# Ignalina/znippy

Hardware: AMD Instinct MI355X
Metric: decompress MB/s (uncompressed) + compress MB/s, 100k x 10KB archive (higher is better)
Workload: dtype u8; 1 GPU; 100k x 10KiB text chunks (BASELINE configs[1]); rows_per_gpu=100000, chunk_bytes=10240, bytes_per_gpu=1024000000, blob_bytes_per_gpu=6400000, parallelism=row-cursor ranges x1, pipelining=step k+1 queued before step k's counters are read (two runs in flight)

## Files before the change

### znippy_amd/csrc/api.hip

```cpp
#include <unistd.h>
#include "common.h"
#include "encode.h"
#include "../../include/znippy_hip.h"

#include <algorithm>
#include <cstdio>
#include <cstdlib>
#include <cstring>
#include <chrono>
#include <memory>
#include <string>
#include <vector>
#include <unordered_map>

namespace zn {
int measure_b3_pass_ns(int cus, hipStream_t s, float *ns_per_pass_per_simd, float *ghz);
size_t decode_lit_scratch_bytes(int grid);
void set_fused_dbg(unsigned long long *p);
void set_fused_abl(int v);
}

using namespace zn;
extern "C" void zn_rounds_totals(const uint64_t *len, const uint8_t *skip, size_t n, uint64_t out[8]);
extern "C" void zn_rows_extents(const uint64_t *bo, const uint64_t *bs, const uint64_t *oo, const uint64_t *us, size_t n, uint64_t out[8]);
extern "C" int zn_rows_pack32(const uint64_t *bo, const uint64_t *bs, const uint64_t *oo, const uint64_t *us, size_t n, uint32_t *dst);

#define HIPCHK(ctx, call)                                                                         \
    do {                                                                                          \
        hipError_t e_ = (call);                                                                   \
        if (e_ != hipSuccess) {                                                                   \
            (ctx)->err = std::string(#call) + ": " + hipGetErrorString(e_);                       \
            return ZNIPPY_E_HIP;                                                                  \
        }                                                                                         \
    } while (0)

struct TDbg {
    bool on;
    const char *what;
    std::chrono::steady_clock::time_point t;
    std::string line;
    TDbg(bool on_, const char *what_) : on(on_), what(what_), t(std::chrono::steady_clock::now()) {}
    void mark(const char *name) {
        if (!on) return;
        const auto now = std::chrono::steady_clock::now();
        char b[96];
        snprintf(b, sizeof b, " %s=%.3f", name, std::chrono::duration<double, std::milli>(now - t).count());
        line += b;
        t = now;
    }
    ~TDbg() { if (on) fprintf(stderr, "[znippy tdbg] %s:%s ms\n", what, line.c_str()); }
};

struct KTime {
    const char *name;
    hipEvent_t t0, t1;
};

struct znippy_ctx {
    int device = 0;
    hipStream_t stream = nullptr;
    bool own_stream = false;
    std::string err;
    int decode_grid = 0;
    uint8_t *lit_scratch = nullptr;
    uint32_t *cursor = nullptr;
    uint8_t *shim_in = nullptr, *shim_out = nullptr;
    size_t shim_in_cap = 0, shim_out_cap = 0;
    int encode_grid = 0, encode_grid_small = 0;
    int gen_share = 3;
    int level = 19;
    int window_log = 0;
    uint32_t *ldm = nullptr;
    size_t ldm_cap = 0;
    uint8_t *enc_prov = nullptr;
    size_t enc_prov_cap = 0;
    uint32_t *enc_seq = nullptr;
    EncTables *enc_tabs = nullptr;
    hipStream_t aux = nullptr;
    hipStream_t copy = nullptr;
    uint8_t *lit_scratch_b = nullptr;
    uint8_t *fz_lit_pool = nullptr;
    unsigned long long *fz_seq_pool = nullptr;
    uint64_t fz_lit_cap = 0, fz_seq_cap = 0;
    uint16_t *bx_fse_pool = nullptr;
    uint16_t *bx_huf_pool = nullptr;
    uint64_t bx_fse_cap = 0, bx_huf_cap = 0;
    uint32_t *rx_pool = nullptr, *rx_chunk = nullptr;
    uint8_t *rx_cdone = nullptr;
    uint64_t rx_cap = 0;
    uint8_t *vs_pool = nullptr;
    uint64_t vs_cap = 0;
    hipEvent_t ev_fork = nullptr, ev_join = nullptr, ev_join2 = nullptr;
    std::vector<KTime> ktimes;
    int n_ktimes = 0;
    std::vector<hipEvent_t> event_pool;
    bool ktime_open = false;
    std::vector<std::pair<size_t, void *>> pinned_pool;
    size_t pinned_pool_bytes = 0;
    std::vector<std::pair<size_t, void *>> dev_pool;
    std::unordered_map<void *, size_t> dev_sizes;
    size_t dev_pool_bytes = 0;
    struct {
        int dbg = 0;
        unsigned lds_pad = 0;
        int store_g = 0;
        bool no_block_items = false, no_fused_blocks = false, ddbg = false, edbg = false, no_fused_store = false,
             nohash = false, no_roles = false, no_fz = false, fz_only = false, no_bx = false, tdbg = false, no_fuse_hash = false, trace = false, no_rx = false, no_pack = false, no_lean = false, no_stored_only = false;
        unsigned roles_min = 2048;
        unsigned bx_big = BX_BIG_SEQ;
        bool bx_big_set = false;
        int ktime = 2;
    } sw;
    int cus = 256;
    int live_tables = 0;
    bool closing = false;
    unsigned long long *clk_buf = nullptr;
    enum Diag { DIAG_FUSED, DIAG_ITEMS, DIAG_FZ, DIAG_GENERAL, DIAG_BX, DIAG_ENCODE, DIAG_N };
    unsigned long long *diag[DIAG_N] = {};
};

static void read_switches(znippy_ctx *ctx) {
    auto on = [](const char *n) { const char *v = getenv(n); return v && *v && *v != '0'; };
    if (const char *e = getenv("ZNIPPY_DBG")) ctx->sw.dbg = atoi(e);
    if (const char *e = getenv("ZNIPPY_LDS_PAD")) ctx->sw.lds_pad = (unsigned)atoi(e);
    ctx->sw.no_block_items = on("ZNIPPY_NO_BLOCK_ITEMS");
    ctx->sw.no_fused_blocks = on("ZNIPPY_NO_FUSED_BLOCKS");
    ctx->sw.ddbg = on("ZNIPPY_DDBG");
    ctx->sw.edbg = on("ZNIPPY_EDBG");
    ctx->sw.no_fused_store = on("ZNIPPY_NO_FUSED_STORE");
    ctx->sw.nohash = on("ZNIPPY_NOHASH");
    ctx->sw.no_roles = on("ZNIPPY_NO_ROLES");
    ctx->sw.no_fz = on("ZNIPPY_NO_FZ");
    ctx->sw.tdbg = on("ZNIPPY_TDBG");
    ctx->sw.trace = on("ZNIPPY_TRACE");
    ctx->sw.no_lean = on("ZNIPPY_NO_LEAN");
    ctx->sw.no_pack = on("ZNIPPY_NO_PACK");
    if (const char *e = getenv("ZNIPPY_STORE_G")) ctx->sw.store_g = atoi(e) == 1 ? 1 : (atoi(e) == 2 ? 2 : 0);
    ctx->sw.no_stored_only = on("ZNIPPY_NO_STORED_ONLY");
    ctx->sw.no_rx = on("ZNIPPY_NO_RX");
    ctx->sw.no_fuse_hash = on("ZNIPPY_NO_FUSE_HASH");
    ctx->sw.no_bx = on("ZNIPPY_NO_BX");
    if (const char *e = getenv("ZNIPPY_BX_BIG")) { ctx->sw.bx_big = (unsigned)atoi(e); ctx->sw.bx_big_set = true; }
    if (const char *lv = getenv("ZNIPPY_LEVEL")) { const int v = atoi(lv); if (v >= 1 && v <= 22) ctx->level = v; }
    if (const char *wl = getenv("ZNIPPY_WINDOW_LOG")) { const int v = atoi(wl); if (v == 0 || (v >= WINDOW_LOG_MIN && v <= WINDOW_LOG_MAX)) ctx->window_log = v; }
    if (const char *gs = getenv("ZNIPPY_GEN_SHARE")) { const int v = atoi(gs); if (v >= 1 && v <= 4) ctx->gen_share = v; }
    ctx->sw.fz_only = on("ZNIPPY_FZ_ONLY");
    if (const char *e = getenv("ZNIPPY_ROLES_MIN")) ctx->sw.roles_min = (unsigned)atoi(e);
    if (const char *e = getenv("ZNIPPY_KTIME")) ctx->sw.ktime = atoi(e);
}

static void *pinned_take(znippy_ctx *ctx, size_t bytes, size_t *cap) {
    size_t best = ctx->pinned_pool.size();
    for (size_t i = 0; i < ctx->pinned_pool.size(); i++)
        if (ctx->pinned_pool[i].first >= bytes && ctx->pinned_pool[i].first <= 4 * bytes + 4096 &&
            (best == ctx->pinned_pool.size() || ctx->pinned_pool[i].first < ctx->pinned_pool[best].first))
            best = i;
    if (best != ctx->pinned_pool.size()) {
        void *p = ctx->pinned_pool[best].second;
        *cap = ctx->pinned_pool[best].first;
        ctx->pinned_pool_bytes -= *cap;
        ctx->pinned_pool.erase(ctx->pinned_pool.begin() + best);
        return p;
    }
    void *p = nullptr;
    if (hipHostMalloc(&p, bytes) != hipSuccess) return nullptr;
    *cap = bytes;
    return p;
}
static void pinned_give(znippy_ctx *ctx, void *p, size_t cap) {
    if (!p) return;
    if (ctx->pinned_pool.size() < 16 && ctx->pinned_pool_bytes + cap <= (256ull << 20)) {
        ctx->pinned_pool.emplace_back(cap, p);
        ctx->pinned_pool_bytes += cap;
    } else (void)hipHostFree(p);
}
static hipEvent_t event_take(znippy_ctx *ctx) {
    if (!ctx->event_pool.empty()) {
        hipEvent_t e = ctx->event_pool.back();
        ctx->event_pool.pop_back();
        return e;
    }
    hipEvent_t e = nullptr;
    if (hipEventCreateWithFlags(&e, hipEventDisableTiming) != hipSuccess) return nullptr;
    return e;
}
static void event_give(znippy_ctx *ctx, hipEvent_t e) {
    if (!e) return;
    if (ctx->event_pool.size() < 64) ctx->event_pool.push_back(e);
    else (void)hipEventDestroy(e);
}

template <class T>
static hipError_t tmalloc(znippy_ctx *ctx, T **out, size_t bytes) {
    bytes = std::max<size_t>(bytes, 16);
    size_t best = ctx->dev_pool.size();
    for (size_t i = 0; i < ctx->dev_pool.size(); i++)
        if (ctx->dev_pool[i].first >= bytes && ctx->dev_pool[i].first <= 2 * bytes + 4096 &&
            (best == ctx->dev_pool.size() || ctx->dev_pool[i].first < ctx->dev_pool[best].first))
            best = i;
    if (best != ctx->dev_pool.size()) {
        *out = (T *)ctx->dev_pool[best].second;
        ctx->dev_sizes[*out] = ctx->dev_pool[best].first;
        ctx->dev_pool_bytes -= ctx->dev_pool[best].first;
        ctx->dev_pool.erase(ctx->dev_pool.begin() + best);
        return hipSuccess;
    }
    void *p = nullptr;
    const hipError_t e = hipMalloc(&p, bytes);
    if (e != hipSuccess) return e;
    *out = (T *)p;
    ctx->dev_sizes[p] = bytes;
    return hipSuccess;
}
static void tfree(znippy_ctx *ctx, void *p) {
    if (!p) return;
    auto it = ctx->dev_sizes.find(p);
    if (it == ctx->dev_sizes.end()) { (void)hipFree(p); return; }
    const size_t cap = it->second;
    ctx->dev_sizes.erase(it);
    if (ctx->dev_pool.size() < 96 && ctx->dev_pool_bytes + cap <= (1ull << 30)) {
        ctx->dev_pool.emplace_back(cap, p);
        ctx->dev_pool_bytes += cap;
    } else (void)hipFree(p);
}

struct PlanBuf {
    std::vector<Tile> tiles;
    std::vector<BigUnit> big;
    uint32_t n_tile_cv = 0;
    std::vector<uint32_t> grp_big, grp_k;
};

template <class LenOf>
static void build_plan(LenOf len_of, uint32_t n, PlanBuf &p) {
    p.tiles.reserve((size_t)n / 4 + 16);
    uint32_t cur_first = 0, cur_units = 0, cur_leaves = 0;
    auto flush = [&]() {
        if (cur_units) p.tiles.push_back(Tile{cur_first, cur_units, 0, cur_leaves, 0, 0});
        cur_units = 0;
        cur_leaves = 0;
    };
    for (uint32_t u = 0; u < n; u++) {
        const uint64_t len_u = len_of(u);
        uint64_t leaves64 = len_u ? (len_u + 1023) >> 10 : 1;
        if (leaves64 > 64) {
            flush();
            uint32_t n_cvs = (uint32_t)((leaves64 + 63) / 64);
            p.big.push_back(BigUnit{u, p.n_tile_cv, n_cvs, 0});
            if (n_cvs > 64)
                for (uint32_t g = 0; g < (n_cvs + 63) / 64; g++) { p.grp_big.push_back((uint32_t)p.big.size() - 1); p.grp_k.push_back(g); }
            for (uint32_t t = 0; t < n_cvs; t++) {
                uint32_t first = t * 64;
                uint32_t nl = (uint32_t)std::min<uint64_t>(64, leaves64 - first);
                p.tiles.push_back(Tile{u, 0, first, nl, p.n_tile_cv + t, 0});
            }
            p.n_tile_cv += n_cvs;
        } else {
            uint32_t leaves = (uint32_t)leaves64;
            if (cur_units == 64 || cur_leaves + leaves > 64) flush();
            if (!cur_units) cur_first = u;
            cur_units++;
            cur_leaves += leaves;
            if (cur_units == 1 && u + 1 < n && len_of(u + 1) == len_u) {
                uint32_t v = u + 1;
                while (v < n && len_of(v) == len_u) v++;
                const uint32_t per = std::min<uint32_t>(64 / leaves, 64), run = v - u, full = run / per;
                if (full >= 1) {
                    for (uint32_t t = 0; t < full; t++) p.tiles.push_back(Tile{u + t * per, per, 0, per * leaves, 0, 0});
                    cur_units = 0; cur_leaves = 0;
                    const uint32_t rest = run - full * per;
                    if (rest) { cur_first = u + full * per; cur_units = rest; cur_leaves = rest * leaves; }
                    u = v - 1;
                }
            }
        }
    }
    flush();
    uint32_t gb = 0;
    for (BigUnit &b : p.big)
        if (b.n_cvs > 64) { b.pad = p.n_tile_cv + gb; gb += (b.n_cvs + 63) / 64; }
}

struct DevPlan {
    Tile *tiles = nullptr;
    BigUnit *big = nullptr;
    uint32_t *tile_cv = nullptr;
    uint32_t *grp_big = nullptr, *grp_k = nullptr;
    uint32_t n_grp = 0;
    uint32_t n_tiles = 0, n_big = 0;
    uint32_t max_cvs = 0;
};

static int upload_plan(znippy_ctx *ctx, const PlanBuf &p, DevPlan &d) {
    d.n_tiles = (uint32_t)p.tiles.size();
    d.n_big = (uint32_t)p.big.size();
    d.max_cvs = 0;
    for (const BigUnit &b : p.big) d.max_cvs = std::max(d.max_cvs, b.n_cvs);
    if (d.n_tiles) {
        HIPCHK(ctx, tmalloc(ctx, &d.tiles, sizeof(Tile) * d.n_tiles));
        HIPCHK(ctx, hipMemcpy(d.tiles, p.tiles.data(), sizeof(Tile) * d.n_tiles, hipMemcpyHostToDevice));
    }
    if (d.n_big) {
        HIPCHK(ctx, tmalloc(ctx, &d.big, sizeof(BigUnit) * d.n_big));
        HIPCHK(ctx, hipMemcpy(d.big, p.big.data(), sizeof(BigUnit) * d.n_big, hipMemcpyHostToDevice));
        HIPCHK(ctx, tmalloc(ctx, &d.tile_cv, 32 * ((size_t)p.n_tile_cv + p.grp_big.size())));
        d.n_grp = (uint32_t)p.grp_big.size();
        if (d.n_grp) {
            HIPCHK(ctx, tmalloc(ctx, &d.grp_big, 4 * (size_t)d.n_grp));
            HIPCHK(ctx, tmalloc(ctx, &d.grp_k, 4 * (size_t)d.n_grp));
            HIPCHK(ctx, hipMemcpy(d.grp_big, p.grp_big.data(), 4 * (size_t)d.n_grp, hipMemcpyHostToDevice));
            HIPCHK(ctx, hipMemcpy(d.grp_k, p.grp_k.data(), 4 * (size_t)d.n_grp, hipMemcpyHostToDevice));
        }
    }
    return ZNIPPY_OK;
}

static void free_plan(znippy_ctx *ctx, DevPlan &d) {
    tfree(ctx, d.tiles);
    tfree(ctx, d.big);
    tfree(ctx, d.tile_cv);
    tfree(ctx, d.grp_big);
    tfree(ctx, d.grp_k);
    d = DevPlan();
}

struct CtlRegion { size_t at, bytes; };
constexpr CtlRegion CTL_COUNTERS{0, 8 * 8};
constexpr CtlRegion CTL_HAND{64, 16 * 4};
constexpr CtlRegion CTL_CURSORS{128, 16 * 4};
constexpr CtlRegion CTL_FZ_POOL{192, 8 * 8};
constexpr CtlRegion CTL_BX_POOL{256, 16 * 8};
constexpr CtlRegion CTL_BX_CTR{384, 16 * 4};
constexpr CtlRegion CTL_RX{448, 16 * 4};
constexpr size_t CTL_HEAD = 512, CTL_MIRROR = 128, CTL_FLAG = 7;
constexpr uint32_t RX_ZERO = 15;
enum Hand : uint32_t {
    H_FUSED = 0,
    H_SERIAL = 1,
    H_ITEMS = 2,
    H_TILES = 3,
    H_FLAGGED = 5,
};
enum Cursor : uint32_t { CUR_GENERAL = 0, CUR_ROLES = 2, CUR_ITEMS = 4, CUR_FALLBACK = 8, CUR_FZ = 12, CUR_FZ_WORK = 13 };
constexpr uint32_t LEAN_ANY = 1u << H_FUSED | 1u << H_SERIAL | 1u << H_FLAGGED, LEAN_SMALL = LEAN_ANY | 1u << H_TILES, LEAN_BLOCKS = LEAN_ANY | 1u << H_ITEMS;
constexpr bool ctl_before(CtlRegion a, CtlRegion b) { return a.at + a.bytes <= b.at; }
static_assert(ctl_before(CTL_COUNTERS, CTL_HAND) && ctl_before(CTL_HAND, CTL_CURSORS) && ctl_before(CTL_CURSORS, CTL_FZ_POOL) && ctl_before(CTL_FZ_POOL, CTL_BX_POOL) &&
              ctl_before(CTL_BX_POOL, CTL_BX_CTR) && ctl_before(CTL_BX_CTR, CTL_RX) && CTL_RX.at + CTL_RX.bytes <= CTL_HEAD, "control block: regions overlap or pass the head");
static_assert(CTL_COUNTERS.at == 0 && CTL_HAND.at == CTL_COUNTERS.bytes && CTL_MIRROR == CTL_HAND.at + CTL_HAND.bytes, "the mirror is exactly counters + hand-over counts");
static_assert(CTL_FLAG < 8 && H_FLAGGED == H_SERIAL + 4 && H_FLAGGED < 8 && CUR_FZ_WORK < 16 && zn::RX_ROUNDS <= RX_ZERO && RX_ZERO < 16, "control block: a word outside its region");

struct znippy_rows {
    znippy_ctx *ctx = nullptr;
    uint64_t row_begin = 0;
    uint32_t n = 0;
    uint32_t n_compressed = 0;
    uint64_t *blob_off = nullptr, *blob_size = nullptr, *usize = nullptr, *out_off = nullptr;
    uint8_t *compressed = nullptr, *checksum = nullptr, *d_bitmap = nullptr;
    uint32_t *h_pack = nullptr, *d_pack = nullptr;
    size_t h_pack_cap = 0;
    unsigned long long *d_pack_sums = nullptr;
    uint8_t *ctl = nullptr;
    size_t ctl_bytes = 0;
    template <class T> T *ctl_at(CtlRegion g, size_t i = 0) const { return reinterpret_cast<T *>(ctl + g.at) + i; }
    uint32_t *hand(Hand h) const { return ctl_at<uint32_t>(CTL_HAND, h); }
    uint32_t *cur(Cursor c) const { return ctl_at<uint32_t>(CTL_CURSORS, c); }
    int32_t *status = nullptr;
    uint32_t *digests = nullptr;
    uint64_t *counters = nullptr;
    uint64_t *h_counters = nullptr;
    const uint32_t *mirror_hand(unsigned slot) const { return reinterpret_cast<const uint32_t *>(reinterpret_cast<const uint8_t *>(h_counters + 16 * slot) + CTL_HAND.at); }
    size_t h_counters_cap = 0;
    int bx_hint = -1;
    bool lean_ok = false;
    int lean_hint = -1;
    bool lean_blocks_ok = false;
    bool lean_mixed_ok = false;
    bool roles_off = false;
    bool small_ok = false, small_off = false;
    uint32_t *all_rows = nullptr;
    int lean_hint2 = -1;
    struct RunArgs { const void *blobs = nullptr; void *out = nullptr; uint64_t base = 0, cap = 0, blob_cap = ~0ull; bool verify = false; } run_args[2];
    uint64_t *vs_off = nullptr;
    uint64_t vs_bytes = 0;
    bool vs_built = false;
    bool no_out = false;
    hipEvent_t ev_done[2] = {nullptr, nullptr};
    uint64_t run_seq = 0;
    uint64_t ext_min_bo = 0, ext_max_bend = 0, ext_max_oend = 0;
    bool ext_wrap = false;
    std::vector<uint64_t> h_blob_off, h_blob_size, h_len, h_out_off;
    uint64_t blob_cap = ~0ull;
    uint64_t val_base = 0, val_bcap = 0, val_ocap = 0;
    bool val_done = false, val_verify = false;
    uint32_t n_bad = 0;
    bool force_full = false;
    uint8_t *status_init = nullptr;
    bool odd_out = false;
    uint64_t *corrupt = nullptr;
    uint32_t corrupt_cap = 0;
    uint32_t *list_a = nullptr;
    uint32_t n_list_a = 0;
    bool wide_rows = false;
    uint32_t *pending = nullptr;
    uint32_t n_cand = 0, n_items = 0;
    uint32_t *cand_row = nullptr, *cand_base = nullptr, *cand_nblocks = nullptr, *pending2 = nullptr;
    uint32_t *fz_base = nullptr, *fz_cap = nullptr, *fz_it_cand = nullptr, *fz_nb = nullptr, *fz_work = nullptr;
    zn::FzItem *fz_items = nullptr;
    uint32_t fz_total = 0;
    uint64_t fz_bytes = 0;
    uint32_t bx_slots = 0, bx_item_cap = 0;
    uint64_t bx_bytes = 0;
    uint64_t bx_nblk = 0;
    uint32_t *bx_cand_row = nullptr, *bx_cand_base = nullptr, *bx_cand_nb = nullptr, *bx_huf_list = nullptr, *bx_seq_list = nullptr, *bx_sort_tmp = nullptr;
    zn::FzItem *bx_items = nullptr;
    zn::BxPrep *bx_prep = nullptr;
    uint64_t rx_words = 0;
    uint64_t rx_words_small = 0;
    uint32_t rx_min = zn::RX_MIN;
    uint32_t *rx_base = nullptr, *rx_fail = nullptr, *rx_blk = nullptr, *rx_list = nullptr;
    uint32_t *item_row = nullptr, *item_k = nullptr, *item_src = nullptr, *row_flag = nullptr;
    uint32_t n_bt = 0;
    uint32_t *bt_tile = nullptr, *bt_item = nullptr;
    uint8_t *tile_done = nullptr, *item_done = nullptr;
    size_t done_bytes = 0;
    uint32_t *todo = nullptr;
    uint32_t n_small_tiles = 0;
    uint32_t *slow_list = nullptr;
    DevPlan plan;
};

struct znippy_rounds {
    znippy_ctx *ctx = nullptr;
    uint32_t n = 0;
    uint64_t *src_off = nullptr, *len = nullptr;
    uint8_t *skip = nullptr;
    uint32_t *digests = nullptr;
    std::vector<uint8_t> h_skip;
    void *plan_scratch[3] = {nullptr, nullptr, nullptr};
    uint64_t in_bytes = 0, enc_bytes = 0;
    bool all_stored_aligned = false;
    uint64_t blob_bound = 0;
    DevPlan plan;
    EncItem *items = nullptr;
    uint32_t n_items = 0;
    uint32_t *order_small = nullptr, *order_wide = nullptr;
    uint32_t n_small = 0, n_wide = 0;
    uint32_t *retry_list = nullptr, *retry_count = nullptr;
    uint64_t prov_bytes = 0;
    uint32_t *piece_len = nullptr, *piece_len_init = nullptr;
    uint64_t *piece_start = nullptr, *local_excl = nullptr, *block_tot = nullptr;
    uint8_t *res = nullptr, *h_res = nullptr;
    uint8_t *res_m[2] = {nullptr, nullptr}, *h_res_m[2] = {nullptr, nullptr};
    size_t h_res_cap_m[2] = {0, 0}, h_stored_cap = 0;
    hipEvent_t ev_enc[2] = {nullptr, nullptr}, ev_res[2] = {nullptr, nullptr};
    uint64_t run_seq = 0;
    size_t res_bytes = 0;
    bool store_incompressible = false;
    int fuse_tiles = 0;
    uint32_t *first_item = nullptr;
    uint8_t *stored = nullptr, *h_stored = nullptr;
    uint64_t *blob_offset = nullptr, *blob_size = nullptr, *total = nullptr;
    uint32_t *overflow = nullptr;
    std::vector<LdmRound> h_ldm;
    uint64_t ldm_entries = 0;
    uint32_t ldm_chunks = 0;
    LdmRound *d_ldm = nullptr;
    uint64_t *d_ldm_desc = nullptr;
};

static bool ktime_on(const znippy_ctx *ctx, const char *name) {
    return ctx->sw.ktime >= 2 || (ctx->sw.ktime == 1 && (!strncmp(name, "decode_verify_", 14) || !strncmp(name, "verify_", 7)));
}
static void ktime_begin(znippy_ctx *ctx, const char *name, hipStream_t on = nullptr) {
    if (ctx->sw.trace) { fprintf(stderr, "[znippy trace] %s ...", name); fflush(stderr); }
    ctx->ktime_open = ktime_on(ctx, name);
    if (!ctx->ktime_open) return;
    if ((int)ctx->ktimes.size() <= ctx->n_ktimes) {
        KTime k{name, nullptr, nullptr};
        (void)hipEventCreate(&k.t0);
        (void)hipEventCreate(&k.t1);
        ctx->ktimes.push_back(k);
    }
    ctx->ktimes[ctx->n_ktimes].name = name;
    (void)hipEventRecord(ctx->ktimes[ctx->n_ktimes].t0, on ? on : ctx->stream);
}
static void ktime_end(znippy_ctx *ctx, hipStream_t on = nullptr) {
    if (ctx->sw.trace) {
        const hipError_t e = hipStreamSynchronize(on ? on : ctx->stream);
        fprintf(stderr, " %s\n", e == hipSuccess ? "done" : hipGetErrorString(e));
        fflush(stderr);
    }
    if (!ctx->ktime_open) return;
    (void)hipEventRecord(ctx->ktimes[ctx->n_ktimes].t1, on ? on : ctx->stream);
    ctx->n_ktimes++;
}

template <class F>
static inline void timed(znippy_ctx *ctx, const char *name, hipStream_t on, F &&launch) {
    ktime_begin(ctx, name, on);
    launch();
    ktime_end(ctx, on);
}
template <size_t N, class Print>
static unsigned long long *diag_cycle(znippy_ctx *ctx, znippy_ctx::Diag which, hipStream_t s0, hipStream_t s1, Print print) {
    unsigned long long *&d = ctx->diag[which];
    if (!d) { (void)hipMalloc(&d, 8 * N); (void)hipMemset(d, 0, 8 * N); }
    unsigned long long h[N];
    (void)hipStreamSynchronize(s0);
    if (s1) (void)hipStreamSynchronize(s1);
    (void)hipMemcpy(h, d, 8 * N, hipMemcpyDeviceToHost);
    print(h);
    (void)hipMemset(d, 0, 8 * N);
    return d;
}

struct RowsRun { const void *d_blobs; uint64_t blob_base; void *d_out; uint64_t out_cap; int preset; unsigned slot; bool verify; };
static void set_out(BlockScanArgs &, uint8_t *) {}
template <class A> static void set_out(A &a, uint8_t *out) { a.out = out; }
template <class A>
static void fill_row_args(A &a, const znippy_rows *r, const RowsRun &run) {
    a.blobs = (const uint8_t *)run.d_blobs; a.blob_base = run.blob_base;
    a.blob_off = r->blob_off; a.blob_size = r->blob_size; a.usize = r->usize; a.out_off = run.verify ? r->vs_off : r->out_off;
    a.out_cap = run.out_cap; a.status = r->status; a.preset = run.preset;
    set_out(a, (uint8_t *)run.d_out);
}

template <class T>
static int dev_upload(znippy_ctx *ctx, T **d, const T *h, size_t n) {
    HIPCHK(ctx, tmalloc(ctx, d, sizeof(T) * n));
    if (n) HIPCHK(ctx, hipMemcpy(*d, h, sizeof(T) * n, hipMemcpyHostToDevice));
    return ZNIPPY_OK;
}

static int ensure_decoder(znippy_ctx *ctx) {
    if (ctx->lit_scratch) return ZNIPPY_OK;
    if (hipMalloc(&ctx->lit_scratch, decode_lit_scratch_bytes(ctx->decode_grid)) != hipSuccess) return ZNIPPY_E_NOMEM;
    return ZNIPPY_OK;
}
static int ensure_fz_pools(znippy_ctx *ctx, uint64_t content_bytes, uint32_t items) {
    constexpr uint64_t CAP = 16ull << 30;
    const uint64_t lit = std::min<uint64_t>(content_bytes + 80ull * items + 4096, CAP);
    const uint64_t seq = std::min<uint64_t>(content_bytes * 3 / 2 + 4096, CAP) / 8;
    if (lit > ctx->fz_lit_cap) {
        (void)hipStreamSynchronize(ctx->stream);
        if (ctx->fz_lit_pool) (void)hipFree(ctx->fz_lit_pool);
        ctx->fz_lit_pool = nullptr; ctx->fz_lit_cap = 0;
        if (hipMalloc(&ctx->fz_lit_pool, lit) != hipSuccess) { (void)hipGetLastError(); ctx->fz_lit_pool = nullptr; return ZNIPPY_OK; }
        ctx->fz_lit_cap = lit;
    }
    if (seq > ctx->fz_seq_cap) {
        (void)hipStreamSynchronize(ctx->stream);
        if (ctx->fz_seq_pool) (void)hipFree(ctx->fz_seq_pool);
        ctx->fz_seq_pool = nullptr; ctx->fz_seq_cap = 0;
        if (hipMalloc(&ctx->fz_seq_pool, seq * 8) != hipSuccess) { (void)hipGetLastError(); ctx->fz_seq_pool = nullptr; return ZNIPPY_OK; }
        ctx->fz_seq_cap = seq;
    }
    return ZNIPPY_OK;
}
static int ensure_bx_pools(znippy_ctx *ctx, uint64_t content_bytes, uint32_t items) {
    constexpr uint64_t CAP = 16ull << 30;
    const uint64_t bytes = std::min<uint64_t>(content_bytes / 2 + 64ull * items + 4096, CAP);
    const uint64_t fse = bytes / 2 + BX_POOL_FIRST, huf = bytes / 2;
    if (fse > ctx->bx_fse_cap) {
        (void)hipStreamSynchronize(ctx->stream);
        if (ctx->bx_fse_pool) (void)hipFree(ctx->bx_fse_pool);
        ctx->bx_fse_pool = nullptr; ctx->bx_fse_cap = 0;
        if (hipMalloc(&ctx->bx_fse_pool, fse * 2) != hipSuccess) { (void)hipGetLastError(); ctx->bx_fse_pool = nullptr; return ZNIPPY_OK; }
        uint16_t predef[BX_POOL_FIRST];
        bx_predefined_tables(predef);
        if (hipMemcpy(ctx->bx_fse_pool, predef, sizeof predef, hipMemcpyHostToDevice) != hipSuccess) return ZNIPPY_E_HIP;
        ctx->bx_fse_cap = fse;
    }
    if (huf > ctx->bx_huf_cap) {
        (void)hipStreamSynchronize(ctx->stream);
        if (ctx->bx_huf_pool) (void)hipFree(ctx->bx_huf_pool);
        ctx->bx_huf_pool = nullptr; ctx->bx_huf_cap = 0;
        if (hipMalloc(&ctx->bx_huf_pool, huf * 2) != hipSuccess) { (void)hipGetLastError(); ctx->bx_huf_pool = nullptr; return ZNIPPY_OK; }
        ctx->bx_huf_cap = huf;
    }
    return ZNIPPY_OK;
}
static int ensure_rx_pool(znippy_ctx *ctx, uint64_t words) {
    constexpr uint64_t CAP = (1ull << 31) - (1ull << 20);
    words = std::min<uint64_t>((words + 1023) & ~1023ull, CAP);
    if (words <= ctx->rx_cap) return ZNIPPY_OK;
    (void)hipStreamSynchronize(ctx->stream);
    if (ctx->rx_pool) (void)hipFree(ctx->rx_pool);
    if (ctx->rx_chunk) (void)hipFree(ctx->rx_chunk);
    if (ctx->rx_cdone) (void)hipFree(ctx->rx_cdone);
    ctx->rx_pool = nullptr; ctx->rx_chunk = nullptr; ctx->rx_cdone = nullptr; ctx->rx_cap = 0;
    if (hipMalloc(&ctx->rx_pool, words * 4) != hipSuccess || hipMalloc(&ctx->rx_chunk, words / 1024 * 4) != hipSuccess || hipMalloc(&ctx->rx_cdone, words / 1024) != hipSuccess) {
        (void)hipGetLastError();
        if (ctx->rx_pool) (void)hipFree(ctx->rx_pool);
        if (ctx->rx_chunk) (void)hipFree(ctx->rx_chunk);
        ctx->rx_pool = nullptr; ctx->rx_chunk = nullptr; ctx->rx_cdone = nullptr;
        return ZNIPPY_OK;
    }
    ctx->rx_cap = words;
    return ZNIPPY_OK;
}
static int ensure_verify_scratch(znippy_ctx *ctx, uint64_t bytes) {
    constexpr uint64_t CAP = 16ull << 30;
    if (!bytes) return ZNIPPY_OK;
    if (bytes > CAP) return ZNIPPY_E_NOMEM;
    bytes += 4096;
    if (bytes <= ctx->vs_cap) return ZNIPPY_OK;
    (void)hipStreamSynchronize(ctx->stream);
    if (ctx->vs_pool) (void)hipFree(ctx->vs_pool);
    ctx->vs_pool = nullptr; ctx->vs_cap = 0;
    if (hipMalloc(&ctx->vs_pool, bytes) != hipSuccess) { (void)hipGetLastError(); ctx->vs_pool = nullptr; return ZNIPPY_E_NOMEM; }
    ctx->vs_cap = bytes;
    return ZNIPPY_OK;
}
static int ensure_encoder(znippy_ctx *ctx) {
    if (ctx->enc_tabs) return ZNIPPY_OK;
    EncTables t;
    build_encode_tables(&t);
    if (hipMalloc(&ctx->enc_seq, (size_t)ctx->encode_grid * MAX_SEQ * 3 * 4) != hipSuccess ||
        hipMalloc(&ctx->enc_tabs, sizeof(EncTables)) != hipSuccess ||
        hipMemcpy(ctx->enc_tabs, &t, sizeof t, hipMemcpyHostToDevice) != hipSuccess) {
        if (ctx->enc_tabs) { (void)hipFree(ctx->enc_tabs); ctx->enc_tabs = nullptr; }
        return ZNIPPY_E_NOMEM;
    }
    return ZNIPPY_OK;
}

__device__ __forceinline__ void block_excl_scan2(unsigned long long &a, unsigned long long &b, unsigned long long *sa, unsigned long long *sb,
                                                 unsigned long long *ta, unsigned long long *tb) {
    const uint32_t t = threadIdx.x;
    const unsigned long long a0 = a, b0 = b;
    sa[t] = a; sb[t] = b;
    __syncthreads();
    for (uint32_t d = 1; d < 256; d <<= 1) {
        unsigned long long xa = 0, xb = 0;
        if (t >= d) { xa = sa[t - d]; xb = sb[t - d]; }
        __syncthreads();
        sa[t] += xa; sb[t] += xb;
        __syncthreads();
    }
    *ta = sa[255]; *tb = sb[255];
    a = sa[t] - a0; b = sb[t] - b0;
    __syncthreads();
}
__global__ __launch_bounds__(256) void k_rows_unpack_sums(const uint32_t *bs32, const uint32_t *us32, uint32_t n, unsigned long long *sums) {
    __shared__ unsigned long long sa[256], sb[256];
    const uint32_t lo = blockIdx.x * 1024 + threadIdx.x * 4;
    unsigned long long a = 0, b = 0, ta, tb;
    for (uint32_t k = 0; k < 4; k++) if (lo + k < n) { a += bs32[lo + k]; b += us32[lo + k]; }
    block_excl_scan2(a, b, sa, sb, &ta, &tb);
    if (threadIdx.x == 0) { sums[2 * blockIdx.x] = ta; sums[2 * blockIdx.x + 1] = tb; }
}
__global__ __launch_bounds__(256) void k_rows_unpack_scan(unsigned long long *sums, uint32_t nblk) {
    __shared__ unsigned long long sa[256], sb[256];
    unsigned long long ca = 0, cb = 0;
    for (uint32_t b0 = 0; b0 < nblk; b0 += 256) {
        const uint32_t i = b0 + threadIdx.x;
        unsigned long long a = i < nblk ? sums[2 * i] : 0, b = i < nblk ? sums[2 * i + 1] : 0, ta, tb;
        block_excl_scan2(a, b, sa, sb, &ta, &tb);
        if (i < nblk) { sums[2 * i] = ca + a; sums[2 * i + 1] = cb + b; }
        ca += ta; cb += tb;
    }
}
__global__ __launch_bounds__(256) void k_rows_unpack_fill(const uint32_t *bs32, const uint32_t *us32, uint32_t n, const unsigned long long *sums,
                                                          uint64_t bo0, uint64_t oo0, uint64_t *bo, uint64_t *bs, uint64_t *oo, uint64_t *us) {
    __shared__ unsigned long long sa[256], sb[256];
    const uint32_t lo = blockIdx.x * 1024 + threadIdx.x * 4;
    uint32_t vb[4] = {0, 0, 0, 0}, vu[4] = {0, 0, 0, 0};
    unsigned long long a = 0, b = 0, ta, tb;
    for (uint32_t k = 0; k < 4; k++) if (lo + k < n) { vb[k] = bs32[lo + k]; vu[k] = us32[lo + k]; a += vb[k]; b += vu[k]; }
    block_excl_scan2(a, b, sa, sb, &ta, &tb);
    unsigned long long pb = bo0 + sums[2 * blockIdx.x] + a, po = oo0 + sums[2 * blockIdx.x + 1] + b;
    for (uint32_t k = 0; k < 4; k++) if (lo + k < n) {
        bo[lo + k] = pb; bs[lo + k] = vb[k]; oo[lo + k] = po; us[lo + k] = vu[k];
        pb += vb[k]; po += vu[k];
    }
}

constexpr unsigned long long VS_ROW_MAX = (16ull << 30) + 16, VS_GROUP_MAX = 32ull << 30;
__device__ __forceinline__ unsigned long long vs_slot_bytes(const uint8_t *comp, const uint64_t *usize, uint32_t i) {
    if (!comp[i]) return 0ull;
    const unsigned long long u = usize[i];
    return u >= VS_ROW_MAX ? VS_ROW_MAX : (u + 15) & ~15ull;
}
__global__ __launch_bounds__(256) void k_rows_slot_sums(const uint8_t *comp, const uint64_t *usize, uint32_t n, unsigned long long *sums) {
    __shared__ unsigned long long sa[256], sb[256];
    const uint32_t lo = blockIdx.x * 1024 + threadIdx.x * 4;
    unsigned long long a = 0, b = 0, ta, tb;
    for (uint32_t k = 0; k < 4; k++) if (lo + k < n) a += vs_slot_bytes(comp, usize, lo + k);
    block_excl_scan2(a, b, sa, sb, &ta, &tb);
    if (threadIdx.x == 0) { sums[2 * blockIdx.x] = ta < VS_GROUP_MAX ? ta : VS_GROUP_MAX; sums[2 * blockIdx.x + 1] = 0; }
}
__global__ __launch_bounds__(256) void k_rows_slot_fill(const uint8_t *comp, const uint64_t *usize, uint32_t n, unsigned long long *sums, uint32_t nblk, uint64_t *slot_off) {
    __shared__ unsigned long long sa[256], sb[256];
    const uint32_t lo = blockIdx.x * 1024 + threadIdx.x * 4;
    unsigned long long v[4] = {0, 0, 0, 0}, a = 0, b = 0, ta, tb;
    for (uint32_t k = 0; k < 4; k++) if (lo + k < n) { v[k] = vs_slot_bytes(comp, usize, lo + k); a += v[k]; }
    block_excl_scan2(a, b, sa, sb, &ta, &tb);
    unsigned long long at = sums[2 * blockIdx.x] + a;
// ... 12 lines not shown
    const uint64_t row = row_begin + i;
    const uint8_t c = bitmap ? (bitmap[row >> 3] >> (row & 7)) & 1 : 1;
    comp[i] = c;
    if (!c) usize[i] = blob_size[i];
}

struct RoundCount { uint32_t items, small, wide; uint64_t prov; };
__device__ __forceinline__ RoundCount round_count(uint64_t L, uint32_t sk) {
    RoundCount c;
    if (sk) { c.items = (uint32_t)(L ? (L + SKIP_PIECE - 1) / SKIP_PIECE : 1); c.small = 0; c.wide = 0; c.prov = 0; return c; }
    const uint32_t nb = (uint32_t)(L ? (L + BLOCK_BYTES - 1) / BLOCK_BYTES : 1);
    const uint32_t tail = (uint32_t)(L - (uint64_t)(nb - 1) * BLOCK_BYTES), tw = tail > 16 * 1024 ? 1u : 0u;
    c.items = nb; c.wide = nb - 1 + tw; c.small = 1 - tw;
    c.prov = (uint64_t)(nb - 1) * enc_slot_bytes(BLOCK_BYTES) + enc_slot_bytes(tail);
    return c;
}
struct RoundSums { uint32_t items, small, wide, pad; uint64_t prov; };
__device__ __forceinline__ void round_block_scan(uint32_t &ai, uint32_t &as, uint32_t &aw, uint64_t &ap, uint32_t *s_i, uint32_t *s_s, uint32_t *s_w, uint64_t *s_p,
                                                 RoundSums *total) {
    const uint32_t t = threadIdx.x;
    const uint32_t vi = ai, vs = as, vw = aw;
    const uint64_t vp = ap;
    s_i[t] = ai; s_s[t] = as; s_w[t] = aw; s_p[t] = ap;
    __syncthreads();
    for (uint32_t d = 1; d < 256; d <<= 1) {
        uint32_t bi = 0, bs = 0, bw = 0; uint64_t bp = 0;
        if (t >= d) { bi = s_i[t - d]; bs = s_s[t - d]; bw = s_w[t - d]; bp = s_p[t - d]; }
        __syncthreads();
        s_i[t] += bi; s_s[t] += bs; s_w[t] += bw; s_p[t] += bp;
        __syncthreads();
    }
    ai = s_i[t] - vi; as = s_s[t] - vs; aw = s_w[t] - vw; ap = s_p[t] - vp;
    if (total) { total->items = s_i[255]; total->small = s_s[255]; total->wide = s_w[255]; total->pad = 0; total->prov = s_p[255]; }
    __syncthreads();
}
__global__ __launch_bounds__(256) void k_rounds_sums(const uint64_t *len, const uint8_t *skip, uint32_t n, RoundSums *sums) {
    __shared__ uint32_t s_i[256], s_s[256], s_w[256];
    __shared__ uint64_t s_p[256];
    const uint32_t lo = blockIdx.x * 1024 + threadIdx.x * 4;
    uint32_t ai = 0, as = 0, aw = 0;
    uint64_t ap = 0;
    for (uint32_t i = lo; i < lo + 4 && i < n; i++) { const RoundCount c = round_count(len[i], skip ? skip[i] : 0); ai += c.items; as += c.small; aw += c.wide; ap += c.prov; }
    RoundSums tot;
    round_block_scan(ai, as, aw, ap, s_i, s_s, s_w, s_p, &tot);
    if (threadIdx.x == 0) sums[blockIdx.x] = tot;
}
__global__ __launch_bounds__(256) void k_rounds_scan(RoundSums *sums, uint32_t nblk) {
    __shared__ uint32_t s_i[256], s_s[256], s_w[256];
    __shared__ uint64_t s_p[256];
    RoundSums carry{0, 0, 0, 0, 0};
    for (uint32_t b0 = 0; b0 < nblk; b0 += 256) {
        const uint32_t b = b0 + threadIdx.x;
        RoundSums v{0, 0, 0, 0, 0};
        if (b < nblk) v = sums[b];
        uint32_t ai = v.items, as = v.small, aw = v.wide;
        uint64_t ap = v.prov;
        RoundSums tot;
        round_block_scan(ai, as, aw, ap, s_i, s_s, s_w, s_p, &tot);
        if (b < nblk) sums[b] = RoundSums{carry.items + ai, carry.small + as, carry.wide + aw, 0, carry.prov + ap};
        carry.items += tot.items; carry.small += tot.small; carry.wide += tot.wide; carry.prov += tot.prov;
    }
}
__global__ __launch_bounds__(256) void k_rounds_fill(const uint64_t *len, const uint8_t *skip, uint32_t n, const RoundSums *sums, uint32_t *first_item,
                                                      EncItem *items, uint32_t *plen, uint32_t *ord_small, uint32_t *ord_wide) {
    __shared__ uint32_t s_i[256], s_s[256], s_w[256];
    __shared__ uint64_t s_p[256];
    const uint32_t lo = blockIdx.x * 1024 + threadIdx.x * 4;
    RoundCount c[4];
    uint32_t ai = 0, as = 0, aw = 0;
    uint64_t ap = 0;
    for (uint32_t q = 0; q < 4; q++) {
        const uint32_t i = lo + q;
        c[q] = i < n ? round_count(len[i], skip ? skip[i] : 0) : RoundCount{0, 0, 0, 0};
        ai += c[q].items; as += c[q].small; aw += c[q].wide; ap += c[q].prov;
    }
    round_block_scan(ai, as, aw, ap, s_i, s_s, s_w, s_p, nullptr);
    const RoundSums base = sums[blockIdx.x];
    uint32_t at = base.items + ai, so = base.small + as, wo = base.wide + aw;
    uint64_t prov = base.prov + ap;
    for (uint32_t q = 0; q < 4; q++) {
        const uint32_t i = lo + q;
        if (i >= n) break;
        const uint64_t L = len[i];
        first_item[i] = at;
        if (skip && skip[i]) {
            const uint32_t np = c[q].items;
            for (uint32_t k = 0; k < np; k++) {
                const uint64_t o = (uint64_t)k * SKIP_PIECE;
                items[at + k] = EncItem{i, k, np, ITEM_SKIP | (k == 0 ? ITEM_FIRST : 0u), o};
                plen[at + k] = (uint32_t)(L - o < SKIP_PIECE ? L - o : SKIP_PIECE);
            }
            at += np;
            continue;
        }
        const uint32_t nb = c[q].items;
        for (uint32_t k = 0; k < nb; k++) {
            const uint32_t bl = (uint32_t)(L - (uint64_t)k * BLOCK_BYTES < BLOCK_BYTES ? L - (uint64_t)k * BLOCK_BYTES : BLOCK_BYTES);
            if (bl > 16 * 1024) ord_wide[wo++] = at + k; else ord_small[so++] = at + k;
            items[at + k] = EncItem{i, k, nb, k == 0 ? ITEM_FIRST : 0u, prov};
            plen[at + k] = 0;
            prov += enc_slot_bytes(bl);
        }
        at += nb;
    }
}

extern "C" {

int znippy_ctx_create(int device, void *hip_stream, znippy_ctx **out) {
    if (!out) return ZNIPPY_E_INVAL;
    znippy_ctx *ctx = new znippy_ctx();
    ctx->device = device;
    read_switches(ctx);
    if (hipSetDevice(device) != hipSuccess) { delete ctx; return ZNIPPY_E_HIP; }
    if (hip_stream) ctx->stream = (hipStream_t)hip_stream;
    else {
        if (hipStreamCreateWithFlags(&ctx->stream, hipStreamNonBlocking) != hipSuccess) { delete ctx; return ZNIPPY_E_HIP; }
        ctx->own_stream = true;
    }
    init_fused_tables();
    if (hipStreamCreateWithFlags(&ctx->aux, hipStreamNonBlocking) != hipSuccess ||
        hipStreamCreateWithFlags(&ctx->copy, hipStreamNonBlocking) != hipSuccess ||
        hipEventCreateWithFlags(&ctx->ev_fork, hipEventDisableTiming) != hipSuccess ||
        hipEventCreateWithFlags(&ctx->ev_join, hipEventDisableTiming) != hipSuccess ||
        hipEventCreateWithFlags(&ctx->ev_join2, hipEventDisableTiming) != hipSuccess) {
        znippy_ctx_destroy(ctx);
        return ZNIPPY_E_HIP;
    }
    ctx->decode_grid = decode_grid_size(device);
    if (hipMalloc(&ctx->cursor, 64) != hipSuccess) {
        znippy_ctx_destroy(ctx);
        return ZNIPPY_E_NOMEM;
    }
    {
        hipDeviceProp_t p;
        int cus = hipGetDeviceProperties(&p, device) == hipSuccess ? p.multiProcessorCount : 256;
        ctx->cus = cus;
        ctx->encode_grid = cus * 8;
        ctx->encode_grid_small = cus * 16;
    }
    *out = ctx;
    return ZNIPPY_OK;
}

static void ctx_teardown(znippy_ctx *ctx);
void znippy_ctx_destroy(znippy_ctx *ctx) {
    if (!ctx || ctx->closing) return;
    if (ctx->live_tables) {
        (void)hipSetDevice(ctx->device);
        (void)hipStreamSynchronize(ctx->stream);
        ctx->closing = true;
        return;
    }
    ctx_teardown(ctx);
}
static void table_released(znippy_ctx *ctx) {
    if (--ctx->live_tables == 0 && ctx->closing) ctx_teardown(ctx);
}
static void ctx_teardown(znippy_ctx *ctx) {
    (void)hipSetDevice(ctx->device);
    (void)hipStreamSynchronize(ctx->stream);
    for (auto &k : ctx->ktimes) { (void)hipEventDestroy(k.t0); (void)hipEventDestroy(k.t1); }
    void *dev[] = {ctx->lit_scratch, ctx->lit_scratch_b, ctx->fz_lit_pool, ctx->fz_seq_pool, ctx->bx_fse_pool, ctx->bx_huf_pool, ctx->rx_pool, ctx->rx_chunk, ctx->rx_cdone, ctx->cursor, ctx->vs_pool,
                   ctx->clk_buf, ctx->shim_in, ctx->shim_out, ctx->enc_prov, ctx->enc_seq, ctx->enc_tabs, ctx->ldm};
    for (void *p : dev) if (p) (void)hipFree(p);
    for (unsigned long long *d : ctx->diag) if (d) (void)hipFree(d);
    if (ctx->aux) { (void)hipStreamSynchronize(ctx->aux); (void)hipStreamDestroy(ctx->aux); }
    if (ctx->copy) { (void)hipStreamSynchronize(ctx->copy); (void)hipStreamDestroy(ctx->copy); }
    for (auto &e : ctx->pinned_pool) (void)hipHostFree(e.second);
    for (auto &e : ctx->dev_pool) (void)hipFree(e.second);
    for (hipEvent_t e : ctx->event_pool) (void)hipEventDestroy(e);
    if (ctx->ev_fork) (void)hipEventDestroy(ctx->ev_fork);
    if (ctx->ev_join) (void)hipEventDestroy(ctx->ev_join);
    if (ctx->ev_join2) (void)hipEventDestroy(ctx->ev_join2);
    if (ctx->own_stream) (void)hipStreamDestroy(ctx->stream);
    delete ctx;
}

const char *znippy_last_error(const znippy_ctx *ctx) { return ctx ? ctx->err.c_str() : "null context"; }

int znippy_ctx_sync(znippy_ctx *ctx) {
    if (ctx && ctx->closing) return ZNIPPY_E_INVAL;
    if (!ctx) return ZNIPPY_E_INVAL;
    HIPCHK(ctx, hipStreamSynchronize(ctx->stream));
    if (ctx->copy) HIPCHK(ctx, hipStreamSynchronize(ctx->copy));
    return ZNIPPY_OK;
}

int znippy_last_kernel_times(znippy_ctx *ctx, const char **names, float *ms, int cap) {
    if (ctx && ctx->closing) return ZNIPPY_E_INVAL;
    if (!ctx) return 0;
    int n = std::min(cap, ctx->n_ktimes);
    for (int i = 0; i < n; i++) {
        names[i] = ctx->ktimes[i].name;
        ms[i] = 0.f;
        (void)hipEventElapsedTime(&ms[i], ctx->ktimes[i].t0, ctx->ktimes[i].t1);
    }
    return n;
}

int znippy_rows_foreign_stats(znippy_ctx *ctx, znippy_rows *r, uint64_t stats[8]) {
    if (ctx && ctx->closing) return ZNIPPY_E_INVAL;
    if (!ctx || !r || r->ctx != ctx || !stats) return ZNIPPY_E_INVAL;
    HIPCHK(ctx, hipSetDevice(ctx->device));
    HIPCHK(ctx, hipStreamSynchronize(ctx->stream));
    HIPCHK(ctx, hipMemcpy(stats, r->ctl + (r->bx_slots ? CTL_BX_POOL : CTL_FZ_POOL).at, 64, hipMemcpyDeviceToHost));
    return ZNIPPY_OK;
}

int znippy_ctx_set_level(znippy_ctx *ctx, int level) {
    if (ctx && ctx->closing) return ZNIPPY_E_INVAL;
    if (!ctx || level < 1 || level > 22) return ZNIPPY_E_INVAL;
    ctx->level = level;
    return ZNIPPY_OK;
}

int znippy_ctx_level(const znippy_ctx *ctx) { return ctx ? ctx->level : ZNIPPY_E_INVAL; }

int znippy_ctx_set_window_log(znippy_ctx *ctx, int window_log) {
    if (ctx && ctx->closing) return ZNIPPY_E_INVAL;
    if (!ctx || (window_log != 0 && (window_log < WINDOW_LOG_MIN || window_log > WINDOW_LOG_MAX))) return ZNIPPY_E_INVAL;
    ctx->window_log = window_log;
    return ZNIPPY_OK;
}

int znippy_ctx_window_log(const znippy_ctx *ctx) { return ctx && !ctx->closing ? ctx->window_log : ZNIPPY_E_INVAL; }

int znippy_ctx_set_kernel_timing(znippy_ctx *ctx, int level) {
    if (ctx && ctx->closing) return ZNIPPY_E_INVAL;
    if (!ctx || level < 0 || level > 2) return ZNIPPY_E_INVAL;
    ctx->sw.ktime = level;
    return ZNIPPY_OK;
}

int znippy_measure_blake3_pass_ns(znippy_ctx *ctx, float *ns_per_pass_per_simd, float *shader_ghz) {
    if (ctx && ctx->closing) return ZNIPPY_E_INVAL;
    if (!ctx || !ns_per_pass_per_simd) return ZNIPPY_E_INVAL;
    HIPCHK(ctx, hipSetDevice(ctx->device));
    HIPCHK(ctx, hipStreamSynchronize(ctx->stream));
    return measure_b3_pass_ns(ctx->cus, ctx->stream, ns_per_pass_per_simd, shader_ghz);
}

int znippy_last_shader_ghz(znippy_ctx *ctx, float *ghz) {
    if (ctx && ctx->closing) return ZNIPPY_E_INVAL;
    if (!ctx || !ghz) return ZNIPPY_E_INVAL;
    *ghz = 0.f;
    if (!ctx->clk_buf) return ZNIPPY_OK;
    HIPCHK(ctx, hipStreamSynchronize(ctx->stream));
    unsigned long long h[2] = {0, 0};
    HIPCHK(ctx, hipMemcpy(h, ctx->clk_buf, 16, hipMemcpyDeviceToHost));
    if (h[1]) *ghz = (float)((double)h[0] / (double)h[1] * 0.1);
    return ZNIPPY_OK;
}

static ptrdiff_t skippable_prefix(const uint8_t *p, size_t n) {
    size_t at = 0;
    while (n - at >= 8) {
        uint32_t magic, sz;
        memcpy(&magic, p + at, 4);
        if ((magic & 0xFFFFFFF0u) != 0x184D2A50u) break;
        memcpy(&sz, p + at + 4, 4);
        if ((uint64_t)8 + sz > n - at) return -1;
        at += 8 + (size_t)sz;
    }
    return (ptrdiff_t)at;
}

int znippy_get_decompressed_size(const void *frame, size_t n, uint64_t *out_size) {
    const uint8_t *p = (const uint8_t *)frame;
    if (!p || !out_size) return ZNIPPY_E_INVAL;
    {
        const ptrdiff_t skip = skippable_prefix(p, n);
        if (skip < 0) return ZNIPPY_E_CORRUPT;
        p += skip;
        n -= (size_t)skip;
    }
    if (n < 5) return ZNIPPY_E_CORRUPT;
    uint32_t magic;
    memcpy(&magic, p, 4);
    if (magic != 0xFD2FB528u) return ZNIPPY_E_CORRUPT;
    uint32_t fhd = p[4], fcs_flag = fhd >> 6, single = (fhd >> 5) & 1, did_flag = fhd & 3;
    if (fhd & 8) return ZNIPPY_E_CORRUPT;
    uint32_t fcs_bytes = fcs_flag == 0 ? single : (1u << fcs_flag);
    uint32_t did_bytes = did_flag == 3 ? 4 : did_flag;
    size_t pos = 5 + (single ? 0 : 1) + did_bytes;
    if (n < pos + fcs_bytes) return ZNIPPY_E_CORRUPT;
    if (!fcs_bytes) return ZNIPPY_E_UNSUPPORTED;
    uint64_t fcs = 0;
    for (uint32_t i = 0; i < fcs_bytes; i++) fcs |= (uint64_t)p[pos + i] << (8 * i);
    if (fcs_bytes == 2) fcs += 256;
    *out_size = fcs;
    return ZNIPPY_OK;
}


void znippy_rows_destroy(znippy_rows *r) {
    if (!r) return;
    (void)hipSetDevice(r->ctx->device);
    void *ptrs[] = {r->blob_off, r->blob_size, r->usize, r->out_off, r->compressed, r->checksum,
                    r->ctl, r->digests, r->corrupt, r->list_a, r->pending,
                    r->cand_row, r->cand_base, r->cand_nblocks, r->fz_base, r->fz_cap, r->fz_it_cand, r->fz_nb, r->fz_work, r->fz_items, r->item_row, r->item_k, r->item_src, r->row_flag, r->pending2,
                    r->bt_tile, r->bt_item, r->tile_done, r->todo, r->status_init, r->slow_list,
                    r->bx_cand_row, r->bx_cand_base, r->bx_cand_nb, r->bx_huf_list, r->bx_seq_list, r->bx_items, r->bx_prep, r->d_bitmap, r->bx_sort_tmp,
                    r->rx_base, r->rx_fail, r->rx_blk, r->rx_list, r->d_pack, r->d_pack_sums, r->all_rows, r->vs_off};
    for (void *p : ptrs)
        tfree(r->ctx, p);
    if (r->h_counters) {
        (void)hipStreamSynchronize(r->ctx->stream);
        pinned_give(r->ctx, r->h_counters, r->h_counters_cap);
    }
    if (r->h_pack) {
        (void)hipStreamSynchronize(r->ctx->stream);
        pinned_give(r->ctx, r->h_pack, r->h_pack_cap);
    }
    for (hipEvent_t e : r->ev_done) event_give(r->ctx, e);
    free_plan(r->ctx, r->plan);
    znippy_ctx *const c = r->ctx;
    delete r;
    table_released(c);
}

struct RowCols {
    const uint64_t *bo, *bs, *us, *oo;
    const uint8_t *bitmap;
    uint64_t row_begin, row_end;
    bool allc;
    uint32_t comp(uint32_t i) const { if (allc) return 1u; const uint64_t row = row_begin + i; return (bitmap[row >> 3] >> (row & 7)) & 1u; }
};
struct RowClasses {
    std::vector<uint32_t> la, cand_row, cand_base, cand_nb, item_row, item_k, fz_base, fz_cap, fz_it_cand;
    uint64_t big_bytes = 0, big_blob = 0, n_big = 0, nblk = 0;
};

static int rows_columns_h2d(znippy_ctx *ctx, znippy_rows *r, const RowCols &c, const uint8_t *checksum, TDbg &td) {
    const uint32_t n = r->n;
    int rc = ZNIPPY_OK;
    const uint64_t bm0 = c.row_begin >> 3, bm1 = (c.row_end + 7) >> 3;
    bool packed = false;
    if (n >= 64 && !ctx->sw.no_pack) {
        r->h_pack = (uint32_t *)pinned_take(ctx, 8 * (size_t)n, &r->h_pack_cap);
        if (r->h_pack && zn_rows_pack32(c.bo, c.bs, c.oo, c.us, n, r->h_pack)) {
            const uint32_t nblk = (n + 1023) / 1024;
            if (tmalloc(ctx, &r->d_pack, 8 * (size_t)n) != hipSuccess || tmalloc(ctx, &r->d_pack_sums, 16 * (size_t)nblk) != hipSuccess ||
                tmalloc(ctx, &r->blob_off, 8 * (size_t)n) != hipSuccess || tmalloc(ctx, &r->blob_size, 8 * (size_t)n) != hipSuccess ||
                tmalloc(ctx, &r->usize, 8 * (size_t)n) != hipSuccess || tmalloc(ctx, &r->out_off, 8 * (size_t)n) != hipSuccess ||
                hipMemcpyAsync(r->d_pack, r->h_pack, 8 * (size_t)n, hipMemcpyHostToDevice, ctx->stream) != hipSuccess)
                return ZNIPPY_E_NOMEM;
            hipLaunchKernelGGL(k_rows_unpack_sums, dim3(nblk), dim3(256), 0, ctx->stream, r->d_pack, r->d_pack + n, n, r->d_pack_sums);
            hipLaunchKernelGGL(k_rows_unpack_scan, dim3(1), dim3(256), 0, ctx->stream, r->d_pack_sums, nblk);
            hipLaunchKernelGGL(k_rows_unpack_fill, dim3(nblk), dim3(256), 0, ctx->stream, r->d_pack, r->d_pack + n, n, r->d_pack_sums, c.bo[0], c.oo[0],
                               r->blob_off, r->blob_size, r->out_off, r->usize);
            packed = true;
        }
    }
    if ((!packed && ((rc = dev_upload(ctx, &r->blob_off, c.bo, n)) || (rc = dev_upload(ctx, &r->blob_size, c.bs, n)) ||
                     (rc = dev_upload(ctx, &r->usize, c.us, n)) || (rc = dev_upload(ctx, &r->out_off, c.oo, n)))) ||
        (c.bitmap && (rc = dev_upload(ctx, &r->d_bitmap, c.bitmap + bm0, (size_t)(bm1 - bm0)))) ||
        tmalloc(ctx, &r->compressed, std::max<size_t>(n, 16)) != hipSuccess)
        return rc ? rc : ZNIPPY_E_NOMEM;
    if (n) hipLaunchKernelGGL(k_rows_fixup, dim3((n + 255) / 256), dim3(256), 0, ctx->stream, r->d_bitmap, c.row_begin - 8 * bm0, n, r->compressed, r->usize, r->blob_size);
    td.mark("columns_h2d");
    if (checksum && (rc = dev_upload(ctx, &r->checksum, checksum + 32 * c.row_begin, (size_t)32 * n))) return rc;
    td.mark("checksum_h2d");
    return ZNIPPY_OK;
}

static void rows_classify(const znippy_ctx *ctx, znippy_rows *r, const RowCols &c, RowClasses &k) {
    constexpr uint64_t BLK = 128 * 1024;
    const uint32_t n = r->n;
    if (c.allc) {
        uint64_t e[8];
        zn_rows_extents(c.bo, c.bs, c.oo, c.us, n, e);
        if (e[6] == 0) {
            r->ext_min_bo = e[0]; r->ext_max_bend = e[1]; r->ext_max_oend = e[2]; r->ext_wrap = e[3] != 0;
            r->n_compressed = n; r->bx_bytes = e[4]; k.nblk = e[5];
            return;
        }
    }
    uint64_t min_bo = ~0ull, max_bend = 0, max_oend = 0;
    bool wrap = false;
    for (uint32_t i = 0; i < n; i++) {
        const uint32_t comp = c.comp(i);
        const uint64_t bo = c.bo[i], bs = c.bs[i], oo = c.oo[i], us = comp ? c.us[i] : bs;
        r->n_compressed += comp;
        if (!comp && (oo & 15)) r->odd_out = true;
        min_bo = std::min(min_bo, bo);
        wrap |= bo + bs < bo || oo + us < oo;
        max_bend = std::max(max_bend, bo + bs);
        max_oend = std::max(max_oend, oo + us);
        if (!comp) continue;
        k.nblk += us ? (us + BLK - 1) / BLK : 1;
        r->bx_bytes += us;
        if (us > 65536 && us < (1ull << 30)) r->rx_words_small += (us + 1023) & ~1023ull;
        if (us >= zn::RX_MIN && us < (1ull << 30)) r->rx_words += (us + 1023) & ~1023ull;
        if (us <= 64 * 1024) continue;
        k.big_bytes += us;
        k.big_blob += bs;
        k.n_big++;
        const uint64_t nb = (us + BLK - 1) / BLK;
        if (nb >= 2 && us < 0xFFFFFFFFull && k.item_row.size() + nb < 0x7FFFFFFFull && !ctx->sw.no_block_items) {
            k.cand_row.push_back(i);
            k.cand_base.push_back((uint32_t)k.item_row.size());
            k.cand_nb.push_back((uint32_t)nb);
            for (uint32_t b = 0; b < nb; b++) { k.item_row.push_back(i); k.item_k.push_back(b); }
            if (!ctx->sw.no_fz && ctx->sw.no_bx && k.fz_it_cand.size() + 2 * nb + 8 < 0x7FFFFFFFull) {
                const uint32_t cap = (uint32_t)(2 * nb + 8);
                k.fz_base.push_back((uint32_t)k.fz_it_cand.size());
                k.fz_cap.push_back(cap);
                k.fz_it_cand.insert(k.fz_it_cand.end(), cap, (uint32_t)k.cand_row.size() - 1);
                r->fz_bytes += us;
            } else { k.fz_base.push_back(0); k.fz_cap.push_back(0); }
        } else k.la.push_back(i);
    }
    r->ext_min_bo = min_bo; r->ext_max_bend = max_bend; r->ext_max_oend = max_oend; r->ext_wrap = wrap;
}

static int rows_batch_buffers(znippy_ctx *ctx, znippy_rows *r, uint64_t nblk) {
    if (tmalloc(ctx, &r->row_flag, std::max<size_t>(4 * (size_t)r->n, 16)) != hipSuccess ||
        tmalloc(ctx, &r->pending2, std::max<size_t>(4 * (size_t)r->n_compressed, 16)) != hipSuccess)
        return ZNIPPY_E_NOMEM;
    if (ctx->sw.no_bx) return ZNIPPY_OK;
    r->bx_nblk = nblk;
    if (r->rx_words_small && r->rx_words_small <= (256ull << 20)) { r->rx_min = 65537; r->rx_words = r->rx_words_small; }
    const uint64_t cap = nblk + nblk / 2 + std::min<uint64_t>(3 * nblk, 65536) + 1024;
    if (cap >= 0x7FFFFFFFull) return ZNIPPY_OK;
    r->bx_slots = r->n_compressed;
    r->bx_item_cap = (uint32_t)cap;
    if (tmalloc(ctx, &r->bx_cand_row, 4 * (size_t)r->bx_slots) != hipSuccess || tmalloc(ctx, &r->bx_cand_base, 4 * (size_t)r->bx_slots) != hipSuccess ||
        tmalloc(ctx, &r->bx_cand_nb, 4 * (size_t)r->bx_slots) != hipSuccess || tmalloc(ctx, &r->bx_huf_list, 4 * (size_t)cap) != hipSuccess ||
        tmalloc(ctx, &r->bx_seq_list, 4 * 4 * (size_t)cap) != hipSuccess || tmalloc(ctx, &r->bx_sort_tmp, 5 * 4 * (size_t)cap) != hipSuccess || tmalloc(ctx, &r->bx_items, sizeof(zn::FzItem) * (size_t)cap) != hipSuccess ||
        tmalloc(ctx, &r->bx_prep, sizeof(zn::BxPrep) * (size_t)cap) != hipSuccess ||
        ((r->rx_words || r->rx_words_small) && !ctx->sw.no_rx &&
         (tmalloc(ctx, &r->rx_base, 4 * (size_t)r->bx_slots) != hipSuccess || tmalloc(ctx, &r->rx_fail, 4 * (size_t)r->bx_slots) != hipSuccess ||
          tmalloc(ctx, &r->rx_blk, 16 * (size_t)cap) != hipSuccess || tmalloc(ctx, &r->rx_list, 4 * (size_t)cap) != hipSuccess)))
        return ZNIPPY_E_NOMEM;
    return ZNIPPY_OK;
}
static int rows_item_buffers(znippy_ctx *ctx, znippy_rows *r, const RowClasses &k) {
    int rc;
    if ((rc = dev_upload(ctx, &r->cand_row, k.cand_row.data(), k.cand_row.size())) ||
        (rc = dev_upload(ctx, &r->cand_base, k.cand_base.data(), k.cand_base.size())) ||
        (rc = dev_upload(ctx, &r->cand_nblocks, k.cand_nb.data(), k.cand_nb.size())) ||
        (rc = dev_upload(ctx, &r->item_row, k.item_row.data(), k.item_row.size())) ||
        (rc = dev_upload(ctx, &r->item_k, k.item_k.data(), k.item_k.size())))
        return rc;
    if (tmalloc(ctx, &r->item_src, 4 * (size_t)r->n_items) != hipSuccess) return ZNIPPY_E_NOMEM;
    r->fz_total = (uint32_t)k.fz_it_cand.size();
    if (!r->fz_total) return ZNIPPY_OK;
    if ((rc = dev_upload(ctx, &r->fz_base, k.fz_base.data(), k.fz_base.size())) ||
        (rc = dev_upload(ctx, &r->fz_cap, k.fz_cap.data(), k.fz_cap.size())) ||
        (rc = dev_upload(ctx, &r->fz_it_cand, k.fz_it_cand.data(), k.fz_it_cand.size())))
        return rc;
    if (tmalloc(ctx, &r->fz_nb, 4 * (size_t)r->n_cand) != hipSuccess || tmalloc(ctx, &r->fz_work, 4 * (size_t)r->fz_total) != hipSuccess ||
        tmalloc(ctx, &r->fz_items, sizeof(zn::FzItem) * (size_t)r->fz_total) != hipSuccess)
        return ZNIPPY_E_NOMEM;
    return ZNIPPY_OK;
}
static int rows_fused_block_buffers(znippy_ctx *ctx, znippy_rows *r, const RowClasses &k, const PlanBuf &p) {
    std::vector<uint32_t> row_base(r->n, 0xFFFFFFFFu), bt_tile, bt_item;
    for (size_t c = 0; c < k.cand_row.size(); c++) row_base[k.cand_row[c]] = k.cand_base[c];
    for (uint32_t ti = 0; ti < (uint32_t)p.tiles.size(); ti++) {
        const Tile &t = p.tiles[ti];
        if (t.n_units == 0 && row_base[t.first_unit] != 0xFFFFFFFFu) {
            bt_tile.push_back(ti);
            bt_item.push_back(row_base[t.first_unit] + (t.first_leaf >> 7));
        }
    }
    r->n_bt = (uint32_t)bt_tile.size();
    int rc;
    if ((rc = dev_upload(ctx, &r->bt_tile, bt_tile.data(), bt_tile.size())) || (rc = dev_upload(ctx, &r->bt_item, bt_item.data(), bt_item.size()))) return rc;
    const size_t td_bytes = (std::max<size_t>(p.tiles.size(), 16) + 15) & ~(size_t)15;
    r->done_bytes = td_bytes + std::max<size_t>(r->n_items, 16);
    if (tmalloc(ctx, &r->tile_done, r->done_bytes) != hipSuccess ||
        tmalloc(ctx, &r->todo, std::max<size_t>(4 * (size_t)r->n_items, 16)) != hipSuccess)
        return ZNIPPY_E_NOMEM;
    r->item_done = r->tile_done + td_bytes;
    return ZNIPPY_OK;
}

int znippy_rows_create(znippy_ctx *ctx, const uint64_t *blob_offset, const uint64_t *blob_size,
                       const uint8_t *compressed_bitmap, const uint64_t *uncompressed_size,
                       const uint64_t *out_offset, const uint8_t *checksum, uint64_t row_begin,
                       uint64_t row_end, znippy_rows **out) {
    if (ctx && ctx->closing) return ZNIPPY_E_INVAL;
    if (!ctx || !out || row_end < row_begin || !blob_offset || !blob_size || !uncompressed_size)
        return ZNIPPY_E_INVAL;
    if (row_end - row_begin >= 0xFFFFFFF0ull) return ZNIPPY_E_INVAL;
    HIPCHK(ctx, hipSetDevice(ctx->device));
    TDbg td(ctx->sw.tdbg, "rows_create");
    std::unique_ptr<znippy_rows, void (*)(znippy_rows *)> guard(new znippy_rows(), znippy_rows_destroy);
    znippy_rows *const r = guard.get();
    r->ctx = ctx;
    ctx->live_tables++;
    r->row_begin = row_begin;
    r->n = (uint32_t)(row_end - row_begin);
    const uint32_t n = r->n;
    bool allc = true;
    if (compressed_bitmap) {
        uint64_t row = row_begin;
        for (; row < row_end && (row & 7); row++) allc &= (compressed_bitmap[row >> 3] >> (row & 7)) & 1;
        for (; row + 8 <= row_end && allc; row += 8) allc &= compressed_bitmap[row >> 3] == 0xFF;
        for (; row < row_end && allc; row++) allc &= (compressed_bitmap[row >> 3] >> (row & 7)) & 1;
    }
    std::vector<uint64_t> own_oo;
    if (!out_offset) {
        r->no_out = true;
        own_oo.resize(n);
        uint64_t at = 0;
        for (uint32_t i = 0; i < n; i++) { own_oo[i] = at; at += uncompressed_size[row_begin + i]; }
    }
    const RowCols c{blob_offset + row_begin, blob_size + row_begin, uncompressed_size + row_begin, out_offset ? out_offset + row_begin : own_oo.data(), compressed_bitmap, row_begin, row_end, allc};
    int rc = rows_columns_h2d(ctx, r, c, checksum, td);
    if (rc) return rc;
    r->corrupt_cap = std::max<uint32_t>(n, 1);
    r->ctl_bytes = CTL_HEAD + std::max<size_t>(4 * (size_t)n, 16);
    if (tmalloc(ctx, &r->ctl, r->ctl_bytes) != hipSuccess ||
        tmalloc(ctx, &r->digests, std::max<size_t>(32 * (size_t)n, 32)) != hipSuccess ||
        !(r->h_counters = (uint64_t *)pinned_take(ctx, 256, &r->h_counters_cap)) ||
        !(r->ev_done[0] = event_take(ctx)) || !(r->ev_done[1] = event_take(ctx)) ||
        tmalloc(ctx, &r->corrupt, 8 * (size_t)r->corrupt_cap) != hipSuccess)
        return ZNIPPY_E_NOMEM;
    r->counters = r->ctl_at<uint64_t>(CTL_COUNTERS);
    r->status = reinterpret_cast<int32_t *>(r->ctl + CTL_HEAD);
    td.mark("allocs");
    PlanBuf p;
    build_plan([=, us = c.us, bs = c.bs, &c](uint32_t i) -> uint64_t { return (allc || c.comp(i)) ? us[i] : bs[i]; }, n, p);
    td.mark("plan");
    if ((rc = upload_plan(ctx, p, r->plan))) return rc;
    td.mark("plan_h2d");
    for (const Tile &t : p.tiles) r->n_small_tiles += t.n_units != 0;
    if (r->n_small_tiles && tmalloc(ctx, &r->slow_list, 4 * (size_t)p.tiles.size()) != hipSuccess) return ZNIPPY_E_NOMEM;
    RowClasses k;
    rows_classify(ctx, r, c, k);
    r->n_list_a = (uint32_t)k.la.size();
    td.mark("big_rows");
    if (r->n_compressed && (rc = rows_batch_buffers(ctx, r, k.nblk))) return rc;
    r->wide_rows = k.n_big && k.big_bytes / k.n_big >= (1u << 20) && k.big_blob * 50 < k.big_bytes;
    r->n_cand = (uint32_t)k.cand_row.size();
    r->n_items = (uint32_t)k.item_row.size();
    const bool hints = !ctx->sw.no_lean && r->n_list_a == 0;
    const uint32_t n_tiles = (uint32_t)p.tiles.size();
    r->small_ok = allc && hints && !ctx->sw.no_bx && r->n_cand == 0 && r->n_small_tiles == n_tiles && r->n_small_tiles > 0 && r->bx_slots;
    r->lean_mixed_ok = hints && r->n_cand == 0 && r->n_small_tiles > 0 && r->n_small_tiles < n_tiles;
    r->lean_blocks_ok = allc && hints && r->n_cand > 0 && r->n_small_tiles == 0;
    r->lean_ok = allc && hints && r->n_cand == 0 && p.big.empty() && r->n_small_tiles == n_tiles && r->n_small_tiles > 0;
    if (r->n_cand && (rc = rows_item_buffers(ctx, r, k))) return rc;
    if (r->n_cand && !ctx->sw.no_fused_blocks && (rc = rows_fused_block_buffers(ctx, r, k, p))) return rc;
    if ((rc = dev_upload(ctx, &r->list_a, k.la.data(), k.la.size()))) return rc;
    if (tmalloc(ctx, &r->pending, std::max<size_t>(4 * (size_t)n, 16)) != hipSuccess) return ZNIPPY_E_NOMEM;
    td.mark("rest");
    *out = guard.release();
    return ZNIPPY_OK;
}

int znippy_rows_set_blob_cap(znippy_rows *r, uint64_t blob_cap) {
    if (!r) return ZNIPPY_E_INVAL;
    r->blob_cap = blob_cap;
    return ZNIPPY_OK;
}

static int rows_validate(znippy_ctx *ctx, znippy_rows *r, uint64_t blob_base, uint64_t out_cap, bool verify) {
    if (verify) out_cap = ~0ull;
    if (r->val_done && r->val_verify == verify && r->val_base == blob_base && r->val_bcap == r->blob_cap && r->val_ocap == out_cap) return ZNIPPY_OK;
    std::vector<int32_t> init;
    uint32_t bad = 0;
    const uint64_t bcap = r->blob_cap;
    const bool fits = !r->ext_wrap && (r->n == 0 || (r->ext_min_bo >= blob_base && (bcap == ~0ull || r->ext_max_bend - blob_base <= bcap) && (verify || r->ext_max_oend <= out_cap)));
    if (!fits && r->h_blob_off.empty() && r->n) {
        r->h_blob_off.resize(r->n); r->h_blob_size.resize(r->n); r->h_len.resize(r->n);
        HIPCHK(ctx, hipStreamSynchronize(ctx->stream));
        HIPCHK(ctx, hipMemcpy(r->h_blob_off.data(), r->blob_off, 8 * (size_t)r->n, hipMemcpyDeviceToHost));
        HIPCHK(ctx, hipMemcpy(r->h_blob_size.data(), r->blob_size, 8 * (size_t)r->n, hipMemcpyDeviceToHost));
        HIPCHK(ctx, hipMemcpy(r->h_len.data(), r->usize, 8 * (size_t)r->n, hipMemcpyDeviceToHost));
    }
    if (!fits && !verify && r->h_out_off.empty() && r->n) {
        r->h_out_off.resize(r->n);
        HIPCHK(ctx, hipStreamSynchronize(ctx->stream));
        HIPCHK(ctx, hipMemcpy(r->h_out_off.data(), r->out_off, 8 * (size_t)r->n, hipMemcpyDeviceToHost));
    }
    for (uint32_t i = 0; i < (fits ? 0u : r->n); i++) {
        const uint64_t bo = r->h_blob_off[i], bs = r->h_blob_size[i], len = verify ? 0 : r->h_len[i], oo = verify ? 0 : r->h_out_off[i];
        int code = 0;
        if (bo < blob_base) code = ZNIPPY_E_CORRUPT;
        else if (bcap != ~0ull && (bs > bcap || bo - blob_base > bcap - bs)) code = ZNIPPY_E_CORRUPT;
        else if (len > out_cap || oo > out_cap - len) code = ZNIPPY_E_DST_SMALL;
        if (code) {
            if (init.empty()) init.assign(r->n, 0);
            init[i] = code;
            bad++;
        }
    }
    if (bad) {
        if (!r->status_init) {
            if (tmalloc(ctx, &r->status_init, r->ctl_bytes) != hipSuccess) return ZNIPPY_E_NOMEM;
            HIPCHK(ctx, hipMemset(r->status_init, 0, r->ctl_bytes));
        }
        HIPCHK(ctx, hipMemcpy(r->status_init + CTL_HEAD, init.data(), 4 * (size_t)r->n, hipMemcpyHostToDevice));
    }
    r->n_bad = bad;
    r->val_base = blob_base; r->val_bcap = r->blob_cap; r->val_ocap = out_cap;
    r->val_done = true; r->val_verify = verify;
    return ZNIPPY_OK;
}

static int rows_verify_slots(znippy_ctx *ctx, znippy_rows *r) {
    if (r->vs_built) return ZNIPPY_OK;
    if (r->n && r->n_compressed) {
        const uint32_t nblk = (r->n + 1023) / 1024;
        unsigned long long *sums = nullptr;
        if (tmalloc(ctx, &r->vs_off, 8 * (size_t)r->n) != hipSuccess) return ZNIPPY_E_NOMEM;
        if (tmalloc(ctx, &sums, 16 * ((size_t)nblk + 1)) != hipSuccess) return ZNIPPY_E_NOMEM;
        hipLaunchKernelGGL(k_rows_slot_sums, dim3(nblk), dim3(256), 0, ctx->stream, r->compressed, r->usize, r->n, sums);
        hipLaunchKernelGGL(k_rows_unpack_scan, dim3(1), dim3(256), 0, ctx->stream, sums, nblk);
        hipLaunchKernelGGL(k_rows_slot_fill, dim3(nblk), dim3(256), 0, ctx->stream, r->compressed, r->usize, r->n, sums, nblk, r->vs_off);
        unsigned long long total = 0;
        const hipError_t e1 = hipStreamSynchronize(ctx->stream), e2 = hipMemcpy(&total, sums + 2 * (size_t)nblk, 8, hipMemcpyDeviceToHost);
        tfree(ctx, sums);
        HIPCHK(ctx, e1);
        HIPCHK(ctx, e2);
        r->vs_bytes = total;
    } else if (r->n) {
        if (tmalloc(ctx, &r->vs_off, 8 * (size_t)r->n) != hipSuccess) return ZNIPPY_E_NOMEM;
        HIPCHK(ctx, hipMemsetAsync(r->vs_off, 0, 8 * (size_t)r->n, ctx->stream));
    }
    r->vs_built = true;
    return ZNIPPY_OK;
}

static void rows_note_hint(znippy_rows *r, unsigned slot) {
    const uint32_t *left = r->mirror_hand(slot);
    const bool handed = left[H_FUSED] || left[H_SERIAL] || left[H_FLAGGED];
    r->bx_hint = (handed || r->n_list_a) ? 1 : 0;
    r->lean_hint = (handed || left[H_TILES]) ? 0 : 1;
    r->lean_hint2 = (handed || left[H_ITEMS]) ? 0 : 1;
    if (r->n_small_tiles && left[H_TILES] >= r->n_small_tiles) r->roles_off = true;
    if (r->small_ok && left[H_FUSED] >= r->n) r->small_off = true;
    if (r->small_off) r->bx_hint = 1;
}

struct RunPlan {
    bool bx;
    bool small_off;
    bool stored_only;
    bool roles;
    bool lean;
    bool lean_mixed;
    bool decode;
    bool one_stream;
    bool lean_blocks;
    bool behind;
    bool rx;
    bool third;
};
static RunPlan rows_plan(const znippy_ctx *ctx, const znippy_rows *r, int preset) {
    const auto &sw = ctx->sw;
    RunPlan p{};
    p.bx = r->bx_slots && ctx->fz_lit_pool && ctx->fz_seq_pool && ctx->bx_fse_pool && ctx->bx_huf_pool && r->bx_hint != 0;
    p.small_off = p.bx && r->small_off && !r->n_bad && !r->force_full && !sw.dbg;
    p.stored_only = r->n_compressed == 0 && !preset && !sw.dbg && !sw.no_stored_only && !r->force_full;
    const bool may_skip = !preset && !r->force_full;
    if (!p.small_off && !p.stored_only) {
        p.roles = !sw.no_roles && sw.roles_min != 0 && r->n_small_tiles >= sw.roles_min && r->n_small_tiles > 0 && !(sw.dbg & (1 | 2 | 4 | 8 | 128)) && !r->roles_off;
        p.lean_mixed = r->lean_mixed_ok && r->lean_hint == 1 && r->bx_hint == 0 && may_skip && !sw.dbg && !sw.ddbg;
        p.lean = p.roles && r->lean_ok && r->lean_hint == 1 && r->bx_hint == 0 && may_skip && !sw.dbg;
    }
    p.decode = !p.lean && !p.lean_mixed && !p.stored_only;
    if (!p.decode) return p;
    p.one_stream = r->n_cand && r->bx_hint == 0 && r->n_small_tiles == 0;
    p.lean_blocks = p.one_stream && r->lean_blocks_ok && r->lean_hint2 == 1 && may_skip && r->n_bt && !sw.ddbg && !r->fz_total;
    if (!r->n_compressed) return p;
    p.behind = !p.bx && r->n_cand && r->bx_hint == 0;
    p.rx = p.bx && r->rx_base && ctx->rx_pool && r->rx_words;
    p.third = p.bx && r->bx_nblk <= 32768;
    return p;
}

static HashArgs rows_hash_args(const znippy_ctx *ctx, const znippy_rows *r, const RowsRun &run) {
    HashArgs h{};
    h.tiles = r->plan.tiles; h.n_tiles = r->plan.n_tiles;
    h.len = r->usize;
    h.srcA = (const uint8_t *)run.d_blobs; h.offA = r->blob_off; h.baseA = run.blob_base;
    h.srcB = (uint8_t *)run.d_out; h.offB = run.verify ? r->vs_off : r->out_off;
    h.sel = r->compressed; h.status = r->status; h.pending_count = r->hand(H_FUSED);
    h.copy_to_B = run.verify ? 0 : 1;
    h.store_tiles = ctx->sw.store_g;
    h.misaligned_dst = !run.verify && (r->odd_out || ((uintptr_t)run.d_out & 15) != 0);
    h.digests = r->digests; h.tile_cv = r->plan.tile_cv;
    return h;
}
static BlockScanArgs rows_scan_args(const znippy_rows *r, const RowsRun &run) {
    BlockScanArgs b{};
    b.cand_row = r->cand_row; b.cand_base = r->cand_base; b.cand_nblocks = r->cand_nblocks; b.n_cand = r->n_cand;
    fill_row_args(b, r, run);
    b.item_src = r->item_src; b.row_flag = r->row_flag;
    b.pending = r->pending2; b.pending_count = r->hand(H_SERIAL);
    return b;
}
static DecodeArgs rows_decode_args(znippy_ctx *ctx, const znippy_rows *r, const RowsRun &run) {
    DecodeArgs a{};
    fill_row_args(a, r, run);
    a.list_a = r->list_a; a.n_list_a = r->n_list_a;
    a.pending = r->pending; a.pending_count = r->hand(H_FUSED);
    a.compressed = r->compressed;
    a.n_rows = r->n; a.cursor = r->cur(CUR_GENERAL);
    a.lit_scratch = ctx->lit_scratch;
    if (ctx->sw.ddbg)
        a.dbg = diag_cycle<8>(ctx, znippy_ctx::DIAG_GENERAL, ctx->stream, nullptr, [](const unsigned long long *h) {
            if (h[0]) fprintf(stderr, "[znippy ddbg] general decoder frames=%llu  kcycles per frame: headers+tree=%.1f huffman-table=%.1f literal-streams=%.1f seq-tables=%.1f first-batch=%.1f decode+execute=%.1f tail=%.1f\n", h[0],
                              h[6] / 1e3 / h[0], h[7] / 1e3 / h[0], h[1] / 1e3 / h[0], h[2] / 1e3 / h[0], h[3] / 1e3 / h[0], h[4] / 1e3 / h[0], h[5] / 1e3 / h[0]);
        });
    return a;
}
static void decode_rest(znippy_ctx *ctx, const znippy_rows *r, DecodeArgs a, uint32_t rows) {
    a.list_a = nullptr; a.n_list_a = 0;
    a.pending = r->pending2; a.pending_count = r->hand(H_SERIAL);
    a.cursor = r->cur(CUR_FALLBACK);
    timed(ctx, "zstd_decode_fallback", ctx->stream, [&] {
        if (!ctx->sw.fz_only) launch_decode(a, std::min<int>(ctx->decode_grid, (int)rows), r->wide_rows, ctx->stream);
    });
}

static int run_clear(znippy_ctx *ctx, znippy_rows *r, const RunPlan &p, const RowsRun &run) {
    hipStream_t s = ctx->stream;
    if (run.preset) HIPCHK(ctx, hipMemcpyAsync(r->ctl, r->status_init, r->ctl_bytes, hipMemcpyDeviceToDevice, s));
    else HIPCHK(ctx, hipMemsetAsync(r->ctl, 0, r->ctl_bytes, s));
    if (p.small_off) HIPCHK(ctx, hipMemsetD32Async((hipDeviceptr_t)r->hand(H_FUSED), (int)r->n, 1, s));
    return ZNIPPY_OK;
}

static int run_small_rows(znippy_ctx *ctx, znippy_rows *r, const RunPlan &p, const RowsRun &run) {
    hipStream_t s = ctx->stream;
    FusedArgs f{};
    f.h = rows_hash_args(ctx, r, run);
    f.h.pass = 1;
    f.blob_size = r->blob_size; f.out_cap = run.out_cap; f.status = r->status;
    f.preset = run.preset;
    f.pending = r->pending; f.pending_count = r->hand(H_FUSED);
    f.dbg = ctx->sw.dbg;
    if (f.dbg & 8) {
        f.dbg_buf = diag_cycle<8>(ctx, znippy_ctx::DIAG_FUSED, s, nullptr, [](const unsigned long long *h4) {
            if (h4[3]) fprintf(stderr, "[znippy dbg] waves=%llu prologue=%.0f decode=%.0f hash=%.0f | parse+lits=%.0f expand-build=%.0f stream-out=%.0f after-match=%.0f cycles/wave\n", h4[3],
                               (double)h4[0] / h4[3], (double)h4[1] / h4[3], (double)h4[2] / h4[3], (double)h4[6] / h4[3], (double)h4[4] / h4[3], (double)h4[5] / h4[3], (double)h4[7] / h4[3]);
        });
        set_fused_dbg(f.dbg_buf);
    }
    if (f.dbg & 32768) {
        if (!ctx->clk_buf) { (void)hipMalloc(&ctx->clk_buf, 64); (void)hipMemset(ctx->clk_buf, 0, 64); }
        f.dbg_buf = ctx->clk_buf;
    }
    if (f.dbg & (16 | 32 | 64)) set_fused_abl(f.dbg);
    f.lds_pad = ctx->sw.lds_pad;
    const hipStream_t fs = p.lean_mixed ? ctx->aux : s;
    if (p.lean_mixed) {
        HIPCHK(ctx, hipEventRecord(ctx->ev_fork, s));
        HIPCHK(ctx, hipStreamWaitEvent(ctx->aux, ctx->ev_fork, 0));
    }
    if (p.roles) {
        f.cursor = r->cur(CUR_ROLES);
        f.tile_list = r->slow_list;
        f.tile_count = r->hand(H_TILES);
        timed(ctx, run.verify ? "verify_roles" : "decode_verify_roles", fs, [&] { launch_fused_roles(f, ctx->cus, fs, run.verify); });
    }
    if (r->n_small_tiles && !p.lean) timed(ctx, run.verify ? "verify_small" : "decode_verify_fused", fs, [&] { launch_fused_small(f, fs, p.roles ? ctx->cus * 5 : 0, run.verify); });
    if (p.lean_mixed) HIPCHK(ctx, hipEventRecord(ctx->ev_join, ctx->aux));
    return ZNIPPY_OK;
}

static void run_two_phase(znippy_ctx *ctx, znippy_rows *r, const RowsRun &run, hipStream_t ba) {
    FzArgs z{};
    z.cand_row = r->cand_row; z.cand_fzbase = r->fz_base; z.cand_fzcap = r->fz_cap; z.n_cand = r->n_cand;
    z.it_cand = r->fz_it_cand; z.total_items = r->fz_total; z.cand_nb = r->fz_nb; z.items = r->fz_items;
    fill_row_args(z, r, run);
    z.row_flag = r->row_flag;
    z.lit_pool = ctx->fz_lit_pool; z.lit_cap = ctx->fz_lit_cap; z.seq_pool = ctx->fz_seq_pool; z.seq_cap = ctx->fz_seq_cap;
    z.pool_used = r->ctl_at<unsigned long long>(CTL_FZ_POOL);
    z.cursor = r->cur(CUR_FZ);
    if (ctx->sw.ddbg)
        z.dbg = diag_cycle<32>(ctx, znippy_ctx::DIAG_FZ, ctx->stream, ba, [](const unsigned long long *h) {
            if (h[0]) fprintf(stderr, "[znippy ddbg] fz exec: frames=%llu groups=%llu seqs=%llu big=%llu rounds=%llu flushes=%llu histreads=%llu rep_groups=%llu | kcycles/frame: total=%.0f records=%.0f rep+scan=%.0f big=%.0f flush=%.0f histread=%.0f lits=%.0f matches=%.0f tail=%.0f\n",
                              h[0], h[1], h[2], h[3], h[4], h[5], h[6], h[7], h[8] / 1e3 / h[0], h[9] / 1e3 / h[0], h[10] / 1e3 / h[0], h[11] / 1e3 / h[0],
                              h[12] / 1e3 / h[0], h[13] / 1e3 / h[0], h[14] / 1e3 / h[0], h[15] / 1e3 / h[0], h[16] / 1e3 / h[0]);
            if (h[20]) fprintf(stderr, "[znippy ddbg] fz entropy: blocks=%llu seqs=%llu | kcycles/block: literal tree=%.0f literal table+streams=%.0f sequence tables=%.0f sequence decode=%.0f\n",
                               h[20], h[25], h[21] / 1e3 / h[20], h[22] / 1e3 / h[20], h[23] / 1e3 / h[20], h[24] / 1e3 / h[20]);
        });
    launch_fz_scan(z, r->fz_work, r->cur(CUR_FZ_WORK), ba);
    timed(ctx, "zstd_foreign_entropy", ba, [&] { launch_fz_entropy(z, ctx->cus, r->fz_work, r->cur(CUR_FZ_WORK), ba); });
    timed(ctx, "zstd_foreign_execute", ba, [&] { launch_fz_exec(z, ba); });
}

static int run_block_items(znippy_ctx *ctx, znippy_rows *r, const RunPlan &p, const RowsRun &run) {
    hipStream_t s = ctx->stream;
    const hipStream_t ba = p.one_stream ? s : ctx->aux;
    const BlockScanArgs b = rows_scan_args(r, run);
    if (!p.one_stream) {
        HIPCHK(ctx, hipEventRecord(ctx->ev_fork, s));
        HIPCHK(ctx, hipStreamWaitEvent(ba, ctx->ev_fork, 0));
    }
    timed(ctx, "zstd_block_scan", ba, [&] { launch_scan_blocks(b, ba); });
    if (r->n_bt) {
        HIPCHK(ctx, hipMemsetAsync(r->tile_done, 0, r->done_bytes, ba));
        FusedBlocksArgs fb{};
        fb.h = rows_hash_args(ctx, r, run);
        fb.h.pass = 0;
        fb.blob_size = r->blob_size;
        fb.bt_tile = r->bt_tile; fb.bt_item = r->bt_item; fb.n_bt = r->n_bt;
        fb.item_src = r->item_src; fb.row_flag = r->row_flag;
        fb.tile_done = r->tile_done; fb.item_done = r->item_done;
        fb.dbg = ctx->sw.dbg;
        timed(ctx, run.verify ? "verify_blocks" : "decode_verify_fused_blocks", ba, [&] { launch_fused_blocks(fb, ba, run.verify); });
        launch_compact_items(r->item_done, r->n_items, r->todo, r->hand(H_ITEMS), ba);
    }
    DecodeArgs a{};
    fill_row_args(a, r, run);
    a.block_mode = 1;
    a.item_row = r->item_row; a.item_k = r->item_k; a.item_src = r->item_src; a.n_items = r->n_items; a.row_flag = r->row_flag;
    a.item_done = r->n_bt ? r->item_done : nullptr;
    a.todo = r->n_bt ? r->todo : nullptr; a.n_todo = r->hand(H_ITEMS);
    a.pending_count = r->hand(H_FUSED);
    a.compressed = r->compressed;
    a.n_rows = r->n; a.cursor = r->cur(CUR_ITEMS);
    a.lit_scratch = ctx->lit_scratch_b;
    if (ctx->sw.ddbg)
        a.dbg = diag_cycle<8>(ctx, znippy_ctx::DIAG_ITEMS, s, ba, [](const unsigned long long *h) {
            if (h[0]) fprintf(stderr, "[znippy ddbg] block items=%llu  cycles per item: literals=%.0f seq-tables=%.0f seq-decode=%.0f execute=%.0f tail=%.0f\n", h[0],
                              (double)h[1] / h[0], (double)h[2] / h[0], (double)h[3] / h[0], (double)h[4] / h[0], (double)h[5] / h[0]);
        });
    if (!p.lean_blocks) timed(ctx, "zstd_decode_blocks", ba, [&] { launch_decode(a, std::min<int>(ctx->decode_grid, (int)r->n_items), false, ba); });
    if (r->fz_total) run_two_phase(ctx, r, run, ba);
    if (!p.one_stream) HIPCHK(ctx, hipEventRecord(ctx->ev_join, ctx->aux));
    return ZNIPPY_OK;
}

static BxArgs rows_bx_args(znippy_ctx *ctx, const znippy_rows *r, const RunPlan &p, const RowsRun &run) {
    BxArgs x{};
    x.list_a = r->list_a; x.n_list_a = r->n_list_a;
    x.pending = r->pending; x.pending_count = r->hand(H_FUSED);
    if (p.small_off) {
        x.list_a = r->all_rows; x.n_list_a = r->n;
        x.pending_count = r->ctl_at<uint32_t>(CTL_RX, RX_ZERO);
    }
    x.bc_row = r->cand_row; x.n_bc = r->n_cand;
    fill_row_args(x, r, run);
    x.row_flag = r->row_flag;
    x.cand_row = r->bx_cand_row; x.cand_base = r->bx_cand_base; x.cand_nb = r->bx_cand_nb; x.slot_cap = r->bx_slots;
    x.items = r->bx_items; x.prep = r->bx_prep; x.item_cap = r->bx_item_cap;
    x.ctr = r->ctl_at<uint32_t>(CTL_BX_CTR);
    x.huf_list = r->bx_huf_list; x.seq_list = r->bx_seq_list; x.sort_tmp = r->bx_sort_tmp;
    x.lit_pool = ctx->fz_lit_pool; x.lit_cap = ctx->fz_lit_cap; x.seq_pool = ctx->fz_seq_pool; x.seq_cap = ctx->fz_seq_cap;
    x.fse_pool = ctx->bx_fse_pool; x.fse_cap = ctx->bx_fse_cap; x.huf_pool = ctx->bx_huf_pool; x.huf_cap = ctx->bx_huf_cap;
    x.pool_used = r->ctl_at<unsigned long long>(CTL_BX_POOL);
    x.pending2 = r->pending2; x.pending2_count = r->hand(H_SERIAL);
    x.big_seq = ctx->sw.bx_big_set || r->bx_nblk > 32768 ? ctx->sw.bx_big : 0u;
    if (p.rx) {
        x.rx_ptr = ctx->rx_pool; x.rx_cap = ctx->rx_cap; x.rx_chunk = ctx->rx_chunk; x.rx_cdone = ctx->rx_cdone;
        x.rx_base = r->rx_base; x.rx_fail = r->rx_fail; x.rx_blk = r->rx_blk; x.rx_list = r->rx_list;
        x.rx_pending = r->ctl_at<uint32_t>(CTL_RX);
        x.rx_bound = std::min<uint64_t>(r->rx_words, ctx->rx_cap);
        x.rx_min = r->rx_min;
    }
    x.small_frames = r->n_compressed && r->bx_bytes / r->n_compressed <= 65536;
    if (ctx->sw.ddbg)
        x.dbg = diag_cycle<128>(ctx, znippy_ctx::DIAG_BX, ctx->stream, nullptr, [](const unsigned long long *h) {
            if (h[64]) {
                const unsigned long long *e = h + 64;
                fprintf(stderr, "[znippy ddbg] batch execute: frames=%llu groups=%llu seqs=%llu big=%llu rounds=%llu flushes=%llu histreads=%llu | kcycles/frame: total=%.1f records=%.1f rep+scan=%.1f big=%.1f flush=%.1f histread=%.1f lits=%.1f matches=%.1f tail=%.1f\n",
                        e[0], e[1], e[2], e[3], e[4], e[5], e[6], e[8] / 1e3 / e[0], e[9] / 1e3 / e[0], e[10] / 1e3 / e[0], e[11] / 1e3 / e[0], e[12] / 1e3 / e[0], e[13] / 1e3 / e[0],
                        e[14] / 1e3 / e[0], e[15] / 1e3 / e[0], e[16] / 1e3 / e[0]);
            }
            if (h[32]) fprintf(stderr, "[znippy ddbg] batch tables: wave passes=%llu  kcycles per pass: literals header + weights=%.1f sequences header=%.1f huffman table=%.1f sequence tables=%.1f\n", h[32],
                               h[33] / 1e3 / h[32], h[34] / 1e3 / h[32], h[35] / 1e3 / h[32], h[36] / 1e3 / h[32]);
        });
    return x;
}
static void bx_stage(znippy_ctx *ctx, const BxArgs &x, BxStage st, hipStream_t on) {
    static const char *const names[10] = {"zstd_batch_scan", "zstd_batch_tables", "zstd_batch_huffman", "zstd_batch_sequences", "zstd_batch_execute", "zstd_batch_finish",
                                          "zstd_batch_sequences_long", "zstd_batch_sort", "zstd_resolve_plan", "zstd_resolve_expand"};
    timed(ctx, names[st], on, [&] { launch_bx_stage(x, ctx->cus, st, on); });
}
static int run_resolve(znippy_ctx *ctx, znippy_rows *r, const BxArgs &x) {
    hipStream_t s = ctx->stream;
    bx_stage(ctx, x, BX_RX_PLAN, s);
    if (ctx->sw.trace) {
        uint32_t g[16];
        unsigned long long pu[16];
        (void)hipMemcpy(g, r->ctl + CTL_BX_CTR.at, CTL_BX_CTR.bytes, hipMemcpyDeviceToHost);
        (void)hipMemcpy(pu, r->ctl + CTL_BX_POOL.at, CTL_BX_POOL.bytes, hipMemcpyDeviceToHost);
        fprintf(stderr, "[znippy trace] resolve plan: slots %u items %u list %u frames %u words %llu extent %llu cap %llu item_cap %u\n", g[0], g[1], g[9], g[11], pu[10], pu[11],
                (unsigned long long)ctx->rx_cap, r->bx_item_cap);
    }
    HIPCHK(ctx, hipEventRecord(ctx->ev_fork, s));
    HIPCHK(ctx, hipStreamWaitEvent(ctx->aux, ctx->ev_fork, 0));
    bx_stage(ctx, x, BX_EXEC, ctx->aux);
    HIPCHK(ctx, hipEventRecord(ctx->ev_join, ctx->aux));
    bx_stage(ctx, x, BX_RX_EXPAND, s);
    static const char *const jump_names[12] = {"zstd_resolve_jump_0", "zstd_resolve_jump_1", "zstd_resolve_jump_2", "zstd_resolve_jump_3", "zstd_resolve_jump_4", "zstd_resolve_jump_5",
                                               "zstd_resolve_jump_6", "zstd_resolve_jump_7", "zstd_resolve_jump_8", "zstd_resolve_jump_9", "zstd_resolve_jump_10", "zstd_resolve_jump_11"};
    static_assert(zn::RX_ROUNDS <= 12, "names");
    if (!ctx->sw.ddbg) ktime_begin(ctx, "zstd_resolve_jump", s);
    for (int rd = 0; rd < (int)zn::RX_ROUNDS; rd++) {
        if (ctx->sw.ddbg) ktime_begin(ctx, jump_names[rd], s);
        launch_bx_stage(x, ctx->cus, BX_RX_JUMP + rd, s);
        if (ctx->sw.ddbg) ktime_end(ctx, s);
    }
    if (!ctx->sw.ddbg) ktime_end(ctx, s);
    timed(ctx, "zstd_resolve_store", s, [&] { launch_bx_stage(x, ctx->cus, BX_RX_STORE, s); });
    HIPCHK(ctx, hipStreamWaitEvent(s, ctx->ev_join, 0));
    return ZNIPPY_OK;
}
static int run_batch_path(znippy_ctx *ctx, znippy_rows *r, const RunPlan &p, const RowsRun &run) {
    hipStream_t s = ctx->stream;
    const DecodeArgs a = rows_decode_args(ctx, r, run);
    if (r->n_cand) {
        HIPCHK(ctx, hipStreamWaitEvent(s, ctx->ev_join, 0));
        launch_finish_blocks(rows_scan_args(r, run), s, true);
    }
    const BxArgs x = rows_bx_args(ctx, r, p, run);
    bx_stage(ctx, x, BX_SCAN, s);
    bx_stage(ctx, x, BX_PREP, s);
    bx_stage(ctx, x, BX_SORT, s);
    HIPCHK(ctx, hipEventRecord(ctx->ev_fork, s));
    HIPCHK(ctx, hipStreamWaitEvent(ctx->aux, ctx->ev_fork, 0));
    bx_stage(ctx, x, BX_FSE_WAVE, ctx->aux);
    HIPCHK(ctx, hipEventRecord(ctx->ev_join, ctx->aux));
    if (p.third) {
        HIPCHK(ctx, hipStreamWaitEvent(ctx->copy, ctx->ev_fork, 0));
        bx_stage(ctx, x, BX_FSE, ctx->copy);
        HIPCHK(ctx, hipEventRecord(ctx->ev_join2, ctx->copy));
    }
    bx_stage(ctx, x, BX_HUF, s);
    if (!p.third) bx_stage(ctx, x, BX_FSE, s);
    HIPCHK(ctx, hipStreamWaitEvent(s, ctx->ev_join, 0));
    if (p.third) HIPCHK(ctx, hipStreamWaitEvent(s, ctx->ev_join2, 0));
    if (p.rx) { const int rc = run_resolve(ctx, r, x); if (rc) return rc; }
    else bx_stage(ctx, x, BX_EXEC, s);
    bx_stage(ctx, x, BX_FINISH, s);
    decode_rest(ctx, r, a, r->n_compressed);
    return ZNIPPY_OK;
}
static int run_serial_flow(znippy_ctx *ctx, znippy_rows *r, const RunPlan &p, const RowsRun &run) {
    hipStream_t s = ctx->stream;
    const DecodeArgs a = rows_decode_args(ctx, r, run);
    if (p.behind) {
        if (!p.one_stream) HIPCHK(ctx, hipStreamWaitEvent(s, ctx->ev_join, 0));
        launch_finish_blocks(rows_scan_args(r, run), s, false);
    }
    if (p.lean_blocks) return ZNIPPY_OK;
    const int gen_grid = r->n_cand && !p.behind ? ctx->decode_grid / 4 * ctx->gen_share : ctx->decode_grid;
    timed(ctx, "zstd_decode_general", s, [&] { launch_decode(a, std::min<int>(gen_grid, (int)r->n_compressed), r->wide_rows, s); });
    if (!r->n_cand) return ZNIPPY_OK;
    if (!p.behind) {
        HIPCHK(ctx, hipStreamWaitEvent(s, ctx->ev_join, 0));
        launch_finish_blocks(rows_scan_args(r, run), s, false);
    }
    decode_rest(ctx, r, a, r->n_cand);
    return ZNIPPY_OK;
}

static void run_second_hash(znippy_ctx *ctx, znippy_rows *r, const RunPlan &p, const RowsRun &run) {
    hipStream_t s = ctx->stream;
    HashArgs h = rows_hash_args(ctx, r, run);
    h.pass = p.stored_only ? 0 : 2;
    h.tile_done = r->n_bt && !p.stored_only ? r->tile_done : nullptr;
    timed(ctx, run.verify ? "blake3_hash_only" : "blake3_second_pass", s, [&] { launch_hash_tiles(h, s); });
    if (r->plan.n_big)
        timed(ctx, "blake3_merge_big", s, [&] {
            launch_merge_big(r->plan.big, r->plan.n_big, r->plan.tile_cv, r->digests, r->plan.grp_big, r->plan.grp_k, r->plan.n_grp, r->plan.max_cvs, s);
        });
}

static int run_verify(znippy_ctx *ctx, znippy_rows *r, const RunPlan &p, const RowsRun &run) {
    hipStream_t s = ctx->stream;
    if (p.lean_mixed) HIPCHK(ctx, hipStreamWaitEvent(s, ctx->ev_join, 0));
    const bool skipped = p.lean || p.lean_blocks || p.lean_mixed;
    timed(ctx, "verify", s, [&] {
        launch_verify(r->digests, r->checksum, r->usize, r->status, r->n, r->row_begin, r->counters, r->corrupt, r->corrupt_cap, s,
                      skipped ? r->ctl_at<uint32_t>(CTL_HAND) : nullptr, (p.lean || p.lean_mixed) ? LEAN_SMALL : LEAN_BLOCKS);
    });
    HIPCHK(ctx, hipMemcpyAsync(r->h_counters + 16 * run.slot, r->counters, CTL_MIRROR, hipMemcpyDeviceToHost, s));
    HIPCHK(ctx, hipEventRecord(r->ev_done[run.slot], s));
    HIPCHK(ctx, hipGetLastError());
    return ZNIPPY_OK;
}

static int rows_launch(znippy_ctx *ctx, znippy_rows *r, const void *d_blobs, uint64_t blob_base, void *d_out, uint64_t out_cap,
                       unsigned slot, bool verify, bool *queued = nullptr) {
    ctx->n_ktimes = 0;
    int rc = ensure_decoder(ctx);
    if (!rc && verify) {
        rc = rows_verify_slots(ctx, r);
        if (!rc) rc = ensure_verify_scratch(ctx, r->vs_bytes);
        d_out = ctx->vs_pool; out_cap = r->vs_bytes;
    }
    if (!rc) rc = rows_validate(ctx, r, blob_base, out_cap, verify);
    if (!rc && r->fz_total) rc = ensure_fz_pools(ctx, r->fz_bytes, r->fz_total);
    if (!rc && r->bx_slots) {
        rc = ensure_fz_pools(ctx, r->bx_bytes, r->bx_item_cap);
        if (!rc) rc = ensure_bx_pools(ctx, r->bx_bytes, r->bx_item_cap);
        if (!rc && r->rx_base && r->bx_hint != 0) rc = ensure_rx_pool(ctx, r->rx_words);
    }
    if (rc) return rc;
    if (r->n_cand && !ctx->lit_scratch_b && hipMalloc(&ctx->lit_scratch_b, decode_lit_scratch_bytes(ctx->decode_grid)) != hipSuccess) return ZNIPPY_E_NOMEM;
    if (r->run_seq && r->bx_hint < 0 && r->n) {
        const unsigned last = (unsigned)((r->run_seq - 1) & 1);
        if (hipEventQuery(r->ev_done[last]) == hipSuccess) rows_note_hint(r, last);
        else (void)hipGetLastError();
    }
    const RowsRun run{d_blobs, blob_base, d_out, out_cap, r->n_bad ? 1 : 0, slot, verify};
    const RunPlan p = rows_plan(ctx, r, run.preset);
    if (p.small_off && !r->all_rows) {
        if (tmalloc(ctx, &r->all_rows, 4 * (size_t)r->n) != hipSuccess) return ZNIPPY_E_NOMEM;
        hipLaunchKernelGGL(k_iota32, dim3((r->n + 255) / 256), dim3(256), 0, ctx->stream, r->all_rows, r->n);
    }
    { auto &ra = r->run_args[slot]; ra.blobs = d_blobs; ra.base = blob_base; ra.out = verify ? nullptr : d_out; ra.cap = verify ? 0 : out_cap; ra.blob_cap = r->blob_cap; ra.verify = verify; }
    if (queued) *queued = true;
    if ((rc = run_clear(ctx, r, p, run)) || !r->n) return rc;
    if (!p.small_off && !p.stored_only && (rc = run_small_rows(ctx, r, p, run))) return rc;
    if (p.decode && r->n_cand && (rc = run_block_items(ctx, r, p, run))) return rc;
    if (p.decode && r->n_compressed && (rc = p.bx ? run_batch_path(ctx, r, p, run) : run_serial_flow(ctx, r, p, run))) return rc;
    if (!p.lean) run_second_hash(ctx, r, p, run);
    return run_verify(ctx, r, p, run);
}

static void rows_abandon(znippy_ctx *ctx, znippy_rows *r);
static int rows_queue(znippy_ctx *ctx, znippy_rows *r, const void *d_blobs, uint64_t blob_base, void *d_out, uint64_t out_cap, bool verify) {
    HIPCHK(ctx, hipSetDevice(ctx->device));
    bool queued = false;
    const int rc = rows_launch(ctx, r, d_blobs, blob_base, d_out, out_cap, (unsigned)(r->run_seq & 1), verify, &queued);
    if (rc && queued) rows_abandon(ctx, r);
    if (rc) return rc;
    r->run_seq++;
    return ZNIPPY_OK;
}
static void rows_abandon(znippy_ctx *ctx, znippy_rows *r) {
    if (hipEventRecord(ctx->ev_join, ctx->aux) == hipSuccess) (void)hipStreamWaitEvent(ctx->stream, ctx->ev_join, 0);
    (void)hipStreamSynchronize(ctx->stream);
    (void)hipGetLastError();
    r->run_seq = 0;
    r->force_full = true;
    r->lean_hint = 0; r->lean_hint2 = 0;
}

int znippy_decode_verify_rows_async(znippy_ctx *ctx, znippy_rows *r, const void *d_blobs,
                                    uint64_t blob_base, void *d_out, uint64_t out_cap) {
    if (ctx && ctx->closing) return ZNIPPY_E_INVAL;
    if (!ctx || !r || r->ctx != ctx) return ZNIPPY_E_INVAL;
    if (r->no_out) return ZNIPPY_E_INVAL;
    if (r->n && (!d_blobs || !d_out)) return ZNIPPY_E_INVAL;
    return rows_queue(ctx, r, d_blobs, blob_base, d_out, out_cap, false);
}

int znippy_verify_rows_async(znippy_ctx *ctx, znippy_rows *r, const void *d_blobs, uint64_t blob_base) {
    if (ctx && ctx->closing) return ZNIPPY_E_INVAL;
    if (!ctx || !r || r->ctx != ctx) return ZNIPPY_E_INVAL;
    if (r->n && !d_blobs) return ZNIPPY_E_INVAL;
    return rows_queue(ctx, r, d_blobs, blob_base, nullptr, 0, true);
}

int znippy_rows_verify_scratch(znippy_ctx *ctx, znippy_rows *r, const void **d_base, uint64_t *bytes, uint64_t *row_offset) {
    if (ctx && ctx->closing) return ZNIPPY_E_INVAL;
    if (!ctx || !r || r->ctx != ctx || !d_base || !bytes) return ZNIPPY_E_INVAL;
    HIPCHK(ctx, hipSetDevice(ctx->device));
    int rc = rows_verify_slots(ctx, r);
    if (!rc) rc = ensure_verify_scratch(ctx, r->vs_bytes);
    if (rc) return rc;
    *d_base = r->vs_bytes ? ctx->vs_pool : nullptr;
    *bytes = r->vs_bytes;
    if (row_offset && r->n) {
        std::vector<uint8_t> comp(r->n);
        std::vector<uint64_t> len(r->n);
        HIPCHK(ctx, hipStreamSynchronize(ctx->stream));
        HIPCHK(ctx, hipMemcpy(row_offset, r->vs_off, 8 * (size_t)r->n, hipMemcpyDeviceToHost));
        HIPCHK(ctx, hipMemcpy(comp.data(), r->compressed, r->n, hipMemcpyDeviceToHost));
        HIPCHK(ctx, hipMemcpy(len.data(), r->usize, 8 * (size_t)r->n, hipMemcpyDeviceToHost));
        for (uint32_t i = 0; i < r->n; i++)
            if (!comp[i] || !len[i]) row_offset[i] = ~0ull;
    }
    return ZNIPPY_OK;
}

static int rows_settle(znippy_ctx *ctx, znippy_rows *r, unsigned slot) {
    if (!r->n || !r->run_seq || !(r->h_counters[16 * slot + 7])) return ZNIPPY_OK;
    HIPCHK(ctx, hipSetDevice(ctx->device));
    HIPCHK(ctx, hipStreamSynchronize(ctx->stream));
    r->force_full = true;
    r->lean_hint = 0; r->lean_hint2 = 0;
    const unsigned latest = (unsigned)((r->run_seq - 1) & 1);
    const unsigned order[2] = {slot, latest};
    for (int i = 0; i < (slot == latest ? 1 : 2); i++) {
        const znippy_rows::RunArgs ra = r->run_args[order[i]];
        r->blob_cap = ra.blob_cap;
        bool queued = false;
        const int rc = rows_launch(ctx, r, ra.blobs, ra.base, ra.out, ra.cap, order[i], ra.verify, &queued);
        if (rc) {
            if (queued) rows_abandon(ctx, r);
            return rc;
        }
    }
    HIPCHK(ctx, hipStreamSynchronize(ctx->stream));
    return ZNIPPY_OK;
}

int znippy_rows_results_lagged(znippy_ctx *ctx, znippy_rows *r, unsigned lag, znippy_verify_counters *counters) {
    if (ctx && ctx->closing) return ZNIPPY_E_INVAL;
    if (!ctx || !r || r->ctx != ctx || !counters || lag > 1 || r->run_seq <= lag) return ZNIPPY_E_INVAL;
    uint64_t c[8] = {0};
    if (r->n) {
        const unsigned slot = (unsigned)((r->run_seq - 1 - lag) & 1);
        HIPCHK(ctx, hipEventSynchronize(r->ev_done[slot]));
        { const int rc = rows_settle(ctx, r, slot); if (rc) return rc; }
        memcpy(c, r->h_counters + 16 * slot, 64);
        rows_note_hint(r, slot);
    }
    counters->total_chunks = c[0]; counters->total_written_bytes = c[1]; counters->verified_bytes = c[2];
    counters->corrupt_bytes = c[3]; counters->corrupt_rows = c[4]; counters->decode_errors = c[5];
    return ZNIPPY_OK;
}

int znippy_rows_results(znippy_ctx *ctx, znippy_rows *r, znippy_verify_counters *counters,
                        uint64_t *corrupt_rows, uint64_t corrupt_cap, int32_t *row_status) {
    if (ctx && ctx->closing) return ZNIPPY_E_INVAL;
    if (!ctx || !r) return ZNIPPY_E_INVAL;
    HIPCHK(ctx, hipSetDevice(ctx->device));
    HIPCHK(ctx, hipStreamSynchronize(ctx->stream));
    uint64_t c[8] = {0};
    if (r->n && r->run_seq) {
        { const int rc = rows_settle(ctx, r, (unsigned)((r->run_seq - 1) & 1)); if (rc) return rc; }
        memcpy(c, r->h_counters + 16 * ((r->run_seq - 1) & 1), 64);
        rows_note_hint(r, (unsigned)((r->run_seq - 1) & 1));
    }
    if (counters) {
        counters->total_chunks = c[0]; counters->total_written_bytes = c[1]; counters->verified_bytes = c[2];
        counters->corrupt_bytes = c[3]; counters->corrupt_rows = c[4]; counters->decode_errors = c[5];
    }
    if (corrupt_rows && corrupt_cap && c[4]) {
        uint64_t k = std::min<uint64_t>(c[4], r->corrupt_cap);
        std::vector<uint64_t> tmp(k);
        HIPCHK(ctx, hipMemcpy(tmp.data(), r->corrupt, 8 * k, hipMemcpyDeviceToHost));
        std::sort(tmp.begin(), tmp.end());
        memcpy(corrupt_rows, tmp.data(), 8 * std::min<uint64_t>(k, corrupt_cap));
    }
    if (row_status && r->n) {
        HIPCHK(ctx, hipMemcpy(row_status, r->status, 4 * (size_t)r->n, hipMemcpyDeviceToHost));
        for (uint32_t i = 0; i < r->n; i++)
            if (row_status[i] > 0) row_status[i] = 0;
    }
    return ZNIPPY_OK;
}

int znippy_decode_verify_rows(znippy_ctx *ctx, znippy_rows *rows, const void *d_blobs,
                              uint64_t blob_base, void *d_out, uint64_t out_cap,
                              znippy_verify_counters *counters, uint64_t *corrupt_rows,
                              uint64_t corrupt_cap, int32_t *row_status) {
    if (ctx && ctx->closing) return ZNIPPY_E_INVAL;
    int rc = znippy_decode_verify_rows_async(ctx, rows, d_blobs, blob_base, d_out, out_cap);
    if (rc) return rc;
    return znippy_rows_results(ctx, rows, counters, corrupt_rows, corrupt_cap, row_status);
}

int znippy_verify_rows(znippy_ctx *ctx, znippy_rows *rows, const void *d_blobs, uint64_t blob_base,
                       znippy_verify_counters *counters, uint64_t *corrupt_rows, uint64_t corrupt_cap, int32_t *row_status) {
    if (ctx && ctx->closing) return ZNIPPY_E_INVAL;
    int rc = znippy_verify_rows_async(ctx, rows, d_blobs, blob_base);
    if (rc) return rc;
    return znippy_rows_results(ctx, rows, counters, corrupt_rows, corrupt_cap, row_status);
}

int znippy_rows_digests(znippy_ctx *ctx, znippy_rows *r, uint8_t *digests) {
    if (ctx && ctx->closing) return ZNIPPY_E_INVAL;
    if (!ctx || !r || !digests) return ZNIPPY_E_INVAL;
    HIPCHK(ctx, hipSetDevice(ctx->device));
    HIPCHK(ctx, hipStreamSynchronize(ctx->stream));
    if (r->n && r->run_seq) { const int rc = rows_settle(ctx, r, (unsigned)((r->run_seq - 1) & 1)); if (rc) return rc; }
    if (r->n) HIPCHK(ctx, hipMemcpy(digests, r->digests, 32 * (size_t)r->n, hipMemcpyDeviceToHost));
    return ZNIPPY_OK;
}

static void rounds_select(znippy_rounds *r, unsigned slot) {
    const size_t n = r->n;
    r->res = r->res_m[slot];
    r->h_res = r->h_res_m[slot];
    r->total = reinterpret_cast<uint64_t *>(r->res);
    r->overflow = reinterpret_cast<uint32_t *>(r->res + 8);
    r->blob_offset = reinterpret_cast<uint64_t *>(r->res + 16);
    r->blob_size = r->blob_offset + n;
    r->digests = reinterpret_cast<uint32_t *>(r->res + 16 + n * 16);
}

void znippy_rounds_destroy(znippy_rounds *r) {
    if (!r) return;
    (void)hipSetDevice(r->ctx->device);
    if (r->ctx->copy) (void)hipStreamSynchronize(r->ctx->copy);
    for (int k = 0; k < 2; k++) {
        pinned_give(r->ctx, r->h_res_m[k], r->h_res_cap_m[k]);
        event_give(r->ctx, r->ev_enc[k]);
        event_give(r->ctx, r->ev_res[k]);
    }
    void *ptrs[] = {r->src_off, r->len, r->skip, r->res_m[0], r->res_m[1], r->items, r->piece_len, r->piece_len_init,
                    r->piece_start, r->local_excl, r->block_tot, r->first_item, r->stored, r->order_small, r->order_wide, r->retry_list, r->retry_count,
                    r->plan_scratch[0], r->plan_scratch[1], r->plan_scratch[2], r->d_ldm, r->d_ldm_desc};
    pinned_give(r->ctx, r->h_stored, r->h_stored_cap);
    for (void *p : ptrs)
        tfree(r->ctx, p);
    free_plan(r->ctx, r->plan);
    znippy_ctx *const c = r->ctx;
    delete r;
    table_released(c);
}

int znippy_rounds_create(znippy_ctx *ctx, const uint64_t *src_offset, const uint64_t *len,
                         const uint8_t *skip, uint64_t n, znippy_rounds **out) {
    if (ctx && ctx->closing) return ZNIPPY_E_INVAL;
    if (!ctx || !out || (n && (!src_offset || !len)) || n >= 0xFFFFFFF0ull) return ZNIPPY_E_INVAL;
    HIPCHK(ctx, hipSetDevice(ctx->device));
    TDbg td(ctx->sw.tdbg, "rounds_create");
    std::unique_ptr<znippy_rounds, void (*)(znippy_rounds *)> guard(new znippy_rounds(), znippy_rounds_destroy);
    znippy_rounds *const r = guard.get();
    r->ctx = ctx;
    ctx->live_tables++;
    r->n = (uint32_t)n;
    if (skip) r->h_skip.assign(skip, skip + n);
    uint64_t tot[8];
    zn_rounds_totals(len, skip, n, tot);
    r->blob_bound = tot[4]; r->in_bytes = tot[5]; r->enc_bytes = tot[6];
    r->all_stored_aligned = n > 0 && r->enc_bytes == 0 && !tot[7];
    if (tot[0] >= 0xFFFFFFF0ull) return ZNIPPY_E_INVAL;
    r->n_items = (uint32_t)tot[0]; r->prov_bytes = tot[1]; r->n_small = (uint32_t)tot[2]; r->n_wide = (uint32_t)tot[3];
    td.mark("totals");
    int rc;
    if ((rc = dev_upload(ctx, &r->src_off, src_offset, n)) || (rc = dev_upload(ctx, &r->len, len, n)) ||
        (skip ? (rc = dev_upload(ctx, &r->skip, skip, n)) : (tmalloc(ctx, &r->skip, std::max<size_t>(n, 16)) != hipSuccess ? (rc = ZNIPPY_E_NOMEM) : 0)))
        return rc;
    if (!skip && n) HIPCHK(ctx, hipMemsetAsync(r->skip, 0, n, ctx->stream));
    td.mark("columns_h2d");
    r->res_bytes = 16 + (size_t)n * (8 + 8 + 32);
    for (int k = 0; k < 2; k++)
        if (tmalloc(ctx, &r->res_m[k], r->res_bytes) != hipSuccess ||
            !(r->h_res_m[k] = (uint8_t *)pinned_take(ctx, r->res_bytes, &r->h_res_cap_m[k])) ||
            !(r->ev_enc[k] = event_take(ctx)) || !(r->ev_res[k] = event_take(ctx)))
            return ZNIPPY_E_NOMEM;
    rounds_select(r, 0);
    td.mark("slabs");
    PlanBuf p;
    build_plan([&](uint32_t u) { return len[u]; }, (uint32_t)n, p);
    if ((rc = upload_plan(ctx, p, r->plan))) return rc;
    if (r->n_items == n && r->n_wide == 0 && r->enc_bytes == r->in_bytes && n) {
        uint32_t max_units = 0;
        for (const Tile &t : p.tiles) max_units = std::max(max_units, t.n_units);
        r->fuse_tiles = 1;
        if (const char *e = getenv("ZNIPPY_FUSE_TILES")) { const int v = atoi(e); if (v >= 1 && v * (int)max_units <= 64) r->fuse_tiles = v; }
    }
    td.mark("hash_plan");
    if (r->n_items > n) {
        for (uint64_t i = 0; i < n; i++)
            if (len[i] > BLOCK_BYTES && len[i] < (1ull << 32) && !(skip && skip[i])) {
                const uint32_t lg = ldm_log2(len[i]);
                r->h_ldm.push_back(LdmRound{(uint32_t)i, r->ldm_chunks, r->ldm_entries | ((uint64_t)lg << 48)});
                r->ldm_entries += 1ull << lg;
                r->ldm_chunks += (uint32_t)((len[i] + LDM_CHUNK - 1) / LDM_CHUNK);
            }
    }
    const size_t ni = std::max<size_t>(r->n_items, 1), nsb = (ni + 255) / 256;
    RoundSums *sums = nullptr;
    const uint32_t nblk = ((uint32_t)n + 1023) / 1024;
    if (tmalloc(ctx, &r->first_item, std::max<size_t>(4 * (size_t)n, 16)) != hipSuccess || tmalloc(ctx, &sums, std::max<size_t>(sizeof(RoundSums) * (size_t)nblk, 64)) != hipSuccess ||
        tmalloc(ctx, &r->order_small, std::max<size_t>(4 * (size_t)r->n_small, 16)) != hipSuccess ||
        tmalloc(ctx, &r->order_wide, std::max<size_t>(4 * (size_t)r->n_wide, 16)) != hipSuccess ||
        tmalloc(ctx, &r->retry_list, std::max<size_t>(4 * (size_t)r->n_small, 16)) != hipSuccess || tmalloc(ctx, &r->retry_count, 64) != hipSuccess ||
        tmalloc(ctx, &r->stored, std::max<size_t>(n, 16)) != hipSuccess ||
        !(r->h_stored = (uint8_t *)pinned_take(ctx, std::max<size_t>(n, 16), &r->h_stored_cap)) ||
        tmalloc(ctx, &r->items, sizeof(EncItem) * ni) != hipSuccess || tmalloc(ctx, &r->piece_len_init, 4 * ni) != hipSuccess ||
        tmalloc(ctx, &r->piece_len, 4 * ni) != hipSuccess || tmalloc(ctx, &r->piece_start, 8 * ni) != hipSuccess ||
        tmalloc(ctx, &r->local_excl, 8 * ni) != hipSuccess || tmalloc(ctx, &r->block_tot, 8 * nsb) != hipSuccess) {
        tfree(ctx, sums);
        return ZNIPPY_E_NOMEM;
    }
    if (n) {
        const uint8_t *const d_skip = skip ? r->skip : (const uint8_t *)nullptr;
        hipLaunchKernelGGL(k_rounds_sums, dim3(nblk), dim3(256), 0, ctx->stream, r->len, d_skip, (uint32_t)n, sums);
        hipLaunchKernelGGL(k_rounds_scan, dim3(1), dim3(256), 0, ctx->stream, sums, nblk);
        hipLaunchKernelGGL(k_rounds_fill, dim3(nblk), dim3(256), 0, ctx->stream, r->len, d_skip, (uint32_t)n, sums, r->first_item, r->items, r->piece_len_init,
                           r->order_small, r->order_wide);
    }
    r->plan_scratch[0] = sums;
    td.mark("encoder_plan");
    if (r->n_items) HIPCHK(ctx, hipMemcpyAsync(r->piece_len, r->piece_len_init, 4 * (size_t)r->n_items, hipMemcpyDeviceToDevice, ctx->stream));
    td.mark("rest");
    *out = guard.release();
    return ZNIPPY_OK;
}

uint64_t znippy_rounds_blob_bound(const znippy_rounds *r) { return r ? r->blob_bound : 0; }

static int hash_rounds_async(znippy_ctx *ctx, znippy_rounds *r, const void *d_src, hipStream_t on = nullptr,
                             void *d_copy_out = nullptr, uint64_t copy_cap = 0) {
    hipStream_t s = on ? on : ctx->stream;
    HashArgs h{};
    h.tiles = r->plan.tiles; h.n_tiles = r->plan.n_tiles;
    h.len = r->len;
    h.srcA = (const uint8_t *)d_src; h.offA = r->src_off; h.baseA = 0;
    h.digests = r->digests; h.tile_cv = r->plan.tile_cv;
    if (d_copy_out) {
        h.srcB = (uint8_t *)d_copy_out; h.offB = r->blob_offset; h.copy_to_B = 1;
        h.store_tiles = ctx->sw.store_g;
        h.copy_mask = r->skip; h.copy_cap = copy_cap;
        h.misaligned_dst = !(r->all_stored_aligned && ((uintptr_t)d_copy_out & 15) == 0);
    }
    if (on && r->enc_bytes * 4 >= r->in_bytes) h.fold_tiles_max = 1;
    ktime_begin(ctx, "blake3_tiles", s);
    launch_hash_tiles(h, s);
    ktime_end(ctx, s);
    if (r->plan.n_big) {
        ktime_begin(ctx, "blake3_merge_big", s);
        launch_merge_big(r->plan.big, r->plan.n_big, r->plan.tile_cv, r->digests, r->plan.grp_big, r->plan.grp_k, r->plan.n_grp, on ? 0xFFFFFFFFu : r->plan.max_cvs, s);
        ktime_end(ctx, s);
    }
    HIPCHK(ctx, hipGetLastError());
    return ZNIPPY_OK;
}

int znippy_hash_rounds(znippy_ctx *ctx, znippy_rounds *r, const void *d_src, uint8_t *digests) {
    if (ctx && ctx->closing) return ZNIPPY_E_INVAL;
    if (!ctx || !r || r->ctx != ctx || !digests || (r->n && !d_src)) return ZNIPPY_E_INVAL;
    HIPCHK(ctx, hipSetDevice(ctx->device));
    ctx->n_ktimes = 0;
    int rc = hash_rounds_async(ctx, r, d_src);
    if (rc) return rc;
    HIPCHK(ctx, hipStreamSynchronize(ctx->stream));
    if (r->n) HIPCHK(ctx, hipMemcpy(digests, r->digests, 32 * (size_t)r->n, hipMemcpyDeviceToHost));
    return ZNIPPY_OK;
}

static int shim_reserve(znippy_ctx *ctx, size_t in_need, size_t out_need) {
    if (in_need > ctx->shim_in_cap || !ctx->shim_in) {
        if (ctx->shim_in) (void)hipFree(ctx->shim_in);
        ctx->shim_in = nullptr; ctx->shim_in_cap = 0;
        size_t cap = std::max<size_t>(in_need + 64, 1 << 16);
        HIPCHK(ctx, hipMalloc(&ctx->shim_in, cap));
        ctx->shim_in_cap = cap;
    }
    if (out_need > ctx->shim_out_cap || !ctx->shim_out) {
        if (ctx->shim_out) (void)hipFree(ctx->shim_out);
        ctx->shim_out = nullptr; ctx->shim_out_cap = 0;
// ... 317 lines not shown
```

### znippy_amd/csrc/common.h

```cpp
#pragma once
#include <hip/hip_runtime.h>
#include <stdint.h>
#include <stddef.h>

namespace zn {

struct Tile {
    uint32_t first_unit;
    uint32_t n_units;
    uint32_t first_leaf;
    uint32_t n_leaves;
    uint32_t cv_index;
    uint32_t pad;
};

struct BigUnit {
    uint32_t unit;
    uint32_t cv_base;
    uint32_t n_cvs;
    uint32_t pad;
};

struct HashArgs {
    const Tile *tiles;
    uint32_t n_tiles;
    const uint64_t *len;
    const uint8_t *srcA;
    const uint64_t *offA;
    uint64_t baseA;
    uint8_t *srcB;
    const uint64_t *offB;
    const uint8_t *sel;
    const int32_t *status;
    const uint32_t *pending_count;
    int pass;
    int copy_to_B;
    uint32_t *digests;
    uint32_t *tile_cv;
    int store_tiles;
    int fold_tiles_max;
    const uint8_t *tile_done;
    const uint8_t *copy_mask;
    uint64_t copy_cap;
    int misaligned_dst;
};

struct DecodeArgs {
    const uint32_t *list_a;
    uint32_t n_list_a;
    const uint32_t *pending;
    const uint32_t *pending_count;
    const uint8_t *blobs;
    uint64_t blob_base;
    const uint64_t *blob_off, *blob_size, *usize, *out_off;
    const uint8_t *compressed;
    uint8_t *out;
    uint64_t out_cap;
    int32_t *status;
    uint32_t n_rows;
    uint32_t *cursor;
    uint8_t *lit_scratch;
    unsigned long long *dbg;
    int block_mode;
    const uint32_t *item_row, *item_k;
    const uint32_t *item_src;
    uint32_t n_items;
    uint32_t *row_flag;
    const uint8_t *item_done;
    const uint32_t *todo, *n_todo;
    uint32_t *seq_scratch;
    int preset;
};

struct FusedArgs {
    HashArgs h;
    const uint64_t *blob_size;
    uint64_t out_cap;
    int32_t *status;
    uint32_t *pending;
    uint32_t *pending_count;
    int dbg;
    unsigned long long *dbg_buf;
    uint32_t lds_pad;
    int preset;
    uint32_t *cursor;
    uint32_t *tile_list;
    uint32_t *tile_count;
};

struct FusedBlocksArgs {
    HashArgs h;
    const uint64_t *blob_size;
    const uint32_t *bt_tile, *bt_item;
    uint32_t n_bt;
    const uint32_t *item_src;
    const uint32_t *row_flag;
    uint8_t *tile_done, *item_done;
    int dbg;
};
void launch_fused_blocks(const FusedBlocksArgs &a, hipStream_t s, bool verify = false);

void launch_hash_tiles(const HashArgs &a, hipStream_t s);
void launch_fused_small(const FusedArgs &a, hipStream_t s, int grid_cap = 0, bool verify = false);
void launch_fused_roles(const FusedArgs &a, int cus, hipStream_t s, bool verify = false);
void init_fused_tables();
void launch_merge_big(const BigUnit *big, uint32_t n_big, uint32_t *tile_cv, uint32_t *digests, const uint32_t *grp_big,
                      const uint32_t *grp_k, uint32_t n_grp, uint32_t max_cvs, hipStream_t s);
void launch_verify(const uint32_t *digests, const uint8_t *checksum, const uint64_t *usize,
                   const int32_t *status, uint32_t n_rows, uint64_t row_begin, uint64_t *counters,
                   uint64_t *corrupt_rows, uint32_t corrupt_cap, hipStream_t s, const uint32_t *lean_lists = nullptr, uint32_t lean_mask = 0);
int decode_grid_size(int device);
void launch_decode(const DecodeArgs &a, int grid, bool wide, hipStream_t s);
struct BlockScanArgs {
    const uint32_t *cand_row, *cand_base, *cand_nblocks;
    uint32_t n_cand;
    const uint8_t *blobs;
    uint64_t blob_base;
    const uint64_t *blob_off, *blob_size, *usize, *out_off;
    uint64_t out_cap;
    uint32_t *item_src;
    uint32_t *row_flag;
    int32_t *status;
    uint32_t *pending, *pending_count;
    int preset;
};
void launch_scan_blocks(const BlockScanArgs &a, hipStream_t s);
void launch_compact_items(const uint8_t *item_done, uint32_t n_items, uint32_t *todo, uint32_t *n_todo, hipStream_t s);
void launch_finish_blocks(const BlockScanArgs &a, hipStream_t s, bool defer_flagged);

struct FzItem {
    uint32_t src;
    uint32_t out;
    uint32_t nseq;
    uint32_t lit_len;
    uint64_t seq_off;
    uint64_t lit_off;
    uint32_t lit_kind;
    int32_t err;
    uint32_t rep[3];
    uint32_t pad;
};
constexpr uint32_t FZ_SYM = 1u << 28;
struct FzArgs {
    const uint32_t *cand_row, *cand_fzbase, *cand_fzcap;
    uint32_t n_cand;
    const uint32_t *it_cand;
    uint32_t total_items;
    uint32_t *cand_nb;
    FzItem *items;
    const uint8_t *blobs;
    uint64_t blob_base;
    const uint64_t *blob_off, *blob_size, *usize, *out_off;
    uint64_t out_cap;
    uint8_t *out;
    uint32_t *row_flag;
    const int32_t *status;
    int preset;
    uint8_t *lit_pool;
    uint64_t lit_cap;
    unsigned long long *seq_pool;
    uint64_t seq_cap;
    unsigned long long *pool_used;
    uint32_t *cursor;
    unsigned long long *dbg;
};
void launch_fz_scan(const FzArgs &a, uint32_t *work, uint32_t *work_count, hipStream_t s);
void launch_fz_entropy(const FzArgs &a, int cus, const uint32_t *work, const uint32_t *work_count, hipStream_t s);
void launch_fz_exec(const FzArgs &a, hipStream_t s);

struct BxPrep {
    uint32_t frame;
    uint32_t k;
    uint32_t n_streams;
    uint32_t huf_off;
    uint32_t huf_log;
    uint32_t st_off[4];
    uint32_t st_len[4];
    uint32_t tab[3];
    uint32_t logs;
    uint32_t bs_off;
    uint32_t bs_len;
};
constexpr uint32_t BX_BIG_SEQ = 2048;
constexpr uint32_t BX_PREDEF_LL = 0, BX_PREDEF_OF = 64, BX_PREDEF_ML = 96, BX_POOL_FIRST = 160;
struct BxArgs {
    const uint32_t *list_a; uint32_t n_list_a;
    const uint32_t *pending; const uint32_t *pending_count;
    const uint32_t *bc_row; uint32_t n_bc;
    const uint8_t *blobs; uint64_t blob_base;
    const uint64_t *blob_off, *blob_size, *usize, *out_off;
    uint64_t out_cap;
    uint8_t *out;
    int32_t *status;
    int preset;
    uint32_t *row_flag;
    uint32_t *cand_row, *cand_base, *cand_nb;
    uint32_t slot_cap;
    FzItem *items; BxPrep *prep; uint32_t item_cap;
    uint32_t *ctr;
    uint32_t *sort_tmp;
    uint32_t *huf_list, *seq_list;
    uint8_t *lit_pool; uint64_t lit_cap;
    unsigned long long *seq_pool; uint64_t seq_cap;
    uint16_t *fse_pool; uint64_t fse_cap;
    uint16_t *huf_pool; uint64_t huf_cap;
    unsigned long long *pool_used;
    uint32_t *pending2, *pending2_count;
    unsigned long long *dbg;
    int small_frames;
    uint32_t big_seq;
    uint32_t *rx_ptr; uint64_t rx_cap;
    uint32_t *rx_chunk;
    uint8_t *rx_cdone;
    uint32_t *rx_base, *rx_fail;
    uint32_t *rx_blk;
    uint32_t *rx_list;
    uint32_t *rx_pending;
    uint64_t rx_bound;
    uint32_t rx_min;
};
constexpr uint32_t RX_NONE = 0xFFFFFFFFu, RX_DONE = 0x80000000u, RX_MIN = 256u << 10, RX_ROUNDS = 12, RX_JUMPS = 6;
enum BxStage : int { BX_SCAN = 0, BX_PREP = 1, BX_HUF = 2, BX_FSE = 3, BX_EXEC = 4, BX_FINISH = 5, BX_FSE_WAVE = 6, BX_SORT = 7, BX_RX_PLAN = 8, BX_RX_EXPAND = 9,
                     BX_RX_JUMP = 10 , BX_RX_STORE = 30 };
void launch_bx_stage(const BxArgs &a, int cus, int stage, hipStream_t s);
void bx_predefined_tables(uint16_t cells[160]);

}
```

### znippy_amd/csrc/fused_small.hip

```cpp
#include "common.h"
#include "hash_dev.h"

#include <algorithm>
#include <cstring>

namespace zn {

constexpr uint32_t EOFF_MAX = 960;
constexpr uint32_t EBUF = EOFF_MAX + 1024 + 64;
constexpr int F_E_CORRUPT = -5, F_E_UNSUP = -6, F_E_DST = -4;
constexpr int F_NOT_SIMPLE = 1;

struct DTab {
    uint16_t next;
    uint8_t nbits, addbits;
    uint32_t base;
};
__constant__ DTab c_dll[64], c_dml[64], c_dof[32];
__constant__ uint32_t c_llb[36] = {0, 1, 2, 3, 4, 5, 6, 7, 8, 9, 10, 11, 12, 13, 14, 15, 16, 18,
                                   20, 22, 24, 28, 32, 40, 48, 64, 128, 256, 512, 1024, 2048,
                                   4096, 8192, 16384, 32768, 65536};
__constant__ uint8_t c_lla[36] = {0, 0, 0, 0, 0, 0, 0, 0, 0, 0, 0, 0, 0, 0, 0, 0, 1, 1,
                                  1, 1, 2, 2, 3, 3, 4, 6, 7, 8, 9, 10, 11, 12, 13, 14, 15, 16};
__constant__ uint32_t c_mlb[53] = {3, 4, 5, 6, 7, 8, 9, 10, 11, 12, 13, 14, 15, 16, 17, 18, 19, 20,
// ... 696 lines not shown
            if (p3) *reinterpret_cast<uint4 *>(d + 3072) = v3;
            x += 4096;
            i0 += 256;
            if (i0 >= body16) open_ = 0;
        }
        return true;
    }
    __device__ __forceinline__ void drain() {
        if (g_abl & 16) return;
        while (step_one()) {}
    }
};
struct BlockFold {
    uint32_t *nodes;
    uint32_t *tab_n, *tab_off, *tab_out;
};
constexpr uint32_t FOLD_UNITS = 16;

template <bool STORE>
__device__ __forceinline__ void fused_tile(const FusedArgs &a, const uint32_t wave, const BlockFold &bf) {
    __shared__ __attribute__((aligned(16))) uint8_t s_W[4][WROWS * WSTRIDE];
    const uint32_t lane = threadIdx.x & 63;
    const Tile t = a.h.tiles[wave];
    if (t.n_units == 0) return;
    static_assert(EBUF <= 64 * 8 * 4, "pattern buffer must fit the wave's node slice");
    uint8_t *const E = reinterpret_cast<uint8_t *>(bf.nodes + (size_t)(threadIdx.x >> 6) * 64 * 8);
    uint8_t *const WL = s_W[threadIdx.x >> 6];
    const bool stamp = (a.dbg & 8) && a.dbg_buf;
    __shared__ unsigned long long s_acc[4][8];
    if (lane < 8) s_acc[threadIdx.x >> 6][lane] = 0;
    unsigned long long t0 = 0, t1 = 0, t2 = 0, t3 = 0;
    if (stamp) t0 = __builtin_amdgcn_s_memtime();

    uint32_t c_sel = 0, c_bs = 0;
    uint64_t c_len = 0, c_src = 0, c_oo = 0;
    int32_t c_st = 0;
    if (lane < t.n_units) {
        const uint32_t row = t.first_unit + lane;
        if (a.preset) c_st = a.status[row];
        c_sel = a.h.sel[row];
        c_len = a.h.len[row];
        c_src = a.h.offA[row] - a.h.baseA;
        c_oo = a.h.offB[row];
        c_bs = (uint32_t)a.blob_size[row];
    }
    __shared__ uint16_t s_desc[4][3][WROWS];
    uint16_t *const d_y = s_desc[threadIdx.x >> 6][0], *const d_B = s_desc[threadIdx.x >> 6][1],
                   *const d_off = s_desc[threadIdx.x >> 6][2];
    __shared__ int32_t s_st[4][64];
    int32_t *const l_st = s_st[threadIdx.x >> 6];
    if (lane < WROWS) d_y[lane] = 0xFFFF;
    l_st[lane] = c_st;
    uint32_t need_reread = 0;

    uint64_t done64 = 0;
    if (t.n_units > WROWS && !(a.dbg & (2 | 128))) {
        FastTabs T;
        {
            const DTab eL = c_dll[lane], eM = c_dml[lane], eO = c_dof[lane & 31];
            T.ll = eL.base | (uint32_t)eL.addbits << 24;
            T.ml = eM.base | (uint32_t)eM.addbits << 24;
            T.of = eO.addbits;
            T.lls = lane < 36 ? c_llb[lane] | (uint32_t)c_lla[lane] << 24 : 0u;
            T.mls = lane < 53 ? c_mlb[lane] | (uint32_t)c_mla[lane] << 24 : 0u;
        }
#pragma unroll 1
        for (uint32_t g0 = WROWS; g0 < t.n_units; g0 += WROWS) {
#pragma unroll 1
            for (uint32_t u = 0; u < WROWS && g0 + u < t.n_units; u++) {
                const uint64_t so = ((uint64_t)__shfl((uint32_t)(c_src >> 32), g0 + u) << 32) | __shfl((uint32_t)c_src, g0 + u);
                const uint32_t n = __shfl(c_bs, g0 + u), o = 8 * lane;
                const uint8_t *p = a.h.srcA + so + o;
                uint64_t v = 0;
                if (__shfl(c_sel, g0 + u) && __shfl(c_st, g0 + u) == 0) {
                    if (o + 8 <= n) __builtin_memcpy(&v, p, 8);
                    else
                        for (uint32_t k = 0; k < 8; k++)
                            if (o + k < n) v |= (uint64_t)p[k] << (8 * k);
                }
                *reinterpret_cast<uint64_t *>(WL + u * WSTRIDE + 8 * lane) = v;
                if (lane < (WSTRIDE - WIN) / 4) *reinterpret_cast<uint32_t *>(WL + u * WSTRIDE + WIN + 4 * lane) = 0;
            }
            const uint32_t gl = g0 + lane < 64 ? g0 + lane : 63;
            const uint32_t g_sel = __shfl(c_sel, gl), g_bs = __shfl(c_bs, gl);
            const uint64_t g_len = ((uint64_t)__shfl((uint32_t)(c_len >> 32), gl) << 32) | __shfl((uint32_t)c_len, gl);
            const uint64_t g_oo = ((uint64_t)__shfl((uint32_t)(c_oo >> 32), gl) << 32) | __shfl((uint32_t)c_oo, gl);
            const bool want = lane < WROWS && g0 + lane < t.n_units && g_sel && g_oo + g_len <= a.out_cap && __shfl(c_st, gl) == 0;
            const FastRow f = parse_fast(WL + (lane < WROWS ? lane : 0) * WSTRIDE, g_bs, g_len, want, T);
            const uint32_t m = (uint32_t)__ballot(f.ok != 0);
            if (m) {
                Emitter e2;
                e2.WL = WL; e2.outbase = a.h.srcB; e2.lane = lane;
                e2.f_lit = f.lit_at; e2.f_L0 = f.L0; e2.f_off = f.off; e2.c_len_lo = (uint32_t)g_len; e2.c_oo = g_oo;
                e2.prepare(m);
                e2.drain();
                done64 |= (uint64_t)m << g0;
                need_reread = 1;
            }
        }
    }

    if (!(a.dbg & 2)) {
        const uint32_t nw = t.n_units < WROWS ? t.n_units : WROWS;
        uint2 wv[WROWS];
#pragma unroll
        for (uint32_t u = 0; u < WROWS; u++) {
            wv[u] = make_uint2(0, 0);
            if (u < nw) {
                const uint64_t so = __shfl(c_src, u);
                const uint32_t n = __shfl(c_bs, u), o = 8 * lane;
                const uint8_t *p = a.h.srcA + so + o;
                if (__shfl(c_sel, u) && __shfl(c_st, u) == 0) {
                    if (o + 8 <= n) __builtin_memcpy(&wv[u], p, 8);
                    else {
                        uint64_t v = 0;
                        for (uint32_t k = 0; k < 8; k++)
                            if (o + k < n) v |= (uint64_t)p[k] << (8 * k);
                        wv[u] = make_uint2((uint32_t)v, (uint32_t)(v >> 32));
                    }
                }
            }
        }
#pragma unroll
        for (uint32_t u = 0; u < WROWS; u++) {
            if (u < nw) {
                *reinterpret_cast<uint2 *>(WL + u * WSTRIDE + 8 * lane) = wv[u];
                if (lane < (WSTRIDE - WIN) / 4) *reinterpret_cast<uint32_t *>(WL + u * WSTRIDE + WIN + 4 * lane) = 0;
            }
        }
    }

    FastRow fr{0, 0, 0, 0};
    if (!(a.dbg & (2 | 128))) {
        FastTabs T;
        {
            const DTab eL = c_dll[lane], eM = c_dml[lane], eO = c_dof[lane & 31];
            T.ll = eL.base | (uint32_t)eL.addbits << 24;
            T.ml = eM.base | (uint32_t)eM.addbits << 24;
            T.of = eO.addbits;
            T.lls = lane < 36 ? c_llb[lane] | (uint32_t)c_lla[lane] << 24 : 0u;
            T.mls = lane < 53 ? c_mlb[lane] | (uint32_t)c_mla[lane] << 24 : 0u;
        }
        const bool want = lane < t.n_units && lane < WROWS && c_sel && c_oo + c_len <= a.out_cap && c_st == 0;
        fr = parse_fast(WL + (lane < WROWS ? lane : 0) * WSTRIDE, c_bs, c_len, want, T);
        const bool ho = !fr.ok && not_simple_fast(WL + (lane < WROWS ? lane : 0) * WSTRIDE, c_bs, c_len, want);
        const uint64_t hom = __ballot(ho);
        if (hom) {
            uint32_t at = 0;
            if (lane == 0) at = atomicAdd(a.pending_count, (uint32_t)__popcll(hom));
            at = (uint32_t)__builtin_amdgcn_readlane((int)at, 0);
            if (ho) {
                const uint32_t row = t.first_unit + lane;
                a.status[row] = F_NOT_SIMPLE;
                l_st[lane] = F_NOT_SIMPLE;
                a.pending[at + (uint32_t)__popcll(hom & ((1ull << lane) - 1ull))] = row;
            }
            done64 |= hom;
        }
    }
    const uint32_t fmask = (uint32_t)__ballot(fr.ok != 0);
    Emitter em;
    em.WL = WL; em.outbase = a.h.srcB; em.lane = lane;
    em.f_lit = fr.lit_at; em.f_L0 = fr.L0; em.f_off = fr.off; em.c_len_lo = (uint32_t)c_len; em.c_oo = c_oo;
    em.prepare(fmask);
    if (fr.ok && !(a.dbg & 4)) {
        d_y[lane] = (uint16_t)(lane * WSTRIDE + fr.lit_at);
        d_B[lane] = (uint16_t)(fr.L0 - fr.off);
        d_off[lane] = (uint16_t)fr.off;
    }
    const bool early = __ballot(lane < t.n_units && (c_len == 0 || ((uint32_t)c_len & 1023) != 0)) != 0ull || (a.dbg & (1 | 4));
    if (early && fmask && (STORE || (a.dbg & 4))) { em.drain(); need_reread = 1; }
    if (stamp) { asm volatile("s_waitcnt vmcnt(0) lgkmcnt(0)" ::: "memory"); t1 = __builtin_amdgcn_s_memtime(); }
    if (!(a.dbg & 64)) __builtin_amdgcn_s_setprio(3);
    for (uint32_t u = 0; u < t.n_units && !(a.dbg & 2); u++) {
        const uint32_t row = t.first_unit + u;
        if (!uni(__shfl(c_sel, u))) continue;
        if ((int32_t)uni((uint32_t)__shfl(c_st, u)) < 0) continue;
        const uint64_t usize = ((uint64_t)uni((uint32_t)(__shfl(c_len, u) >> 32)) << 32) | uni((uint32_t)__shfl(c_len, u));
        const uint64_t ooff = ((uint64_t)uni((uint32_t)(__shfl(c_oo, u) >> 32)) << 32) | uni((uint32_t)__shfl(c_oo, u));
        const uint64_t soff = ((uint64_t)uni((uint32_t)(__shfl(c_src, u) >> 32)) << 32) | uni((uint32_t)__shfl(c_src, u));
        const uint32_t bsz = uni(__shfl(c_bs, u));
        if ((u < 32 && (fmask >> u & 1)) || (done64 >> u & 1)) continue;
        int rc;
        Periodic per;
        per.ok = 0;
        if (ooff + usize > a.out_cap) rc = F_E_DST;
        else rc = decode_simple(a.h.srcA + soff, bsz, a.h.srcB + ooff, usize, E, u < WROWS ? WL + u * WSTRIDE : nullptr, &per,
                                stamp ? s_acc[threadIdx.x >> 6] : nullptr);
        rc = (int)uni((uint32_t)rc);
        const bool periodic = rc == 0 && uni(per.ok) && u < WROWS && !(a.dbg & 4);
        if (periodic) {
            if (lane == 0) {
                d_y[u] = (uint16_t)(u * WSTRIDE + per.lit_at);
                d_B[u] = (uint16_t)(per.L0 - per.off);
                d_off[u] = (uint16_t)per.off;
            }
        } else if (rc == 0) {
            need_reread = 1;
        }
        if (rc != 0 && lane == 0) {
            a.status[row] = rc;
            l_st[u] = rc;
            if (rc == F_NOT_SIMPLE) a.pending[atomicAdd(a.pending_count, 1u)] = row;
        }
    }
    __builtin_amdgcn_s_setprio(0);
    if (need_reread) fwave_mem_sync();
    if (stamp) t2 = __builtin_amdgcn_s_memtime();
    if (!(a.dbg & 1)) {
        LdsSrc ls{WL, d_y, d_B, d_off, WROWS, l_st, c_len, c_src, c_oo, c_sel, (!STORE || early || (g_abl & 16)) ? 0u : fmask};
        LeafOut lo;
        hash_tile_leaves<STORE, true>(a.h, t, &ls, lo);
        if (t.n_units <= FOLD_UNITS && !(a.dbg & 256)) {
            const uint32_t w = threadIdx.x >> 6;
            if (lo.active) {
                uint4 *d = reinterpret_cast<uint4 *>(bf.nodes + (size_t)(w * 64 + lane) * 8);
                d[0] = make_uint4(lo.cv[0], lo.cv[1], lo.cv[2], lo.cv[3]);
                d[1] = make_uint4(lo.cv[4], lo.cv[5], lo.cv[6], lo.cv[7]);
            }
            const uint32_t act = __shfl(lo.active ? 1u : 0u, lo.u_head & 63);
            if (lane < t.n_units) {
                bf.tab_n[w * FOLD_UNITS + lane] = act ? lo.u_cnt : 0u;
                bf.tab_off[w * FOLD_UNITS + lane] = w * 64 + lo.u_head;
                bf.tab_out[w * FOLD_UNITS + lane] = t.first_unit + lane;
            }
        } else {
            fold_tile_now(a.h, t, lo);
        }
    }
    if (stamp) {
        t3 = __builtin_amdgcn_s_memtime();
        if (lane == 0) {
            atomicAdd(&a.dbg_buf[0], t1 - t0);
            atomicAdd(&a.dbg_buf[1], t2 - t1);
            atomicAdd(&a.dbg_buf[2], t3 - t2);
            atomicAdd(&a.dbg_buf[3], 1ull);
            for (int q = 4; q < 8; q++) atomicAdd(&a.dbg_buf[q], s_acc[threadIdx.x >> 6][q]);
        }
    }
}

__device__ __forceinline__ void lds_barrier() {
    asm volatile("s_waitcnt lgkmcnt(0)\n\ts_barrier" ::: "memory");
}

template <bool STORE>
__global__ __launch_bounds__(256, 5) void k_fused_small(FusedArgs a) {
    __shared__ __attribute__((aligned(16))) uint32_t s_nodes[4 * 64 * 8];
    __shared__ uint32_t s_tab[3][4 * FOLD_UNITS];
    const uint32_t lane = threadIdx.x & 63, w = threadIdx.x >> 6;
    const bool clk = (a.dbg & 32768) && a.dbg_buf && blockIdx.x == 2000 && threadIdx.x == 0;
    const unsigned long long c0 = clk ? __builtin_amdgcn_s_memtime() : 0, r0 = clk ? __builtin_amdgcn_s_memrealtime() : 0;
    const BlockFold bf{s_nodes, s_tab[0], s_tab[1], s_tab[2]};
    const uint32_t n_work = a.tile_list ? *a.tile_count : a.h.n_tiles;
    for (uint32_t base = blockIdx.x * 4, it = 0; base < n_work; base += gridDim.x * 4, it++) {
        if (lane < FOLD_UNITS) bf.tab_n[w * FOLD_UNITS + lane] = 0;
        const uint32_t idx = base + w;
        if (idx < n_work) fused_tile<STORE>(a, a.tile_list ? a.tile_list[idx] : idx, bf);
        lds_barrier();
        if (w == ((blockIdx.x + it) * 2654435761u) >> 30) {
            FoldQueue<4> fq;
            fq.n_tab = 4 * FOLD_UNITS;
            fq.tb_n = bf.tab_n[lane];
            fq.tb_off = bf.tab_off[lane];
            fq.tb_out = bf.tab_out[lane];
            fq.tb_root = 1;
            if (__ballot(fq.tb_n != 0) != 0ull) {
                FoldQueue<4> fd = fq.dense16();
                uint32_t U = 0;
                const uint32_t n = (a.dbg & 262144) ? 0u : fd.uniform(&U);
                if (n) fd.fold_uniform_and_write(s_nodes, a.h, n, U);
                else fq.fold_and_write(s_nodes, a.h);
            }
        }
        if (base + gridDim.x * 4 < n_work) lds_barrier();
    }
    if (clk) { a.dbg_buf[0] = __builtin_amdgcn_s_memtime() - c0; a.dbg_buf[1] = __builtin_amdgcn_s_memrealtime() - r0; }
}

#ifndef ZN_R_SLOTS
#define ZN_R_SLOTS 32
#endif
#ifndef ZN_R_WAVES
#define ZN_R_WAVES 16
#endif
#ifndef ZN_R_LOADERS
#define ZN_R_LOADERS 1
#endif
#ifndef ZN_R_LOADER_EMITS
#define ZN_R_LOADER_EMITS 0
#endif
constexpr uint32_t R_SLOTS = ZN_R_SLOTS, R_GROUP = 4, R_WAVES = ZN_R_WAVES, R_LOADERS = ZN_R_LOADERS;
constexpr bool R_LOADER_EMITS = ZN_R_LOADER_EMITS != 0;
static_assert((R_SLOTS & (R_SLOTS - 1)) == 0 && R_SLOTS >= 2 * R_GROUP, "ring size: a power of two, at least two groups");
constexpr uint32_t R_SLOT_BYTES = WROWS * WSTRIDE;
constexpr uint32_t R_SLOT_NODES = R_SLOT_BYTES / 32;
static_assert(R_SLOT_BYTES % 32 == 0 && R_SLOT_BYTES >= 64 * 32, "a slot must hold 64 chaining values, node-aligned");

typedef __attribute__((address_space(3))) uint32_t lds_u32;
__device__ __forceinline__ uint32_t lds_ld(const uint32_t *p) { return __builtin_amdgcn_readfirstlane(*(const volatile lds_u32 *)p); }
__device__ __forceinline__ void lds_st(uint32_t *p, uint32_t v) { *(volatile lds_u32 *)p = v; }
__device__ __forceinline__ void lds_fence() { asm volatile("s_waitcnt lgkmcnt(0)" ::: "memory"); }

struct alignas(16) RolesShared {
    uint8_t slots[R_SLOTS][R_SLOT_BYTES];
    __attribute__((aligned(16))) uint32_t tree[R_WAVES - R_LOADERS][64 * 8];
    uint64_t oo[R_SLOTS][WROWS];
    uint32_t len[R_SLOTS][WROWS];
    uint32_t tn[R_SLOTS][WROWS], toff[R_SLOTS][WROWS];
    uint16_t dy[R_SLOTS][WROWS], dB[R_SLOTS][WROWS], doff[R_SLOTS][WROWS];
    uint32_t first[R_SLOTS], nunits[R_SLOTS], nleaves[R_SLOTS];
    uint32_t ready, take, finished;
    uint32_t next_iter;
    uint32_t cnt[R_SLOTS / R_GROUP];
    uint32_t gen[R_SLOTS / R_GROUP];
};

__device__ __forceinline__ void emit_periodic_row(uint8_t *Y, uint32_t L0, uint32_t off, float inv, uint8_t *out, uint32_t osize,
                                                  uint32_t lane) {
    const uint32_t B = L0 - off, lim = L0 + 64;
    Y[L0 + lane] = Y[B + lmod(lane, off, inv)];
    const uint32_t head = (uint32_t)((16 - ((uintptr_t)out & 15)) & 15);
    const uint32_t body16 = (osize - head) >> 4;
    const uint32_t step = smod(1024, off), rb = smod(B, off);
    if (lane < head) out[lane] = Y[lane];
    const uint32_t tail = (osize - head) & 15, p = head + 16 * body16 + lane;
    if (lane < tail) {
        uint32_t rt = lmod(p, off, inv) + off - rb;
        if (rt >= off) rt -= off;
        out[p] = p < lim ? Y[p] : Y[B + rt];
    }
    uint32_t x = head + 16 * lane;
    uint32_t r = lmod(x, off, inv) + off - rb;
    if (r >= off) r -= off;
    for (uint32_t i0 = 0; i0 < body16; i0 += 256) {
        const uint32_t i = i0 + lane;
        uint4 v0 = make_uint4(0, 0, 0, 0), v1 = v0, v2 = v0, v3 = v0;
        const uint32_t r0 = r;
        uint32_t r1 = r0 + step; if (r1 >= off) r1 -= off;
        uint32_t r2 = r1 + step; if (r2 >= off) r2 -= off;
        uint32_t r3 = r2 + step; if (r3 >= off) r3 -= off;
        r = r3 + step; if (r >= off) r -= off;
        const bool p0 = i < body16, p1 = i + 64 < body16, p2 = i + 128 < body16, p3 = i + 192 < body16;
        if (p0) v0 = lds16(x + 16 <= lim ? Y + x : Y + B + r0);
        if (p1) v1 = lds16(Y + B + r1);
        if (p2) v2 = lds16(Y + B + r2);
        if (p3) v3 = lds16(Y + B + r3);
        uint8_t *d = out + x;
        if (p0) *reinterpret_cast<uint4 *>(d) = v0;
        if (p1) *reinterpret_cast<uint4 *>(d + 1024) = v1;
        if (p2) *reinterpret_cast<uint4 *>(d + 2048) = v2;
        if (p3) *reinterpret_cast<uint4 *>(d + 3072) = v3;
        x += 4096;
    }
}

template <bool STORE>
__device__ __forceinline__ void roles_loader(const FusedArgs &a, RolesShared &S) {
    const uint32_t lane = threadIdx.x & 63, j = lane >> 4, u = lane & 15;
    FastTabs T;
    {
        const DTab eL = c_dll[lane], eM = c_dml[lane], eO = c_dof[lane & 31];
        T.ll = eL.base | (uint32_t)eL.addbits << 24;
        T.ml = eM.base | (uint32_t)eM.addbits << 24;
        T.of = eO.addbits;
        T.lls = lane < 36 ? c_llb[lane] | (uint32_t)c_lla[lane] << 24 : 0u;
        T.mls = lane < 53 ? c_mlb[lane] | (uint32_t)c_mla[lane] << 24 : 0u;
    }
    for (;;) {
        const uint32_t iter = uni(atomicAdd(&S.next_iter, lane == 0 ? 1u : 0u));
        const uint32_t base = uni(atomicAdd(a.cursor, lane == 0 ? R_GROUP : 0u));
        const bool last = base >= a.h.n_tiles;
        const uint32_t grp = iter & (R_SLOTS / R_GROUP - 1), use = iter / (R_SLOTS / R_GROUP);
        const uint32_t ti = base + j;
        Tile t{0, 0, 0, 0, 0, 0};
        if (ti < a.h.n_tiles) t = a.h.tiles[ti];
        const bool small = t.n_units >= 1;
        const bool cand = small && t.n_units <= WROWS;
        const bool rowv = cand && u < t.n_units;
        uint32_t c_sel = 0, c_bs = 0;
        uint64_t c_len = 0, c_src = 0, c_oo = 0;
        int32_t c_st = 0;
        if (rowv) {
            const uint32_t row = t.first_unit + u;
            if (a.preset) c_st = a.status[row];
            c_sel = a.h.sel[row];
            c_len = a.h.len[row];
            c_src = a.h.offA[row] - a.h.baseA;
            if (STORE) c_oo = a.h.offB[row];
            const uint64_t bs = a.blob_size[row];
            c_bs = bs > 0xFFFFFFFFull ? 0xFFFFFFFFu : (uint32_t)bs;
        }
        const bool want = rowv && c_sel && c_st == 0 && c_len != 0 && (c_len & 1023) == 0 && c_len <= 0x10000 &&
                          (!STORE || c_oo + c_len <= a.out_cap) && c_bs >= 12 && c_bs <= WIN;
        while (lds_ld(&S.gen[grp]) != use) __builtin_amdgcn_s_sleep(4);
        asm volatile("" ::: "memory");
        const uint32_t slot = grp * R_GROUP + j;
        uint8_t *const win = S.slots[slot] + (u < WROWS ? u : 0) * WSTRIDE;
        const uint8_t *const src = a.h.srcA + c_src;
        const uint32_t nb = want ? c_bs : 0, full = nb >> 4, tail = nb & 15;
        for (uint32_t i = 0; __ballot(i < full) != 0ull; i++)
            if (i < full) {
                const uint4 v = ld16(src + 16 * i);
                *reinterpret_cast<uint4 *>(win + 16 * i) = v;
            }
        if (tail) {
            uint32_t w4[4] = {0, 0, 0, 0};
            for (uint32_t k = 0; k < tail; k++) w4[k >> 2] |= (uint32_t)src[16 * full + k] << (8 * (k & 3));
            *reinterpret_cast<uint4 *>(win + 16 * full) = make_uint4(w4[0], w4[1], w4[2], w4[3]);
        }
        const FastRow fr = parse_fast(win, c_bs, c_len, want, T);
        const uint64_t badm = __ballot(rowv && !fr.ok);
        const bool fast = cand && ((badm >> (16 * j)) & 0xFFFFull) == 0;
        if (small && !fast && u == 0) a.tile_list[atomicAdd(a.tile_count, 1u)] = ti;
        if (u == 0) {
            S.first[slot] = t.first_unit;
            S.nunits[slot] = fast ? t.n_units : 0u;
            S.nleaves[slot] = t.n_leaves;
        }
        const bool mine = fast && rowv;
        if (mine) {
            S.len[slot][u] = (uint32_t)c_len;
            if (STORE) S.oo[slot][u] = c_oo;
            S.dy[slot][u] = (uint16_t)(u * WSTRIDE + fr.lit_at);
            S.dB[slot][u] = (uint16_t)(fr.L0 - fr.off);
            S.doff[slot][u] = (uint16_t)fr.off;
        }
        lds_fence();
        if (R_LOADER_EMITS && STORE) {
            const float inv_l = 1.0f / (float)(mine ? fr.off : 1u);
            for (uint64_t m = __ballot(mine); m && !(a.dbg & 16); m &= m - 1) {
                const uint32_t l = (uint32_t)__builtin_ctzll(m);
                const uint32_t sl = grp * R_GROUP + (l >> 4);
                const uint32_t lit_at = __builtin_amdgcn_readlane(fr.lit_at, l), L0 = __builtin_amdgcn_readlane(fr.L0, l),
                               off = __builtin_amdgcn_readlane(fr.off, l), osize = __builtin_amdgcn_readlane((uint32_t)c_len, l);
                const float inv = __uint_as_float(__builtin_amdgcn_readlane(__float_as_uint(inv_l), l));
                const uint64_t oo = ((uint64_t)__builtin_amdgcn_readlane((uint32_t)(c_oo >> 32), l) << 32) |
                                    __builtin_amdgcn_readlane((uint32_t)c_oo, l);
                emit_periodic_row(S.slots[sl] + (l & 15) * WSTRIDE + lit_at, L0, off, inv, a.h.srcB + oo, osize, lane);
            }
            lds_fence();
        }
        while (lds_ld(&S.ready) != iter * R_GROUP) __builtin_amdgcn_s_sleep(2);
        if (lane == 0) lds_st(&S.ready, (iter + 1) * R_GROUP);
        if (last) break;
    }
    lds_fence();
    atomicAdd(&S.finished, lane == 0 ? 1u : 0u);
}

__device__ __forceinline__ bool tree_op_6x10(uint32_t n, uint32_t &l, uint32_t &r, bool &root) {
    root = false;
    if (n < 30) { const uint32_t row = n / 5, j = n - 5 * row; l = row * 10 + 2 * j; r = l + 1; return true; }
    if (n >= 32 && n < 44) { const uint32_t m = n - 32, row = m >> 1, j = m & 1; l = row * 10 + 4 * j; r = l + 2; return true; }
    if (n >= 44 && n < 50) { l = (n - 44) * 10; r = l + 4; return true; }
    if (n >= 52 && n < 58) { l = (n - 52) * 10; r = l + 8; root = true; return true; }
    l = r = 0;
    return false;
}

template <bool STORE>
__device__ __forceinline__ void roles_hash_6x10(const FusedArgs &a, RolesShared &S, uint32_t slot, uint32_t *tree, bool have_prev,
                                                   uint32_t prev_first, uint32_t cv[8]) {
    typedef __attribute__((address_space(3))) uint8_t lds8b;
    const uint32_t lane = threadIdx.x & 63;
    const bool leaf = lane < 60;
    const uint32_t row = leaf ? lane / 10 : 0, kk = leaf ? lane - 10 * row : 0, ps = lane & 3;
    const lds8b *const Y = leaf ? (const lds8b *)(S.slots[slot] + S.dy[slot][row]) : (const lds8b *)tree;
    const uint32_t yB = S.dB[slot][row], yoff = S.doff[slot][row];
    const uint32_t yL0 = leaf ? yB + yoff : 0xFFFFFFFFu;
    uint32_t p = leaf ? kk << 10 : 64 * ps, step = leaf ? 64u : 256u, gap = 0;
    const uint32_t p1 = (kk << 10) > yB + yoff ? (kk << 10) : (((yB + yoff) >> 6) + 1) << 6;
    uint32_t r = (p1 - yB) % yoff;
    const uint32_t step64 = 64 % yoff;
    uint8_t *const dst = STORE ? a.h.srcB + S.oo[slot][row] + (kk << 10) : nullptr;
    uint32_t *const dig = a.h.digests + (size_t)(prev_first + ps) * 8;
    const uint32_t vmask = (leaf || !have_prev) ? 0u : (ps < 2 ? 0x7FFFu : 0x7FFFu & ~((1u << 7) | (1u << 12) | (1u << 14)));
    const bool store = STORE && leaf && !(a.dbg & 16);
    b3::set_iv(cv);
    uint4 n0, n1, n2, n3;
    uint32_t wq = 0, wq_next = 0;
    auto fetch = [&]() {
        uint32_t q = p;
        if (p > yL0) {
            q = yB + r;
            r += step64;
            if (r >= yoff) r -= yoff;
        }
        const lds_u4 *q3 = (const lds_u4 *)(Y + q), *q4 = (const lds_u4 *)(Y + q + 32 + gap);
        const u4v a0 = q3[0], a1 = q3[1], a2 = q4[0], a3 = q4[1];
        n0 = make_uint4(a0.x, a0.y, a0.z, a0.w); n1 = make_uint4(a1.x, a1.y, a1.z, a1.w);
        n2 = make_uint4(a2.x, a2.y, a2.z, a2.w); n3 = make_uint4(a3.x, a3.y, a3.z, a3.w);
        wq_next = q;
        p += step;
    };
    fetch();
#pragma unroll 1
    for (uint32_t b = 0; b < 16; b++) {
        uint32_t m[16] = {n0.x, n0.y, n0.z, n0.w, n1.x, n1.y, n1.z, n1.w, n2.x, n2.y, n2.z, n2.w, n3.x, n3.y, n3.z, n3.w};
        wq = wq_next;
        if (b < 15) {
            if (b == 7 || b == 10 || b == 12) {
                if (!leaf) {
                    if (b == 7) { p = 320 * (ps >> 1) + 128 * (ps & 1); step = 640; gap = 32; }
                    else if (b == 10) { p = 320 * ps; step = 1280; gap = 96; }
                    else { p = 320 * ps; gap = 224; }
                }
            }
            fetch();
        }
        if (store) {
            uint8_t *d = dst + b * 64;
            st16(d, make_uint4(m[0], m[1], m[2], m[3]));
            st16(d + 16, make_uint4(m[4], m[5], m[6], m[7]));
            st16(d + 32, make_uint4(m[8], m[9], m[10], m[11]));
            st16(d + 48, make_uint4(m[12], m[13], m[14], m[15]));
        }
        const uint32_t fl = (b == 0 ? b3::CHUNK_START : 0u) | (b == 15 ? b3::CHUNK_END : 0u);
        const uint32_t fp = b3::PARENT | (b >= 13 ? b3::ROOT : 0u);
        if (!leaf) b3::set_iv(cv);
        b3::compress(cv, m, kk, 0, 64, leaf ? fl : fp);
        if ((vmask >> b) & 1u) {
            if (b >= 13) {
                uint4 *o = reinterpret_cast<uint4 *>(dig + (b - 13) * 32);
                o[0] = make_uint4(cv[0], cv[1], cv[2], cv[3]);
                o[1] = make_uint4(cv[4], cv[5], cv[6], cv[7]);
            } else {
                lds_u4a *o = (lds_u4a *)(Y + wq);
                o[0] = u4v{cv[0], cv[1], cv[2], cv[3]};
                o[1] = u4v{cv[4], cv[5], cv[6], cv[7]};
            }
        }
    }
}

__device__ __forceinline__ void roles_flush_tree_6x10(const FusedArgs &a, uint32_t *tree, uint32_t prev_first) {
    const uint32_t lane = threadIdx.x & 63;
#pragma unroll 1
    for (uint32_t lv = 0; lv < 4; lv++) {
        const uint32_t base = lv == 0 ? 0u : (lv == 1 ? 32u : (lv == 2 ? 44u : 52u));
        const uint32_t cntl = lv == 0 ? 30u : (lv == 1 ? 12u : 6u);
        uint32_t l = 0, rr = 0;
        bool root = false;
        const bool on = lane < cntl && tree_op_6x10(base + lane, l, rr, root);
        uint32_t cv[8], L[8], R[8];
        const lds_u4a *pl = (const lds_u4a *)(tree + l * 8), *pr = (const lds_u4a *)(tree + rr * 8);
        const u4v l0 = pl[0], l1 = pl[1], r0 = pr[0], r1 = pr[1];
        L[0] = l0.x; L[1] = l0.y; L[2] = l0.z; L[3] = l0.w; L[4] = l1.x; L[5] = l1.y; L[6] = l1.z; L[7] = l1.w;
        R[0] = r0.x; R[1] = r0.y; R[2] = r0.z; R[3] = r0.w; R[4] = r1.x; R[5] = r1.y; R[6] = r1.z; R[7] = r1.w;
        b3::parent(cv, L, R, root);
        __builtin_amdgcn_wave_barrier();
        if (on) {
            if (root) {
                uint4 *o = reinterpret_cast<uint4 *>(a.h.digests + (size_t)(prev_first + l / 10) * 8);
                o[0] = make_uint4(cv[0], cv[1], cv[2], cv[3]);
                o[1] = make_uint4(cv[4], cv[5], cv[6], cv[7]);
            } else {
                lds_u4a *o = (lds_u4a *)(tree + l * 8);
                o[0] = u4v{cv[0], cv[1], cv[2], cv[3]};
                o[1] = u4v{cv[4], cv[5], cv[6], cv[7]};
            }
        }
        __builtin_amdgcn_wave_barrier();
    }
}

template <bool STORE>
__device__ __forceinline__ void roles_hasher(const FusedArgs &a, RolesShared &S) {
    const uint32_t lane = threadIdx.x & 63;
    HashArgs h = a.h;
    h.pass = PASS_ALL;
    uint32_t *const tree = S.tree[(threadIdx.x >> 6) - R_LOADERS];
    bool have_prev = false;
    uint32_t prev_first = 0;
    const bool inline_tree = !(a.dbg & 524288);
    for (;;) {
        const uint32_t take = uni(atomicAdd(&S.take, lane == 0 ? 1u : 0u));
        bool go = false;
        for (;;) {
            const uint32_t f = lds_ld(&S.finished);
            if (lds_ld(&S.ready) > take) { go = true; break; }
            if (f == R_LOADERS) break;
            __builtin_amdgcn_s_sleep(2);
        }
        if (!go) {
            if (have_prev) roles_flush_tree_6x10(a, tree, prev_first);
            return;
        }
        asm volatile("" ::: "memory");
        const uint32_t slot = take & (R_SLOTS - 1), grp = slot / R_GROUP;
        const uint32_t nu = lds_ld(&S.nunits[slot]);
        if (nu) {
            const Tile t{lds_ld(&S.first[slot]), nu, 0, lds_ld(&S.nleaves[slot]), 0, 0};
            const uint32_t lu = lane < nu ? lane : 0;
            if (!R_LOADER_EMITS) {
                uint8_t bytes[WROWS];
#pragma unroll
                for (uint32_t q = 0; q < WROWS; q++) {
                    bytes[q] = 0;
                    if (q < nu) {
                        const uint32_t off = S.doff[slot][q];
                        bytes[q] = S.slots[slot][S.dy[slot][q] + S.dB[slot][q] + lmod(lane, off, 1.0f / (float)off)];
                    }
                }
#pragma unroll
                for (uint32_t q = 0; q < WROWS; q++)
                    if (q < nu) S.slots[slot][S.dy[slot][q] + S.dB[slot][q] + S.doff[slot][q] + lane] = bytes[q];
            }
            const bool shape610 = inline_tree && !R_LOADER_EMITS && nu == 6 && t.n_leaves == 60 && !(a.dbg & 8192) &&
                                  __ballot(lane < 6 && S.len[slot][lu] != 10240u) == 0ull;
            if (shape610) {
                uint32_t cv[8];
                roles_hash_6x10<STORE>(a, S, slot, tree, have_prev, prev_first, cv);
                if (lane < 60) {
                    lds_u4a *o = (lds_u4a *)(tree + lane * 8);
                    o[0] = u4v{cv[0], cv[1], cv[2], cv[3]};
                    o[1] = u4v{cv[4], cv[5], cv[6], cv[7]};
                }
                have_prev = true;
                prev_first = t.first_unit;
                if (lane < WROWS) S.tn[slot][lane] = 0u;
            } else {
            LdsSrc ls{S.slots[slot], S.dy[slot], S.dB[slot], S.doff[slot], WROWS, nullptr,
                      lane < nu ? (uint64_t)S.len[slot][lu] : 0ull, 0ull, STORE ? S.oo[slot][lu] : 0ull, 1u,
                      (R_LOADER_EMITS || !STORE || (a.dbg & 16)) ? 0u : 0x3Fu, 0ull};
            LeafOut lo;
            if (a.dbg & 8192) {
                lo.active = false; lo.u_cnt = 0; lo.u_head = 0;
#pragma unroll
                for (int q = 0; q < 8; q++) lo.cv[q] = 0;
            } else
                hash_tile_leaves<STORE && !R_LOADER_EMITS, true>(h, t, &ls, lo);
            if (lo.active) {
                uint4 *d = reinterpret_cast<uint4 *>(S.slots[slot] + lane * 32);
                d[0] = make_uint4(lo.cv[0], lo.cv[1], lo.cv[2], lo.cv[3]);
                d[1] = make_uint4(lo.cv[4], lo.cv[5], lo.cv[6], lo.cv[7]);
            }
            const uint32_t act = __shfl(lo.active ? 1u : 0u, lo.u_head & 63);
            if (lane < WROWS) {
                S.tn[slot][lane] = (lane < nu && act) ? lo.u_cnt : 0u;
                S.toff[slot][lane] = (slot % R_GROUP) * R_SLOT_NODES + lo.u_head;
            }
            }
        } else if (lane < WROWS) {
            S.tn[slot][lane] = 0u;
        }
        lds_fence();
        const uint32_t old = uni(atomicAdd(&S.cnt[grp], lane == 0 ? 1u : 0u));
        if (old == R_GROUP - 1) {
            asm volatile("" ::: "memory");
            const uint32_t jj = lane >> 4, uu = lane & 15, sl = grp * R_GROUP + jj;
            FoldQueue<4> fq;
            fq.n_tab = 64;
            fq.tb_n = uu < WROWS ? S.tn[sl][uu] : 0u;
            fq.tb_off = uu < WROWS ? S.toff[sl][uu] : 0u;
            fq.tb_out = S.first[sl] + uu;
            fq.tb_root = 1;
            if (__ballot(fq.tb_n != 0) != 0ull && !(a.dbg & 131072)) {
                uint32_t *const nodes = reinterpret_cast<uint32_t *>(S.slots[grp * R_GROUP]);
                FoldQueue<4> fd = fq.dense16();
                uint32_t U = 0;
                const uint32_t n = (a.dbg & 262144) ? 0u : fd.uniform(&U);
                if (n) fd.fold_uniform_and_write(nodes, h, n, U);
                else fq.fold_and_write(nodes, h);
            }
            lds_fence();
            if (lane == 0) {
                lds_st(&S.cnt[grp], 0u);
                lds_st(&S.gen[grp], lds_ld(&S.gen[grp]) + 1u);
            }
        }
    }
}

template <bool STORE>
__global__ __launch_bounds__(R_WAVES * 64) void k_fused_roles(FusedArgs a) {
    extern __shared__ __attribute__((aligned(16))) uint8_t s_roles_raw[];
    RolesShared &S = *reinterpret_cast<RolesShared *>(s_roles_raw);
    if (threadIdx.x == 0) { S.ready = 0; S.take = 0; S.finished = 0; S.next_iter = 0; }
    if (threadIdx.x < R_SLOTS / R_GROUP) { S.cnt[threadIdx.x] = 0; S.gen[threadIdx.x] = 0; }
    __syncthreads();
    const bool clk = (a.dbg & 32768) && a.dbg_buf && blockIdx.x == 7 && threadIdx.x == 64 * R_LOADERS;
    const unsigned long long c0 = clk ? __builtin_amdgcn_s_memtime() : 0, r0 = clk ? __builtin_amdgcn_s_memrealtime() : 0;
    if (threadIdx.x < 64 * R_LOADERS) {
        if (!(a.dbg & 64)) __builtin_amdgcn_s_setprio(3);
        roles_loader<STORE>(a, S);
    } else roles_hasher<STORE>(a, S);
    if (clk) { a.dbg_buf[0] = __builtin_amdgcn_s_memtime() - c0; a.dbg_buf[1] = __builtin_amdgcn_s_memrealtime() - r0; }
}

void launch_fused_roles(const FusedArgs &a, int cus, hipStream_t s, bool verify) {
    if (!a.h.n_tiles) return;
    static bool attr_set[2] = {false, false};
    if (!attr_set[verify]) {
        (void)hipFuncSetAttribute(verify ? reinterpret_cast<const void *>(k_fused_roles<false>) : reinterpret_cast<const void *>(k_fused_roles<true>),
                                  hipFuncAttributeMaxDynamicSharedMemorySize, (int)sizeof(RolesShared));
        attr_set[verify] = true;
    }
    const uint32_t want = (a.h.n_tiles + R_GROUP - 1) / R_GROUP;
    const uint32_t per_cu = sizeof(RolesShared) > 80 * 1024 ? 1u : 2u;
    uint32_t grid = std::min<uint32_t>((uint32_t)cus * per_cu, want);
    if (a.lds_pad) grid = std::min<uint32_t>(grid, a.lds_pad);
    if (verify) hipLaunchKernelGGL(k_fused_roles<false>, dim3(grid), dim3(R_WAVES * 64), sizeof(RolesShared), s, a);
    else hipLaunchKernelGGL(k_fused_roles<true>, dim3(grid), dim3(R_WAVES * 64), sizeof(RolesShared), s, a);
}

template <bool STORE>
__global__ __launch_bounds__(256, 4) void k_fused_blocks(FusedBlocksArgs a) {
    __shared__ __attribute__((aligned(16))) uint8_t s_area[4][STAGE_FULL_BYTES];
    uint32_t *const s_nodes = reinterpret_cast<uint32_t *>(&s_area[0][0]);
    constexpr uint32_t AREA_NODES = STAGE_FULL_BYTES / 32;
    static_assert(STAGE_FULL_BYTES % 32 == 0, "area must be a whole number of nodes");
    __shared__ uint32_t s_tab[3][4 * FOLD_UNITS];
    __shared__ __attribute__((aligned(16))) uint8_t s_Wb[4][WSTRIDE];
    __shared__ uint16_t s_d[4][3];
    const uint32_t lane = threadIdx.x & 63, w = threadIdx.x >> 6;
    if (lane < FOLD_UNITS) s_tab[0][w * FOLD_UNITS + lane] = 0;
    const uint32_t idx = blockIdx.x * 4 + w;
    if (idx < a.n_bt) {
        const uint32_t ti = a.bt_tile[idx], item = a.bt_item[idx];
        const Tile t = a.h.tiles[ti];
        const uint32_t row = t.first_unit;
        const uint32_t src_pos = a.item_src[item];
        const uint64_t usize = a.h.len[row];
        const uint64_t origin = (uint64_t)(t.first_leaf >> 7) << 17;
        if (src_pos != 0xFFFFFFFFu && a.row_flag[row] == 0 && t.n_leaves == 64 && usize - origin >= 128 * 1024) {
            uint8_t *const WL = s_Wb[w];
            const uint64_t n = a.blob_size[row];
            const uint8_t *const src = a.h.srcA + (a.h.offA[row] - a.h.baseA) + src_pos;
            const uint32_t avail = n - src_pos < WIN ? (uint32_t)(n - src_pos) : WIN;
            {
                const uint32_t o = 8 * lane;
                uint64_t v = 0;
                if (o + 8 <= avail) __builtin_memcpy(&v, src + o, 8);
                else
                    for (uint32_t k = 0; k < 8; k++)
                        if (o + k < avail) v |= (uint64_t)src[o + k] << (8 * k);
                *reinterpret_cast<uint64_t *>(WL + o) = v;
                if (lane < (WSTRIDE - WIN) / 4) *reinterpret_cast<uint32_t *>(WL + WIN + 4 * lane) = 0;
            }
            FastTabs T;
            {
                const DTab eL = c_dll[lane], eM = c_dml[lane], eO = c_dof[lane & 31];
                T.ll = eL.base | (uint32_t)eL.addbits << 24;
                T.ml = eM.base | (uint32_t)eM.addbits << 24;
                T.of = eO.addbits;
                T.lls = lane < 36 ? c_llb[lane] | (uint32_t)c_lla[lane] << 24 : 0u;
                T.mls = lane < 53 ? c_mlb[lane] | (uint32_t)c_mla[lane] << 24 : 0u;
            }
            const uint32_t bh = uni(*reinterpret_cast<const uint32_t *>(WL)) & 0xFFFFFF;
            if (avail >= 3 && ((bh >> 1) & 3) == 0 && (bh >> 3) == 128 * 1024 && src_pos + 3 + 128 * 1024ull <= n) {
                LeafOut lo;
                hash_tile_leaves<true, false, STORE, false, !STORE>(a.h, t, nullptr, lo, s_area[w], src + 3 - origin);
                uint4 *d = reinterpret_cast<uint4 *>(s_nodes + (size_t)(w * AREA_NODES + lane) * 8);
                d[0] = make_uint4(lo.cv[0], lo.cv[1], lo.cv[2], lo.cv[3]);
                d[1] = make_uint4(lo.cv[4], lo.cv[5], lo.cv[6], lo.cv[7]);
                if (lane == 0) {
                    s_tab[0][w * FOLD_UNITS] = 64;
                    s_tab[1][w * FOLD_UNITS] = w * AREA_NODES;
                    s_tab[2][w * FOLD_UNITS] = t.cv_index;
                    a.tile_done[ti] = 1;
                    a.item_done[item] = 1;
                }
            }
            const FastRow fr = parse_fast_block<false>(WL, 0, avail, 128 * 1024, avail >= 12, T);
            if (uni(fr.ok)) {
                const uint32_t lit_at = uni(fr.lit_at), L0 = uni(fr.L0), off = uni(fr.off);
                uint8_t *y = WL + lit_at;
                y[L0 + lane] = y[L0 - off + lmod(lane, off, 1.0f / (float)off)];
                if (lane == 0) { s_d[w][0] = (uint16_t)lit_at; s_d[w][1] = (uint16_t)(L0 - off); s_d[w][2] = (uint16_t)off; }
                LdsSrc ls{WL, &s_d[w][0], &s_d[w][1], &s_d[w][2], 1, nullptr, 0, 0, 0, 0, (!STORE || (a.dbg & 16)) ? 0u : 1u, origin};
                LeafOut lo;
                hash_tile_leaves<STORE, true, STORE>(a.h, t, &ls, lo, STORE ? s_area[w] : nullptr);
                uint4 *d = reinterpret_cast<uint4 *>(s_nodes + (size_t)(w * AREA_NODES + lane) * 8);
                d[0] = make_uint4(lo.cv[0], lo.cv[1], lo.cv[2], lo.cv[3]);
                d[1] = make_uint4(lo.cv[4], lo.cv[5], lo.cv[6], lo.cv[7]);
                if (lane == 0) {
                    s_tab[0][w * FOLD_UNITS] = 64;
                    s_tab[1][w * FOLD_UNITS] = w * AREA_NODES;
                    s_tab[2][w * FOLD_UNITS] = t.cv_index;
                    a.tile_done[ti] = 1;
                    a.item_done[item] = 1;
                }
            }
        }
    }
    lds_barrier();
    if (w != (blockIdx.x * 2654435761u) >> 30) return;
    FoldQueue<4> fq;
    fq.n_tab = 4 * FOLD_UNITS;
    fq.tb_n = s_tab[0][lane];
    fq.tb_off = s_tab[1][lane];
    fq.tb_out = s_tab[2][lane];
    fq.tb_root = 0;
    if (__ballot(fq.tb_n != 0) == 0ull) return;
    fq.fold_and_write(s_nodes, a.h);
}

void launch_fused_blocks(const FusedBlocksArgs &a, hipStream_t s, bool verify) {
    if (!a.n_bt) return;
    if (verify) hipLaunchKernelGGL(k_fused_blocks<false>, dim3((a.n_bt + 3) / 4), dim3(256), 0, s, a);
    else hipLaunchKernelGGL(k_fused_blocks<true>, dim3((a.n_bt + 3) / 4), dim3(256), 0, s, a);
}

void set_fused_dbg(unsigned long long *) {}
void set_fused_abl(int v) { (void)hipMemcpyToSymbol(HIP_SYMBOL(g_abl), &v, sizeof v); }

void launch_fused_small(const FusedArgs &a, hipStream_t s, int grid_cap, bool verify) {
    if (!a.h.n_tiles) return;
    uint32_t grid = (a.h.n_tiles + 3) / 4;
    if (grid_cap > 0 && grid > (uint32_t)grid_cap) grid = (uint32_t)grid_cap;
    if (verify) hipLaunchKernelGGL(k_fused_small<false>, dim3(grid), dim3(256), a.lds_pad, s, a);
    else hipLaunchKernelGGL(k_fused_small<true>, dim3(grid), dim3(256), a.lds_pad, s, a);
}

}
```

Measured before the change: 1.999 million MB/s.

## Fold verify and control reset into the roles kernel's last block

On the lean path, the roles kernel now compares each 6x10 tile's digests against stored checksums inline. It counts verified rows and bytes per workgroup, and records up to 64 odd-shaped tiles in a device list. The last block, chosen by a global ticket counter, checks the odd tiles, writes the counters and hand-over mirror to host memory, and zeroes the control head. This lets the next run skip the clear memset and the separate verify kernels. The aim is fewer launches and less per-run host/stream overhead. The cost is extra LDS, a grid-wide ticket serialisation, and hard-coded assumptions about the 6-row by 10240-byte tile shape.

```diff
diff --git a/znippy_amd/csrc/api.hip b/znippy_amd/csrc/api.hip
--- a/znippy_amd/csrc/api.hip
+++ b/znippy_amd/csrc/api.hip
@@ -105,7 +105,7 @@
         unsigned lds_pad = 0;
         int store_g = 0;
         bool no_block_items = false, no_fused_blocks = false, ddbg = false, edbg = false, no_fused_store = false,
-             nohash = false, no_roles = false, no_fz = false, fz_only = false, no_bx = false, tdbg = false, no_fuse_hash = false, trace = false, no_rx = false, no_pack = false, no_lean = false, no_stored_only = false;
+             nohash = false, no_roles = false, no_fz = false, fz_only = false, no_bx = false, tdbg = false, no_fuse_hash = false, trace = false, no_rx = false, no_pack = false, no_lean = false, no_stored_only = false, no_one_launch = false;
         unsigned roles_min = 2048;
         unsigned bx_big = BX_BIG_SEQ;
         bool bx_big_set = false;
@@ -134,6 +134,7 @@
     ctx->sw.tdbg = on("ZNIPPY_TDBG");
     ctx->sw.trace = on("ZNIPPY_TRACE");
     ctx->sw.no_lean = on("ZNIPPY_NO_LEAN");
+    ctx->sw.no_one_launch = on("ZNIPPY_NO_ONE_LAUNCH");
     ctx->sw.no_pack = on("ZNIPPY_NO_PACK");
     if (const char *e = getenv("ZNIPPY_STORE_G")) ctx->sw.store_g = atoi(e) == 1 ? 1 : (atoi(e) == 2 ? 2 : 0);
     ctx->sw.no_stored_only = on("ZNIPPY_NO_STORED_ONLY");
@@ -341,13 +342,15 @@
     H_TILES = 3,
     H_FLAGGED = 5,
 };
-enum Cursor : uint32_t { CUR_GENERAL = 0, CUR_ROLES = 2, CUR_ITEMS = 4, CUR_FALLBACK = 8, CUR_FZ = 12, CUR_FZ_WORK = 13 };
+enum Cursor : uint32_t { CUR_GENERAL = 0, CUR_ROLES = 2, CUR_ITEMS = 4, CUR_FALLBACK = 8, CUR_FZ = 12, CUR_FZ_WORK = 13,
+                         CUR_ODD = 14, CUR_TICKET = 15 };
+constexpr uint32_t ONE_ODD_CAP = 64;
 constexpr uint32_t LEAN_ANY = 1u << H_FUSED | 1u << H_SERIAL | 1u << H_FLAGGED, LEAN_SMALL = LEAN_ANY | 1u << H_TILES, LEAN_BLOCKS = LEAN_ANY | 1u << H_ITEMS;
 constexpr bool ctl_before(CtlRegion a, CtlRegion b) { return a.at + a.bytes <= b.at; }
 static_assert(ctl_before(CTL_COUNTERS, CTL_HAND) && ctl_before(CTL_HAND, CTL_CURSORS) && ctl_before(CTL_CURSORS, CTL_FZ_POOL) && ctl_before(CTL_FZ_POOL, CTL_BX_POOL) &&
               ctl_before(CTL_BX_POOL, CTL_BX_CTR) && ctl_before(CTL_BX_CTR, CTL_RX) && CTL_RX.at + CTL_RX.bytes <= CTL_HEAD, "control block: regions overlap or pass the head");
 static_assert(CTL_COUNTERS.at == 0 && CTL_HAND.at == CTL_COUNTERS.bytes && CTL_MIRROR == CTL_HAND.at + CTL_HAND.bytes, "the mirror is exactly counters + hand-over counts");
-static_assert(CTL_FLAG < 8 && H_FLAGGED == H_SERIAL + 4 && H_FLAGGED < 8 && CUR_FZ_WORK < 16 && zn::RX_ROUNDS <= RX_ZERO && RX_ZERO < 16, "control block: a word outside its region");
+static_assert(CTL_FLAG < 8 && H_FLAGGED == H_SERIAL + 4 && H_FLAGGED < 8 && CUR_TICKET < 16 && zn::RX_ROUNDS <= RX_ZERO && RX_ZERO < 16, "control block: a word outside its region");
 
 struct znippy_rows {
     znippy_ctx *ctx = nullptr;
@@ -394,6 +397,10 @@
     bool val_done = false, val_verify = false;
     uint32_t n_bad = 0;
     bool force_full = false;
+    uint32_t n_odd_tiles = 0;
+    int clean_hint = -1;
+    bool head_clean = false;
+    uint8_t *one_buf = nullptr;
     uint8_t *status_init = nullptr;
     bool odd_out = false;
     uint64_t *corrupt = nullptr;
@@ -1012,7 +1019,7 @@
                     r->cand_row, r->cand_base, r->cand_nblocks, r->fz_base, r->fz_cap, r->fz_it_cand, r->fz_nb, r->fz_work, r->fz_items, r->item_row, r->item_k, r->item_src, r->row_flag, r->pending2,
                     r->bt_tile, r->bt_item, r->tile_done, r->todo, r->status_init, r->slow_list,
                     r->bx_cand_row, r->bx_cand_base, r->bx_cand_nb, r->bx_huf_list, r->bx_seq_list, r->bx_items, r->bx_prep, r->d_bitmap, r->bx_sort_tmp,
-                    r->rx_base, r->rx_fail, r->rx_blk, r->rx_list, r->d_pack, r->d_pack_sums, r->all_rows, r->vs_off};
+                    r->rx_base, r->rx_fail, r->rx_blk, r->rx_list, r->d_pack, r->d_pack_sums, r->all_rows, r->vs_off, r->one_buf};
     for (void *p : ptrs)
         tfree(r->ctx, p);
     if (r->h_counters) {
@@ -1238,7 +1245,10 @@
     td.mark("plan");
     if ((rc = upload_plan(ctx, p, r->plan))) return rc;
     td.mark("plan_h2d");
-    for (const Tile &t : p.tiles) r->n_small_tiles += t.n_units != 0;
+    for (const Tile &t : p.tiles) {
+        r->n_small_tiles += t.n_units != 0;
+        r->n_odd_tiles += t.n_units != 0 && !(t.n_units == 6 && t.n_leaves == 60);
+    }
     if (r->n_small_tiles && tmalloc(ctx, &r->slow_list, 4 * (size_t)p.tiles.size()) != hipSuccess) return ZNIPPY_E_NOMEM;
     RowClasses k;
     rows_classify(ctx, r, c, k);
@@ -1343,6 +1353,7 @@
     r->bx_hint = (handed || r->n_list_a) ? 1 : 0;
     r->lean_hint = (handed || left[H_TILES]) ? 0 : 1;
     r->lean_hint2 = (handed || left[H_ITEMS]) ? 0 : 1;
+    r->clean_hint = (r->h_counters[16 * slot + 4] || r->h_counters[16 * slot + 5]) ? 0 : 1;
     if (r->n_small_tiles && left[H_TILES] >= r->n_small_tiles) r->roles_off = true;
     if (r->small_ok && left[H_FUSED] >= r->n) r->small_off = true;
     if (r->small_off) r->bx_hint = 1;
@@ -1354,6 +1365,7 @@
     bool stored_only;
     bool roles;
     bool lean;
+    bool one_launch;
     bool lean_mixed;
     bool decode;
     bool one_stream;
@@ -1373,6 +1385,7 @@
         p.roles = !sw.no_roles && sw.roles_min != 0 && r->n_small_tiles >= sw.roles_min && r->n_small_tiles > 0 && !(sw.dbg & (1 | 2 | 4 | 8 | 128)) && !r->roles_off;
         p.lean_mixed = r->lean_mixed_ok && r->lean_hint == 1 && r->bx_hint == 0 && may_skip && !sw.dbg && !sw.ddbg;
         p.lean = p.roles && r->lean_ok && r->lean_hint == 1 && r->bx_hint == 0 && may_skip && !sw.dbg;
+        p.one_launch = p.lean && !sw.no_one_launch && r->clean_hint == 1 && r->n_odd_tiles <= ONE_ODD_CAP;
     }
     p.decode = !p.lean && !p.lean_mixed && !p.stored_only;
     if (!p.decode) return p;
@@ -1435,6 +1448,28 @@
     if (run.preset) HIPCHK(ctx, hipMemcpyAsync(r->ctl, r->status_init, r->ctl_bytes, hipMemcpyDeviceToDevice, s));
     else HIPCHK(ctx, hipMemsetAsync(r->ctl, 0, r->ctl_bytes, s));
     if (p.small_off) HIPCHK(ctx, hipMemsetD32Async((hipDeviceptr_t)r->hand(H_FUSED), (int)r->n, 1, s));
+    return ZNIPPY_OK;
+}
+
+constexpr size_t ONE_ARG_STRIDE = 128;
+static_assert(sizeof(FusedArgs::OneLaunch) <= ONE_ARG_STRIDE, "one-launch arguments: more than their slot");
+static int rows_one_launch_args(znippy_ctx *ctx, znippy_rows *r) {
+    if (r->one_buf) return ZNIPPY_OK;
+    if (tmalloc(ctx, &r->one_buf, 2 * ONE_ARG_STRIDE + sizeof(uint2) * ONE_ODD_CAP) != hipSuccess) return ZNIPPY_E_NOMEM;
+    uint8_t img[2 * ONE_ARG_STRIDE] = {0};
+    for (unsigned slot = 0; slot < 2; slot++) {
+        FusedArgs::OneLaunch o{};
+        o.n_rows = r->n; o.flag = (uint32_t)CTL_FLAG;
+        o.checksum = r->checksum;
+        o.counters = r->ctl_at<unsigned long long>(CTL_COUNTERS);
+        o.hand = r->ctl_at<uint32_t>(CTL_HAND); o.lean_mask = LEAN_SMALL;
+        o.odd_cap = ONE_ODD_CAP; o.odd_list = reinterpret_cast<uint2 *>(r->one_buf + 2 * ONE_ARG_STRIDE);
+        o.odd_count = r->cur(CUR_ODD); o.ticket = r->cur(CUR_TICKET);
+        o.head = reinterpret_cast<uint32_t *>(r->ctl); o.n_head_words = (uint32_t)((CTL_CURSORS.at + CTL_CURSORS.bytes) / 4);
+        o.mirror = reinterpret_cast<uint32_t *>(r->h_counters + 16 * slot);
+        memcpy(img + ONE_ARG_STRIDE * slot, &o, sizeof o);
+    }
+    HIPCHK(ctx, hipMemcpy(r->one_buf, img, sizeof img, hipMemcpyHostToDevice));
     return ZNIPPY_OK;
 }
 
@@ -1469,6 +1504,7 @@
         f.cursor = r->cur(CUR_ROLES);
         f.tile_list = r->slow_list;
         f.tile_count = r->hand(H_TILES);
+        if (p.one_launch) f.one = reinterpret_cast<const FusedArgs::OneLaunch *>(r->one_buf + ONE_ARG_STRIDE * run.slot);
         timed(ctx, run.verify ? "verify_roles" : "decode_verify_roles", fs, [&] { launch_fused_roles(f, ctx->cus, fs, run.verify); });
     }
     if (r->n_small_tiles && !p.lean) timed(ctx, run.verify ? "verify_small" : "decode_verify_fused", fs, [&] { launch_fused_small(f, fs, p.roles ? ctx->cus * 5 : 0, run.verify); });
@@ -1721,13 +1757,21 @@
         if (tmalloc(ctx, &r->all_rows, 4 * (size_t)r->n) != hipSuccess) return ZNIPPY_E_NOMEM;
         hipLaunchKernelGGL(k_iota32, dim3((r->n + 255) / 256), dim3(256), 0, ctx->stream, r->all_rows, r->n);
     }
+    if (p.one_launch && (rc = rows_one_launch_args(ctx, r))) return rc;
     { auto &ra = r->run_args[slot]; ra.blobs = d_blobs; ra.base = blob_base; ra.out = verify ? nullptr : d_out; ra.cap = verify ? 0 : out_cap; ra.blob_cap = r->blob_cap; ra.verify = verify; }
     if (queued) *queued = true;
-    if ((rc = run_clear(ctx, r, p, run)) || !r->n) return rc;
+    const bool cleared = p.one_launch && r->head_clean;
+    r->head_clean = p.one_launch;
+    if ((!cleared && (rc = run_clear(ctx, r, p, run))) || !r->n) return rc;
     if (!p.small_off && !p.stored_only && (rc = run_small_rows(ctx, r, p, run))) return rc;
     if (p.decode && r->n_cand && (rc = run_block_items(ctx, r, p, run))) return rc;
     if (p.decode && r->n_compressed && (rc = p.bx ? run_batch_path(ctx, r, p, run) : run_serial_flow(ctx, r, p, run))) return rc;
     if (!p.lean) run_second_hash(ctx, r, p, run);
+    if (p.one_launch) {
+        HIPCHK(ctx, hipEventRecord(r->ev_done[run.slot], ctx->stream));
+        HIPCHK(ctx, hipGetLastError());
+        return ZNIPPY_OK;
+    }
     return run_verify(ctx, r, p, run);
 }
 
@@ -1748,6 +1792,7 @@
     r->run_seq = 0;
     r->force_full = true;
     r->lean_hint = 0; r->lean_hint2 = 0;
+    r->head_clean = false;
 }
 
 int znippy_decode_verify_rows_async(znippy_ctx *ctx, znippy_rows *r, const void *d_blobs,
diff --git a/znippy_amd/csrc/common.h b/znippy_amd/csrc/common.h
--- a/znippy_amd/csrc/common.h
+++ b/znippy_amd/csrc/common.h
@@ -86,6 +86,22 @@
     uint32_t *cursor;
     uint32_t *tile_list;
     uint32_t *tile_count;
+    struct OneLaunch {
+        uint32_t n_rows;
+        uint32_t flag;
+        const uint8_t *checksum;
+        unsigned long long *counters;
+        const uint32_t *hand;
+        uint32_t lean_mask;
+        uint32_t odd_cap;
+        uint2 *odd_list;
+        uint32_t *odd_count;
+        uint32_t *ticket;
+        uint32_t *head;
+        uint32_t n_head_words;
+        uint32_t *mirror;
+    };
+    const OneLaunch *one;
 };
 
 struct FusedBlocksArgs {
diff --git a/znippy_amd/csrc/fused_small.hip b/znippy_amd/csrc/fused_small.hip
--- a/znippy_amd/csrc/fused_small.hip
+++ b/znippy_amd/csrc/fused_small.hip
@@ -1022,9 +1022,11 @@
 __device__ __forceinline__ void lds_st(uint32_t *p, uint32_t v) { *(volatile lds_u32 *)p = v; }
 __device__ __forceinline__ void lds_fence() { asm volatile("s_waitcnt lgkmcnt(0)" ::: "memory"); }
 
+constexpr uint32_t R_WCK = 64 * 8;
+constexpr uint32_t V_ONE = 1u << 29, V_CMP = 1u << 30, V_BAD = 1u << 31, V_TILES = V_ONE - 1;
 struct alignas(16) RolesShared {
     uint8_t slots[R_SLOTS][R_SLOT_BYTES];
-    __attribute__((aligned(16))) uint32_t tree[R_WAVES - R_LOADERS][64 * 8];
+    __attribute__((aligned(16))) uint32_t tree[R_WAVES - R_LOADERS][64 * 8 + WROWS * 8];
     uint64_t oo[R_SLOTS][WROWS];
     uint32_t len[R_SLOTS][WROWS];
     uint32_t tn[R_SLOTS][WROWS], toff[R_SLOTS][WROWS];
@@ -1034,7 +1036,15 @@
     uint32_t next_iter;
     uint32_t cnt[R_SLOTS / R_GROUP];
     uint32_t gen[R_SLOTS / R_GROUP];
+    __attribute__((aligned(16))) uint32_t ck[R_SLOTS][WROWS][8];
+    uint32_t v_tiles, v_bad, v_done;
+    unsigned long long clk[2];
+    uint32_t one[2];
 };
+__device__ __forceinline__ const FusedArgs::OneLaunch *roles_one(const RolesShared &S) {
+    return reinterpret_cast<const FusedArgs::OneLaunch *>((uint64_t)lds_ld(&S.one[1]) << 32 | lds_ld(&S.one[0]));
+}
+static_assert(sizeof(RolesShared) <= 160 * 1024, "the ring must fit the CU's 160 KiB of LDS");
 
 __device__ __forceinline__ void emit_periodic_row(uint8_t *Y, uint32_t L0, uint32_t off, float inv, uint8_t *out, uint32_t osize,
                                                   uint32_t lane) {
@@ -1111,6 +1121,14 @@
             const uint64_t bs = a.blob_size[row];
             c_bs = bs > 0xFFFFFFFFull ? 0xFFFFFFFFu : (uint32_t)bs;
         }
+        const FusedArgs::OneLaunch *const one = roles_one(S);
+        const uint8_t *const ckp = one ? one->checksum : nullptr;
+        const bool ckv = ckp && rowv;
+        uint4 k0 = make_uint4(0, 0, 0, 0), k1 = k0;
+        if (ckv) {
+            const uint4 *k = reinterpret_cast<const uint4 *>(ckp) + (size_t)(t.first_unit + u) * 2;
+            k0 = k[0]; k1 = k[1];
+        }
         const bool want = rowv && c_sel && c_st == 0 && c_len != 0 && (c_len & 1023) == 0 && c_len <= 0x10000 &&
                           (!STORE || c_oo + c_len <= a.out_cap) && c_bs >= 12 && c_bs <= WIN;
         while (lds_ld(&S.gen[grp]) != use) __builtin_amdgcn_s_sleep(4);
@@ -1129,6 +1147,11 @@
             for (uint32_t k = 0; k < tail; k++) w4[k >> 2] |= (uint32_t)src[16 * full + k] << (8 * (k & 3));
             *reinterpret_cast<uint4 *>(win + 16 * full) = make_uint4(w4[0], w4[1], w4[2], w4[3]);
         }
+        if (ckv) {
+            lds_u4a *k = (lds_u4a *)S.ck[slot][u];
+            k[0] = u4v{k0.x, k0.y, k0.z, k0.w};
+            k[1] = u4v{k1.x, k1.y, k1.z, k1.w};
+        }
         const FastRow fr = parse_fast(win, c_bs, c_len, want, T);
         const uint64_t badm = __ballot(rowv && !fr.ok);
         const bool fast = cand && ((badm >> (16 * j)) & 0xFFFFull) == 0;
@@ -1179,9 +1202,15 @@
     return false;
 }
 
+__device__ __forceinline__ bool roles_differs(const uint32_t cv[8], const uint32_t *want) {
+    const lds_u4a *w = (const lds_u4a *)want;
+    const u4v w0 = w[0], w1 = w[1];
+    return ((cv[0] ^ w0.x) | (cv[1] ^ w0.y) | (cv[2] ^ w0.z) | (cv[3] ^ w0.w) | (cv[4] ^ w1.x) | (cv[5] ^ w1.y) | (cv[6] ^ w1.z) | (cv[7] ^ w1.w)) != 0;
+}
+
 template <bool STORE>
 __device__ __forceinline__ void roles_hash_6x10(const FusedArgs &a, RolesShared &S, uint32_t slot, uint32_t *tree, bool have_prev,
-                                                   uint32_t prev_first, uint32_t cv[8]) {
+                                                   uint32_t prev_first, uint32_t cv[8], uint32_t &acc) {
     typedef __attribute__((address_space(3))) uint8_t lds8b;
     const uint32_t lane = threadIdx.x & 63;
     const bool leaf = lane < 60;
@@ -1245,6 +1274,7 @@
                 uint4 *o = reinterpret_cast<uint4 *>(dig + (b - 13) * 32);
                 o[0] = make_uint4(cv[0], cv[1], cv[2], cv[3]);
                 o[1] = make_uint4(cv[4], cv[5], cv[6], cv[7]);
+                if ((acc & V_CMP) && roles_differs(cv, tree + R_WCK + ((b - 13) * 4 + ps) * 8)) acc |= V_BAD;
             } else {
                 lds_u4a *o = (lds_u4a *)(Y + wq);
                 o[0] = u4v{cv[0], cv[1], cv[2], cv[3]};
@@ -1254,7 +1284,7 @@
     }
 }
 
-__device__ __forceinline__ void roles_flush_tree_6x10(const FusedArgs &a, uint32_t *tree, uint32_t prev_first) {
+__device__ __forceinline__ void roles_flush_tree_6x10(const FusedArgs &a, uint32_t *tree, uint32_t prev_first, uint32_t &acc) {
     const uint32_t lane = threadIdx.x & 63;
 #pragma unroll 1
     for (uint32_t lv = 0; lv < 4; lv++) {
@@ -1275,6 +1305,7 @@
                 uint4 *o = reinterpret_cast<uint4 *>(a.h.digests + (size_t)(prev_first + l / 10) * 8);
                 o[0] = make_uint4(cv[0], cv[1], cv[2], cv[3]);
                 o[1] = make_uint4(cv[4], cv[5], cv[6], cv[7]);
+                if ((acc & V_CMP) && roles_differs(cv, tree + R_WCK + (l / 10) * 8)) acc |= V_BAD;
             } else {
                 lds_u4a *o = (lds_u4a *)(tree + l * 8);
                 o[0] = u4v{cv[0], cv[1], cv[2], cv[3]};
@@ -1285,12 +1316,82 @@
     }
 }
 
+__device__ __forceinline__ uint32_t ld_dev(const uint32_t *p) { return __hip_atomic_load(p, __ATOMIC_RELAXED, __HIP_MEMORY_SCOPE_AGENT); }
+__device__ __forceinline__ unsigned long long ld_dev(const unsigned long long *p) { return __hip_atomic_load(p, __ATOMIC_RELAXED, __HIP_MEMORY_SCOPE_AGENT); }
+__device__ __forceinline__ unsigned long long wave_sum(unsigned long long x) {
+#pragma unroll
+    for (int d = 32; d >= 1; d >>= 1) x += __shfl_xor(x, d);
+    return x;
+}
+
+__device__ __forceinline__ void roles_finish_run(const FusedArgs::OneLaunch &o, const uint32_t *digests, const uint64_t *len) {
+    static_assert(WROWS <= 8, "eight lanes per tile of the odd list");
+    const uint32_t lane = threadIdx.x & 63;
+    uint32_t flag = ld_dev(o.counters + o.flag) != 0ull;
+    uint32_t n_odd = ld_dev(o.odd_count);
+    if (n_odd > o.odd_cap) { n_odd = o.odd_cap; flag = 1; }
+    unsigned long long v_rows = 0, v_bytes = 0;
+    uint32_t differs = 0;
+    for (uint32_t e0 = 0; e0 < n_odd; e0 += 8) {
+        const uint32_t e = e0 + (lane >> 3), u = lane & 7;
+        if (e >= n_odd) continue;
+        const uint32_t *ent = reinterpret_cast<const uint32_t *>(o.odd_list + e);
+        const uint32_t first = ld_dev(ent), nu = ld_dev(ent + 1);
+        if (u >= nu || first + u >= o.n_rows) continue;
+        const uint32_t row = first + u;
+        uint32_t x = 0;
+        if (o.checksum) {
+            const uint32_t *want = reinterpret_cast<const uint32_t *>(o.checksum) + (size_t)row * 8, *got = digests + (size_t)row * 8;
+#pragma unroll
+            for (uint32_t q = 0; q < 8; q++) x |= want[q] ^ ld_dev(got + q);
+        }
+        v_rows += 1;
+        if (x) differs = 1;
+        else v_bytes += len[row];
+    }
+    const unsigned long long rows = ld_dev(o.counters + 0) + wave_sum(v_rows), bytes = ld_dev(o.counters + 2) + wave_sum(v_bytes);
+    const uint32_t hand = (lane >= 16 && lane < 32) ? ld_dev(o.hand + (lane - 16)) : 0u;
+    const bool left = lane >= 16 && lane < 32 && ((o.lean_mask >> (lane - 16)) & 1u) && hand != 0;
+    if (rows != o.n_rows || __ballot(differs != 0 || left) != 0ull) flag = 1;
+    uint32_t w = hand;
+    if (lane < 16) {
+        const unsigned long long c = lane < 2 ? rows : (lane < 6 ? bytes : (lane >> 1 == o.flag ? (unsigned long long)flag : 0ull));
+        w = (uint32_t)(lane & 1 ? c >> 32 : c);
+    }
+    if (lane < 32) __hip_atomic_store(o.mirror + lane, w, __ATOMIC_RELAXED, __HIP_MEMORY_SCOPE_SYSTEM);
+    __threadfence_system();
+    for (uint32_t i = lane; i < o.n_head_words; i += 64) o.head[i] = 0u;
+}
+
+__device__ __forceinline__ void roles_hasher_done(const FusedArgs::OneLaunch *one, const uint32_t *digests, const uint64_t *len, RolesShared *Sp, uint32_t acc) {
+    RolesShared &S = *Sp;
+    const uint32_t lane = threadIdx.x & 63;
+    __threadfence();
+    const uint32_t any_bad = __ballot((acc & V_BAD) != 0) != 0ull ? 1u : 0u;
+    atomicAdd(&S.v_tiles, lane == 0 ? acc & V_TILES : 0u);
+    atomicOr(&S.v_bad, lane == 0 ? any_bad : 0u);
+    lds_fence();
+    if (uni(atomicAdd(&S.v_done, lane == 0 ? 1u : 0u)) != R_WAVES - R_LOADERS - 1) return;
+    asm volatile("" ::: "memory");
+    const uint32_t tiles = lds_ld(&S.v_tiles), wg_bad = lds_ld(&S.v_bad);
+    const FusedArgs::OneLaunch o = *one;
+    atomicAdd(o.counters + 0, lane == 0 ? 6ull * tiles : 0ull);
+    atomicAdd(o.counters + 2, lane == 0 ? 6ull * 10240ull * tiles : 0ull);
+    if (wg_bad) atomicAdd(o.counters + o.flag, lane == 0 ? 1ull : 0ull);
+    __threadfence();
+    if (uni(atomicAdd(o.ticket, lane == 0 ? 1u : 0u)) != gridDim.x - 1) return;
+    __threadfence();
+    roles_finish_run(o, digests, len);
+}
+
 template <bool STORE>
-__device__ __forceinline__ void roles_hasher(const FusedArgs &a, RolesShared &S) {
+__device__ __forceinline__ uint32_t roles_hasher(const FusedArgs &a, RolesShared &S) {
     const uint32_t lane = threadIdx.x & 63;
     HashArgs h = a.h;
     h.pass = PASS_ALL;
     uint32_t *const tree = S.tree[(threadIdx.x >> 6) - R_LOADERS];
+    uint32_t acc = 0;
+    if (const FusedArgs::OneLaunch *one = roles_one(S)) acc = one->checksum ? V_ONE | V_CMP : V_ONE;
     bool have_prev = false;
     uint32_t prev_first = 0;
     const bool inline_tree = !(a.dbg & 524288);
@@ -1304,8 +1405,8 @@
             __builtin_amdgcn_s_sleep(2);
         }
         if (!go) {
-            if (have_prev) roles_flush_tree_6x10(a, tree, prev_first);
-            return;
+            if (have_prev) roles_flush_tree_6x10(a, tree, prev_first, acc);
+            return acc;
         }
         asm volatile("" ::: "memory");
         const uint32_t slot = take & (R_SLOTS - 1), grp = slot / R_GROUP;
@@ -1331,7 +1432,9 @@
                                   __ballot(lane < 6 && S.len[slot][lu] != 10240u) == 0ull;
             if (shape610) {
                 uint32_t cv[8];
-                roles_hash_6x10<STORE>(a, S, slot, tree, have_prev, prev_first, cv);
+                roles_hash_6x10<STORE>(a, S, slot, tree, have_prev, prev_first, cv, acc);
+                if ((acc & V_CMP) && lane < WROWS * 8) tree[R_WCK + lane] = S.ck[slot][0][lane];
+                acc++;
                 if (lane < 60) {
                     lds_u4a *o = (lds_u4a *)(tree + lane * 8);
                     o[0] = u4v{cv[0], cv[1], cv[2], cv[3]};
@@ -1341,6 +1444,12 @@
                 prev_first = t.first_unit;
                 if (lane < WROWS) S.tn[slot][lane] = 0u;
             } else {
+            if (acc & V_ONE) {
+                const FusedArgs::OneLaunch *const one = roles_one(S);
+                const uint32_t k = uni(atomicAdd(one->odd_count, lane == 0 ? 1u : 0u));
+                if (k >= one->odd_cap) acc |= V_BAD;
+                else if (lane == 0) one->odd_list[k] = make_uint2(t.first_unit, nu);
+            }
             LdsSrc ls{S.slots[slot], S.dy[slot], S.dB[slot], S.doff[slot], WROWS, nullptr,
                       lane < nu ? (uint64_t)S.len[slot][lu] : 0ull, 0ull, STORE ? S.oo[slot][lu] : 0ull, 1u,
                       (R_LOADER_EMITS || !STORE || (a.dbg & 16)) ? 0u : 0x3Fu, 0ull};
@@ -1397,16 +1506,18 @@
 __global__ __launch_bounds__(R_WAVES * 64) void k_fused_roles(FusedArgs a) {
     extern __shared__ __attribute__((aligned(16))) uint8_t s_roles_raw[];
     RolesShared &S = *reinterpret_cast<RolesShared *>(s_roles_raw);
-    if (threadIdx.x == 0) { S.ready = 0; S.take = 0; S.finished = 0; S.next_iter = 0; }
+    if (threadIdx.x == 0) { S.ready = 0; S.take = 0; S.finished = 0; S.next_iter = 0; S.v_tiles = 0; S.v_bad = 0; S.v_done = 0; S.one[0] = (uint32_t)(uintptr_t)a.one; S.one[1] = (uint32_t)((uintptr_t)a.one >> 32); }
     if (threadIdx.x < R_SLOTS / R_GROUP) { S.cnt[threadIdx.x] = 0; S.gen[threadIdx.x] = 0; }
     __syncthreads();
-    const bool clk = (a.dbg & 32768) && a.dbg_buf && blockIdx.x == 7 && threadIdx.x == 64 * R_LOADERS;
-    const unsigned long long c0 = clk ? __builtin_amdgcn_s_memtime() : 0, r0 = clk ? __builtin_amdgcn_s_memrealtime() : 0;
-    if (threadIdx.x < 64 * R_LOADERS) {
+    if ((a.dbg & 32768) && a.dbg_buf && blockIdx.x == 7 && threadIdx.x == 64 * R_LOADERS) { S.clk[0] = __builtin_amdgcn_s_memtime(); S.clk[1] = __builtin_amdgcn_s_memrealtime(); }
+    if (uni(threadIdx.x) < 64 * R_LOADERS) {
         if (!(a.dbg & 64)) __builtin_amdgcn_s_setprio(3);
         roles_loader<STORE>(a, S);
-    } else roles_hasher<STORE>(a, S);
-    if (clk) { a.dbg_buf[0] = __builtin_amdgcn_s_memtime() - c0; a.dbg_buf[1] = __builtin_amdgcn_s_memrealtime() - r0; }
+    } else {
+        const uint32_t acc = roles_hasher<STORE>(a, S);
+        if (acc & V_ONE) roles_hasher_done(roles_one(S), a.h.digests, a.h.len, &S, acc);
+    }
+    if ((a.dbg & 32768) && a.dbg_buf && blockIdx.x == 7 && threadIdx.x == 64 * R_LOADERS) { a.dbg_buf[0] = __builtin_amdgcn_s_memtime() - S.clk[0]; a.dbg_buf[1] = __builtin_amdgcn_s_memrealtime() - S.clk[1]; }
 }
 
 void launch_fused_roles(const FusedArgs &a, int cus, hipStream_t s, bool verify) {
```

Measured after the change: 996,000 MB/s. -50.2%, worse.
